# bronemos/view-fusion

Hardware: AMD Instinct MI355X
Metric: denoise_steps_per_sec (higher is better)
Workload: dtype f32; 1 GPU; small UNet 64x64 (33.9M params), B=16/GPU N=6 (S=96 views/GPU), training iteration fwd+bwd+Adam, linear T=2000 schedule; global_batch=16, views=6, parallelism=dp1, launch=HIP-graph replay of the whole iteration

## Files before the change

### include/vf_hip.h

```cpp
#ifndef VF_HIP_H
#define VF_HIP_H
#ifdef __cplusplus
extern "C" {
#endif

int vf_gn_fwd(const float* x, const float* gamma, const float* beta, float* y, float* mean ,
              float* rstd , int S, int C, int HW, int groups, float eps, int silu, void* stream);
int vf_gn_bwd_emits_rowsum(int C, int HW, int groups);
int vf_gn_bwd(const float* x, const float* gamma, const float* beta, const float* mean, const float* rstd,
              const float* dy, const float* addend, float* dx, float* dgamma_part, float* dbeta_part,
              float* dx_rowsum, int S, int C, int HW, int groups, int silu, void* stream);
int vf_gn_cat_fwd(const float* x, const float* x2, int C1, const float* gamma, const float* beta, float* y, float* mean,
                  float* rstd, int S, int C, int HW, int groups, float eps, int silu, void* stream);
int vf_gn_cat_bwd(const float* x, const float* x2, int C1, const float* gamma, const float* beta, const float* mean,
                  const float* rstd, const float* dy, const float* addend, const float* addend2, float* dx, float* dx2,
                  float* dgamma_part, float* dbeta_part, float* dx_rowsum, int S, int C, int HW, int groups, int silu,
                  void* stream);
int vf_rowsum(const float* x, float* out , int rows, int len, void* stream);
int vf_bias_grad(const float* dy, float* db, float* dvb, int S, int C, int HW, void* stream);
int vf_colsum(const float* part , float* out , int batch, int S, int C,
              void* stream);
int vf_colsum_multi(const void* desc, int n, long total_blocks, void* stream);

int vf_conv_pack_sizes(int Cout, int Cin, int KS, long* fwd_floats, long* bwd_floats);
int vf_conv_pack_weights(const float* w_oihw, float* w_fwd, float* w_bwd , int Cout, int Cin, int KS,
                         void* stream);
int vf_conv_pack_weights_multi(const void* desc, int nlayers, long total_blocks, void* stream);
int vf_conv_fwd(const float* x, const float* w_packed, const float* bias ,
                const float* view_bias , const float* residual , float* y,
                float* ws , long ws_floats, int S, int Cin, int Cout, int H, int W, int KS, int mode,
                void* stream);
int vf_conv_fwd_gn(const float* x, const float* w_packed, const float* bias, const float* view_bias, const float* residual,
                   float* y, int store_y, const float* gn_gamma, const float* gn_beta, float* a_out, float* gn_stats,
                   int groups, float eps, int silu, float* ws, long ws_floats, int S, int Cin, int Cout, int H, int W,
                   int KS, int mode, void* stream);
int vf_conv_small_supported(int Cin, int Cout, int H, int W, int KS, int mode);
int vf_conv_small(const float* x, const float* x2 , int C1, const float* w_oihw, const float* bias ,
                  const float* view_bias , const float* residual , float* y, int S, int Cin, int Cout,
                  int H, int W, int KS, int mode, void* stream);
int vf_conv_small_res(const float* x, const float* w_oihw, const float* bias , const float* view_bias ,
                      float* y, int S, int Cin, int Cout, int H, int W, const float* rx, const float* rx2 ,
                      int rC1, int rC, const float* rw_oihw, const float* rbias , void* stream);
int vf_conv_small_gn(const float* x, const float* x2 , int C1, const float* w_oihw, const float* bias ,
                     const float* view_bias , const float* residual , float* y, int S, int Cin,
                     int Cout, int H, int W, int KS, const unsigned long long* in_stats ,
                     const float* in_gamma, const float* in_beta, int in_groups, float eps, int silu,
                     unsigned long long* out_stats , const float* rx , const float* rx2 ,
                     int rC1, int rC, const float* rw_oihw, const float* rbias , const float* w_packed ,
                     int mode, void* stream);
long vf_conv_small_pack_floats(int Cout, int Cin);
int vf_conv_small_pack(const float* w_oihw, float* w_packed, int Cout, int Cin, void* stream);
long vf_conv_fwd_ws_floats(int S, int Cin, int Cout, int H, int W, int KS);
int vf_conv1x1_cat_fwd(const float* x1, const float* x2, int C1, const float* w_packed, const float* bias, float* y,
                       float* ws, long ws_floats, int S, int Cin, int Cout, int H, int W, void* stream);
int vf_conv1x1_cat_dgrad(const float* dy, const float* w_packed_bwd, float* dx1, float* dx2, int C1, int S, int Cin,
                         int Cout, int H, int W, void* stream);
int vf_conv1x1_cat_wgrad(const float* x1, const float* x2, int C1, const float* dy, float* dw_oihw, float* ws,
                         long ws_floats, int S, int Cin, int Cout, int H, int W, void* stream);
long vf_conv1x1_bf16x3_pack_dwords(int M, int K);
int vf_conv1x1_bf16x3_pack(const float* w_oihw, void* w3_fwd, void* w3_bwd, int Cout, int Cin, void* stream);
int vf_conv1x1_bf16x3(const float* x, const float* x2, int C1in, const void* w3, const float* bias,
                      const float* view_bias, const float* residual, float* y, float* y2, int C1out, int S, int Cin,
                      int Cout, int HW, void* stream);
long vf_conv_wgrad_ws_floats(int S, int Cin, int Cout, int H, int W, int KS);
int vf_conv_wgrad(const float* x, const float* dy, float* dw_oihw, float* ws, long ws_floats, int S, int Cin,
                  int Cout, int H, int W, int KS, int mode, void* stream);
int vf_conv_wgrad_main(const float* x, const float* dy, float* dw_oihw, float* ws, long ws_floats, int S, int Cin,
                       int Cout, int H, int W, int KS, int mode, long long* desc9, int* nblocks, void* stream);
int vf_conv1x1_cat_wgrad_main(const float* x1, const float* x2, int C1, const float* dy, float* dw_oihw, float* ws,
                              long ws_floats, int S, int Cin, int Cout, int H, int W, long long* desc9, int* nblocks,
                              void* stream);
int vf_sumpool2(const float* x, float* y, long n_out, int Wo, void* stream);

int vf_wino_supported(int H, int W, int mode);
int vf_wino_pack_sizes(int Cout, int Cin, long* fwd_floats, long* bwd_floats);
int vf_wino_pack_weights(const float* w_oihw, float* u_fwd, float* u_bwd , int Cout, int Cin,
                         void* stream);
int vf_wino_pack_weights_multi(const void* desc, int nlayers, long total_blocks, void* stream);
long vf_wino_conv_ws_floats(int S, int Cin, int Cout, int H, int W);
int vf_wino_conv_fill_pct(int S, int Cin, int Cout, int H, int W, int* tiles_out);
int vf_wino_conv_fwd(const float* x, const float* u_packed, const float* bias, const float* view_bias,
                     const float* residual, float* y, float* ws, long ws_floats, int S, int Cin, int Cout, int H,
                     int W, int mode, void* stream);
int vf_wino_conv_gn_fusable(int S, int Cin, int Cout, int H, int W, int mode, int groups);
int vf_wino_conv_fwd_gn(const float* x, const float* u_packed, const float* bias , const float* view_bias ,
                        const float* residual , float* y, int store_y, const float* gn_gamma, const float* gn_beta,
                        float* a_out, int groups, float eps, int silu, float* ws, long ws_floats, int S, int Cin, int Cout,
                        int H, int W, int mode, void* stream);
int vf_wino44_supported(int H, int W, int mode);
int vf_wino44_pack_sizes(int Cout, int Cin, long* fwd_floats, long* bwd_floats);
int vf_wino44_pack_weights(const float* w_oihw, float* u_fwd, float* u_bwd , int Cout, int Cin,
                           void* stream);
int vf_wino44_pack_weights_multi(const void* desc, int nlayers, long total_blocks, void* stream);
long vf_wino44_conv_ws_floats(int S, int Cin, int Cout, int H, int W);
int vf_wino44_conv_fill_pct(int S, int Cin, int Cout, int H, int W, int* tiles_out);
int vf_wino44_conv_fwd(const float* x, const float* u_packed, const float* bias, const float* view_bias,
                       const float* residual, float* y, float* ws, long ws_floats, int S, int Cin, int Cout, int H,
                       int W, int mode, void* stream);
int vf_wino_wgrad_supported(int H, int W, int mode);
long vf_wino_wgrad_ws_floats(int S, int Cin, int Cout, int H, int W);
int vf_wino_wgrad(const float* x, const float* dy, float* dw_oihw, float* db, float* db2, float* ws, long ws_floats,
                  int S, int Cin, int Cout, int H, int W, int mode, void* stream);
int vf_wino_wgrad_main(const float* x, const float* dy, float* dw_oihw, float* db, float* db2, float* ws, long ws_floats,
                       int S, int Cin, int Cout, int H, int W, int mode, long long* desc9, int* nblocks, void* stream);
int vf_wino44_reduce_multi(const void* table, int nrows, int nblocks, void* stream);

int vf_time_affine_fwd(const void* desc, int ngroups, const float* emb, float* out, int S, int K, int CT,
                       void* stream);
long vf_time_affine_ws_floats(int S, int K);
int vf_time_affine_bwd(const void* desc, int ngroups, const float* emb, const float* de, float* dw ,
                       float* db , const void* gdst, float* demb , float* ws, int S, int K,
                       int CT, void* stream);

int vf_bgemm(const float* A, const float* B, float* C, const float* bias , int batch, int M, int N,
             int K, long sAb, long sAm, long sAk, long sBb, long sBk, long sBn, long sCb, long sCm, long sCn,
             float alpha, float beta, void* stream);
int vf_attention_fwd(const float* qkv, float* out, float* P , int S, int C, int L, void* stream);
int vf_attention_dscore(const float* qkv, const float* dO, const float* P, float* dS, float* dqkv, int S, int C, int L,
                        void* stream);
int vf_attention_dvdk(const float* qkv, const float* dO, const float* P, const float* dS, float* dqkv, int S, int C, int L,
                      void* stream);
int vf_attn_stream_fwd(const float* qkv, float* out, float* lse , int S, int C, int L, void* stream);
int vf_attn_stream_bwd(const float* qkv, const float* out, const float* dO, const float* lse, float* delta,
                       float* dqkv, int S, int C, int L, void* stream);
int vf_softmax_fwd(const float* x, float* y, int rows, int cols, void* stream);
int vf_softmax_bwd(const float* y, const float* dy, float* dx, int rows, int cols, void* stream);

int vf_sincos_embed(const float* level , const float* angle , float* out , int S, int dim,
                    void* stream);
int vf_swish_fwd(const float* x, float* y, long n, void* stream);
int vf_swish_bwd(const float* x, const float* dy, float* dx, long n, void* stream);
int vf_concat_channels(float* a, float* b, float* out, int S, long na, long nb, int split, void* stream);
int vf_dropout(const float* x, const float* u, float* y, long n, float p, void* stream);

int vf_gather_level(const float* gammas, const long long* t, const float* u , float* level, int B,
                    void* stream);
int vf_stack_views(const float* y_cond , const float* y_t ,
                   const float* noise , const float* level, const float* angle, const int* off ,
                   float* x , float* level_s, float* angle_s, int B, int Nmax,
                   int Cc , int HW, int S,
                   int copy_cond, void* stream);
int vf_compose_fwd(const float* unet_out, const int* off, const float* target , float* noise_hat,
                   float* weights , float* loss_part , float* loss, int B,
                   int Cout, int HW, int maxV, int weighting, void* stream);
int vf_compose_mse_bwd(const float* unet_out, const int* off, const float* target, const float* noise_hat,
                       const float* gloss, float* dout, int B, int Cout, int HW, int weighting, void* stream);
int vf_p_sample_tail(const float* unet_out, const int* off, const float* y_t, const float* z ,
                     const long long* t, const float* sqrt_recip_gammas, const float* sqrt_recipm1_gammas,
                     const float* posterior_log_variance, const float* posterior_mean_coef1,
                     const float* posterior_mean_coef2, float* y_next , float* mean_out ,
                     float* weights , int B, int Cout, int HW, int maxV, int weighting, int clip,
                     void* stream);

int vf_psnr(const float* generated, const float* target, float* out , int B, int n, void* stream);

int vf_adam_multi(const void* desc, int ntensors, long total_blocks, float lr, float beta1, float beta2, float eps,
                  float bias_correction1, float bias_correction2, void* stream);
int vf_adam_multi_dev(const void* desc, int ntensors, long total_blocks, const float* scalars, float beta1, float beta2,
                      float eps, void* stream);
int vf_adam_set_scalars(float* scalars, float lr, float bc1, float bc2, void* stream);

int vf_xgmi_alloc(void** ptr, long bytes);
int vf_xgmi_free(void* ptr);
int vf_xgmi_export(void* ptr, void* handle64 );
int vf_xgmi_open(const void* handle64, void** ptr);
int vf_xgmi_close(void* ptr);
int vf_xgmi_signal(const void* const* peer_flags, int world, int rank, int slot, unsigned epoch, void* stream);
int vf_xgmi_wait(const void* my_flags, int world, int slot_lo, int slot_hi, unsigned epoch, void* status,
                 long timeout_us, void* stream);
int vf_xgmi_reduce_adam(const void* desc, int ntensors, long total_blocks, const void* const* peer_bases,
                        const float* my_base, float* gavg_base, int world, const float* scalars, float beta1,
                        float beta2, float eps, void* stream);

#ifdef __cplusplus
}
#endif
#endif
```

### view_fusion_amd/_lib.py

```python
import ctypes
import os

import torch

_HERE = os.path.dirname(os.path.abspath(__file__))
LIB_PATH = os.path.join(_HERE, "lib", "libvf_hip.so")
_OVERRIDE = os.environ.get("VF_HIP_LIB") if os.environ.get("VF_DEBUG_AB") == "1" else None
if _OVERRIDE:
    LIB_PATH = _OVERRIDE
elif os.environ.get("VF_HIP_LIB"):
    import warnings
    warnings.warn("VF_HIP_LIB is ignored unless VF_DEBUG_AB=1 (kernel-tuning aid)", stacklevel=2)

_P, _I, _L, _F = ctypes.c_void_p, ctypes.c_int, ctypes.c_long, ctypes.c_float

SIGNATURES = {
    "vf_gn_fwd": [_P, _P, _P, _P, _P, _P, _I, _I, _I, _I, _F, _I, _P],
    "vf_gn_bwd_emits_rowsum": [_I, _I, _I],
    "vf_gn_cat_fwd": [_P, _P, _I, _P, _P, _P, _P, _P, _I, _I, _I, _I, _F, _I, _P],
    "vf_gn_cat_bwd": [_P, _P, _I, _P, _P, _P, _P, _P, _P, _P, _P, _P, _P, _P, _P, _I, _I, _I, _I, _I, _P],
    "vf_conv1x1_cat_fwd": [_P, _P, _I, _P, _P, _P, _P, _L, _I, _I, _I, _I, _I, _P],
    "vf_conv1x1_cat_dgrad": [_P, _P, _P, _P, _I, _I, _I, _I, _I, _I, _P],
    "vf_conv1x1_cat_wgrad": [_P, _P, _I, _P, _P, _P, _L, _I, _I, _I, _I, _I, _P],
    "vf_gn_bwd": [_P, _P, _P, _P, _P, _P, _P, _P, _P, _P, _P, _I, _I, _I, _I, _I, _P],
    "vf_rowsum": [_P, _P, _I, _I, _P],
    "vf_bias_grad": [_P, _P, _P, _I, _I, _I, _P],
    "vf_colsum": [_P, _P, _I, _I, _I, _P],
    "vf_colsum_multi": [_P, _I, _L, _P],
    "vf_conv_pack_sizes": [_I, _I, _I, ctypes.POINTER(_L), ctypes.POINTER(_L)],
    "vf_conv_pack_weights": [_P, _P, _P, _I, _I, _I, _P],
    "vf_conv_pack_weights_multi": [_P, _I, _L, _P],
    "vf_conv_fwd": [_P, _P, _P, _P, _P, _P, _P, _L, _I, _I, _I, _I, _I, _I, _I, _P],
    "vf_conv_fwd_ws_floats": [_I, _I, _I, _I, _I, _I],
    "vf_conv_fwd_gn": [_P, _P, _P, _P, _P, _P, _I, _P, _P, _P, _P, _I, _F, _I, _P, _L, _I, _I, _I, _I, _I, _I, _I, _P],
    "vf_conv_wgrad_ws_floats": [_I, _I, _I, _I, _I, _I],
    "vf_conv_wgrad": [_P, _P, _P, _P, _L, _I, _I, _I, _I, _I, _I, _I, _P],
    "vf_conv1x1_bf16x3_pack_dwords": [_I, _I],
    "vf_conv1x1_bf16x3_pack": [_P, _P, _P, _I, _I, _P],
    "vf_conv1x1_bf16x3": [_P, _P, _I, _P, _P, _P, _P, _P, _P, _I, _I, _I, _I, _I, _P],
    "vf_wino_supported": [_I, _I, _I],
    "vf_wino_pack_sizes": [_I, _I, ctypes.POINTER(_L), ctypes.POINTER(_L)],
    "vf_wino_pack_weights": [_P, _P, _P, _I, _I, _P],
    "vf_wino_pack_weights_multi": [_P, _I, _L, _P],
    "vf_wino_conv_ws_floats": [_I, _I, _I, _I, _I],
    "vf_wino_conv_fill_pct": [_I, _I, _I, _I, _I, ctypes.POINTER(_I)],
    "vf_wino_conv_fwd": [_P, _P, _P, _P, _P, _P, _P, _L, _I, _I, _I, _I, _I, _I, _P],
    "vf_wino_conv_gn_fusable": [_I, _I, _I, _I, _I, _I, _I],
    "vf_wino_conv_fwd_gn": [_P, _P, _P, _P, _P, _P, _I, _P, _P, _P, _I, _F, _I, _P, _L, _I, _I, _I, _I, _I, _I, _P],
    "vf_wino44_supported": [_I, _I, _I],
    "vf_wino44_pack_sizes": [_I, _I, ctypes.POINTER(_L), ctypes.POINTER(_L)],
    "vf_wino44_pack_weights": [_P, _P, _P, _I, _I, _P],
    "vf_wino44_pack_weights_multi": [_P, _I, _L, _P],
    "vf_wino44_conv_ws_floats": [_I, _I, _I, _I, _I],
    "vf_wino44_conv_fill_pct": [_I, _I, _I, _I, _I, ctypes.POINTER(_I)],
    "vf_wino44_conv_fwd": [_P, _P, _P, _P, _P, _P, _P, _L, _I, _I, _I, _I, _I, _I, _P],
    "vf_wino_wgrad_ws_floats": [_I, _I, _I, _I, _I],
    "vf_wino_wgrad_supported": [_I, _I, _I],
    "vf_wino_wgrad": [_P, _P, _P, _P, _P, _P, _L, _I, _I, _I, _I, _I, _I, _P],
    "vf_wino_wgrad_main": [_P, _P, _P, _P, _P, _P, _L, _I, _I, _I, _I, _I, _I, _P, _P, _P],
    "vf_wino44_reduce_multi": [_P, _I, _I, _P],
    "vf_conv_wgrad_main": [_P, _P, _P, _P, _L, _I, _I, _I, _I, _I, _I, _I, _P, _P, _P],
    "vf_conv1x1_cat_wgrad_main": [_P, _P, _I, _P, _P, _P, _L, _I, _I, _I, _I, _I, _P, _P, _P],
    "vf_sumpool2": [_P, _P, _L, _I, _P],
    "vf_time_affine_fwd": [_P, _I, _P, _P, _I, _I, _I, _P],
    "vf_time_affine_ws_floats": [_I, _I],
    "vf_time_affine_bwd": [_P, _I, _P, _P, _P, _P, _P, _P, _P, _I, _I, _I, _P],
    "vf_bgemm": [_P, _P, _P, _P, _I, _I, _I, _I, _L, _L, _L, _L, _L, _L, _L, _L, _L, _F, _F, _P],
    "vf_attention_fwd": [_P, _P, _P, _I, _I, _I, _P],
    "vf_attention_dscore": [_P, _P, _P, _P, _P, _I, _I, _I, _P],
    "vf_attention_dvdk": [_P, _P, _P, _P, _P, _I, _I, _I, _P],
    "vf_attn_stream_fwd": [_P, _P, _P, _I, _I, _I, _P],
    "vf_attn_stream_bwd": [_P, _P, _P, _P, _P, _P, _I, _I, _I, _P],
    "vf_softmax_fwd": [_P, _P, _I, _I, _P],
    "vf_softmax_bwd": [_P, _P, _P, _I, _I, _P],
    "vf_sincos_embed": [_P, _P, _P, _I, _I, _P],
    "vf_swish_fwd": [_P, _P, _L, _P],
    "vf_swish_bwd": [_P, _P, _P, _L, _P],
    "vf_concat_channels": [_P, _P, _P, _I, _L, _L, _I, _P],
    "vf_dropout": [_P, _P, _P, _L, _F, _P],
    "vf_adam_multi": [_P, _I, _L, _F, _F, _F, _F, _F, _F, _P],
    "vf_conv_small_supported": [_I, _I, _I, _I, _I, _I],
    "vf_conv_small": [_P, _P, _I, _P, _P, _P, _P, _P, _I, _I, _I, _I, _I, _I, _I, _P],
    "vf_conv_small_res": [_P, _P, _P, _P, _P, _I, _I, _I, _I, _I, _P, _P, _I, _I, _P, _P, _P],
    "vf_conv_small_gn": [_P, _P, _I, _P, _P, _P, _P, _P, _I, _I, _I, _I, _I, _I, _P, _P, _P, _I, _F, _I, _P, _P, _P, _I, _I,
                         _P, _P, _P, _I, _P],
    "vf_conv_small_pack_floats": [_I, _I],
    "vf_conv_small_pack": [_P, _P, _I, _I, _P],
    "vf_adam_multi_dev": [_P, _I, _L, _P, _F, _F, _F, _P],
    "vf_adam_set_scalars": [_P, _F, _F, _F, _P],
    "vf_xgmi_alloc": [ctypes.POINTER(_P), _L],
    "vf_xgmi_free": [_P],
    "vf_xgmi_export": [_P, _P],
    "vf_xgmi_open": [_P, ctypes.POINTER(_P)],
    "vf_xgmi_close": [_P],
    "vf_xgmi_signal": [ctypes.POINTER(_P), _I, _I, _I, ctypes.c_uint, _P],
    "vf_xgmi_wait": [_P, _I, _I, _I, ctypes.c_uint, _P, _L, _P],
    "vf_xgmi_reduce_adam": [_P, _I, _L, ctypes.POINTER(_P), _P, _P, _I, _P, _F, _F, _F, _P],
    "vf_psnr": [_P, _P, _P, _I, _I, _P],
    "vf_gather_level": [_P, _P, _P, _P, _I, _P],
    "vf_stack_views": [_P, _P, _P, _P, _P, _P, _P, _P, _P, _I, _I, _I, _I, _I, _I, _P],
    "vf_compose_fwd": [_P, _P, _P, _P, _P, _P, _P, _I, _I, _I, _I, _I, _P],
    "vf_compose_mse_bwd": [_P, _P, _P, _P, _P, _P, _I, _I, _I, _I, _P],
    "vf_p_sample_tail": [_P, _P, _P, _P, _P, _P, _P, _P, _P, _P, _P, _P, _P, _I, _I, _I, _I, _I, _I, _P],
}
_RESTYPE = {"vf_conv1x1_bf16x3_pack_dwords": _L, "vf_conv_wgrad_ws_floats": _L, "vf_time_affine_ws_floats": _L, "vf_wino_conv_ws_floats": _L, "vf_wino44_conv_ws_floats": _L, "vf_wino_wgrad_ws_floats": _L, "vf_conv_fwd_ws_floats": _L,
            "vf_conv_small_pack_floats": _L}

_lib = None
N_CALLS = 0


class VFHipError(RuntimeError):
    pass


def load():
    global _lib
    if _lib is None:
        if not os.path.exists(LIB_PATH):
            raise VFHipError(
                f"{LIB_PATH} not found: build it with `python -m view_fusion_amd.build` "
                "(there is no CPU / eager fallback for the ViewFusion hot path)")
        lib = ctypes.CDLL(LIB_PATH)
        if _OVERRIDE:
            import sys
            print(f"[view_fusion_amd] VF_DEBUG_AB: loading {LIB_PATH} instead of lib/libvf_hip.so", file=sys.stderr)
        missing = [name for name in SIGNATURES if not hasattr(lib, name)]
        if missing:
            raise VFHipError(f"{LIB_PATH} does not export {missing}: stale build? run `python -m view_fusion_amd.build`")
        for name, args in SIGNATURES.items():
            fn = getattr(lib, name)
            fn.argtypes = args
            fn.restype = _RESTYPE.get(name, _I)
        _lib = lib
    return _lib


def call(name, *args):
    global N_CALLS
    N_CALLS += 1
    rc = getattr(load(), name)(*args)
    if rc != 0:
        raise VFHipError(f"{name} failed with hipError_t {rc}")
```

### view_fusion_amd/csrc/common.h

```cpp
#pragma once
#include <hip/hip_runtime.h>
#include <stdint.h>

typedef float f32x2 __attribute__((ext_vector_type(2)));
typedef float f32x4 __attribute__((ext_vector_type(4)));
typedef float f32x16 __attribute__((ext_vector_type(16)));

#define VF_WAVE 64

#define VF_RETURN_LAST_ERROR() return (int)hipGetLastError()

__device__ __forceinline__ float wave_sum(float v) {
#pragma unroll
    for (int o = 32; o > 0; o >>= 1) v += __shfl_xor(v, o, VF_WAVE);
    return v;
}

template <int SEG>
__device__ __forceinline__ float seg_sum(float v) {
#pragma unroll
    for (int o = SEG / 2; o > 0; o >>= 1) v += __shfl_xor(v, o, VF_WAVE);
    return v;
}

__device__ __forceinline__ float wave_max(float v) {
#pragma unroll
    for (int o = 32; o > 0; o >>= 1) v = fmaxf(v, __shfl_xor(v, o, VF_WAVE));
    return v;
}

template <int NT>
__device__ __forceinline__ float block_sum(float v, float* red) {
    v = wave_sum(v);
    const int lane = threadIdx.x & 63, wid = threadIdx.x >> 6;
    __syncthreads();
    if (lane == 0) red[wid] = v;
    __syncthreads();
    float t = 0.f;
#pragma unroll
    for (int i = 0; i < NT / 64; ++i) t += red[i];
    return t;
}

__device__ __forceinline__ float sigmoid_f(float z) {
#ifdef VF_EXACT_SILU
    return 1.0f / (1.0f + expf(-z));
#else
    return __builtin_amdgcn_rcpf(1.0f + __builtin_amdgcn_exp2f(z * -1.44269504088896341f));
#endif
}
__device__ __forceinline__ float silu_f(float z) { return z * sigmoid_f(z); }

__device__ __forceinline__ unsigned xcd_remap(unsigned bid, unsigned nblk) {
    const unsigned q = nblk >> 3, r = nblk & 7u;
    const unsigned xcd = bid & 7u, slot = bid >> 3;
    const unsigned start = xcd < r ? xcd * (q + 1) : r * (q + 1) + (xcd - r) * q;
    return start + slot;
}

__device__ __forceinline__ f32x2 pk_sub(f32x2 a, f32x2 b) {
    f32x2 d;
    asm("v_pk_add_f32 %0, %1, %2 neg_lo:[0,1] neg_hi:[0,1]" : "=v"(d) : "v"(a), "v"(b));
    return d;
}
__device__ __forceinline__ f32x2 pk_add(f32x2 a, f32x2 b) {
    f32x2 d;
    asm("v_pk_add_f32 %0, %1, %2" : "=v"(d) : "v"(a), "v"(b));
    return d;
}
template <int K>
__device__ __forceinline__ f32x2 pk_fmak(f32x2 a, f32x2 c) {
    f32x2 d;
    if (K == 2) asm("v_pk_fma_f32 %0, %1, 2.0, %2 op_sel_hi:[1,0,1]" : "=v"(d) : "v"(a), "v"(c));
    else if (K == 4) asm("v_pk_fma_f32 %0, %1, 4.0, %2 op_sel_hi:[1,0,1]" : "=v"(d) : "v"(a), "v"(c));
    else {
        const f32x2 a2 = pk_add(a, a);
        asm("v_pk_fma_f32 %0, %1, 4.0, %2 op_sel_hi:[1,0,1]" : "=v"(d) : "v"(a2), "v"(c));
    }
    return d;
}
__device__ __forceinline__ f32x2 pk_fma(f32x2 a, f32x2 b, f32x2 c) {
    f32x2 d;
    asm("v_pk_fma_f32 %0, %1, %2, %3" : "=v"(d) : "v"(a), "v"(b), "v"(c));
    return d;
}
__device__ __forceinline__ f32x2 pk_nmul4_add(f32x2 a, f32x2 c) {
    f32x2 d;
    asm("v_pk_fma_f32 %0, %1, 4.0, %2 op_sel_hi:[1,0,1] neg_lo:[1,0,0] neg_hi:[1,0,0]" : "=v"(d) : "v"(a), "v"(c));
    return d;
}
__device__ __forceinline__ f32x2 pk_hi_pm_lo(f32x2 p) {
    f32x2 d;
    asm("v_pk_add_f32 %0, %1, %1 op_sel:[1,0] op_sel_hi:[1,0] neg_hi:[0,1]" : "=v"(d) : "v"(p));
    return d;
}
__device__ __forceinline__ f32x2 pk_hi_pm_2lo(f32x2 q) {
    f32x2 d;
    asm("v_pk_fma_f32 %0, %1, 2.0, %1 op_sel:[0,0,1] op_sel_hi:[0,0,1] neg_hi:[1,0,0]" : "=v"(d) : "v"(q));
    return d;
}
__device__ __forceinline__ f32x2 pk_lo_pm_hi(f32x2 a, f32x2 b) {
    f32x2 d;
    asm("v_pk_add_f32 %0, %1, %2 op_sel:[0,1] op_sel_hi:[0,1] neg_hi:[0,1]" : "=v"(d) : "v"(a), "v"(b));
    return d;
}

__device__ __forceinline__ float dpp_row_shr1(float v) {
    return __int_as_float(__builtin_amdgcn_update_dpp(0, __float_as_int(v), 0x111, 0xf, 0xf, true));
}

#define VF_LDS_BARRIER() asm volatile("s_waitcnt lgkmcnt(0)\n\ts_barrier" ::: "memory")

__device__ __forceinline__ const char* uniform_ptr(const void* p) {
    const unsigned long long v = (unsigned long long)p;
    const unsigned lo = __builtin_amdgcn_readfirstlane((unsigned)v), hi = __builtin_amdgcn_readfirstlane((unsigned)(v >> 32));
    return (const char*)(((unsigned long long)hi << 32) | lo);
}
```

### view_fusion_amd/csrc/norm.hip

```cpp
#include "common.h"
#include "any_geom.h"

namespace {

__device__ __forceinline__ float4 ld_nt(const float4* p) {
    const f32x4 t = __builtin_nontemporal_load(reinterpret_cast<const f32x4*>(p));
    return make_float4(t.x, t.y, t.z, t.w);
}

__device__ __forceinline__ const float4* cat_ptr(const float* x1, const float* x2, int C1, int C, int s, int c,
                                                 int HW) {
    return reinterpret_cast<const float4*>(c < C1 ? x1 + ((size_t)s * C1 + c) * HW
                                                  : x2 + ((size_t)s * (C - C1) + (c - C1)) * HW);
}

template <int NV, int NT>
__global__ __launch_bounds__(NT) void gn_fwd_kernel(const float* __restrict__ x, const float* __restrict__ x2, int C1,
                                                    const float* __restrict__ gamma,
                                                    const float* __restrict__ beta,
                                                    float* __restrict__ y, float* __restrict__ mean_out,
                                                    float* __restrict__ rstd_out, int C, int HW, int cpg,
                                                    float eps, int silu) {
    __shared__ float red[NT / 64];
    const int G = C / cpg;
    const int sg = blockIdx.x;
    const int s = sg / G, g = sg - s * G;
    const size_t base = ((size_t)s * C + (size_t)g * cpg) * HW;
    const int n = cpg * HW, n4 = n >> 2;
    const int hwsh = 31 - __clz(HW >> 2), hwmask = (HW >> 2) - 1;
    const float4* x4 = reinterpret_cast<const float4*>(x + base);
    float4* y4 = reinterpret_cast<float4*>(y + base);

    float4 v[NV];
    float gam[NV], bet[NV];
    if (x2) {
#pragma unroll
        for (int i = 0; i < NV; ++i) {
            const int idc = min((int)threadIdx.x + i * NT, n4 - 1);
            v[i] = cat_ptr(x, x2, C1, C, s, g * cpg + (idc >> hwsh), HW)[idc & hwmask];
        }
    } else {
#pragma unroll
        for (int i = 0; i < NV; ++i) v[i] = x4[min((int)threadIdx.x + i * NT, n4 - 1)];
    }
#pragma unroll
    for (int i = 0; i < NV; ++i) {
        const int c = g * cpg + (min((int)threadIdx.x + i * NT, n4 - 1) >> hwsh);
        gam[i] = gamma[c];
        bet[i] = beta[c];
    }
#ifdef VF_GN_PRESTATS
    const float mean = mean_out[sg], rstd = rstd_out[sg];
    (void)red; (void)n; (void)eps;
#else
    float sum = 0.f;
#pragma unroll
    for (int i = 0; i < NV; ++i) {
        if ((int)threadIdx.x + i * NT >= n4) v[i] = make_float4(0.f, 0.f, 0.f, 0.f);
        sum += (v[i].x + v[i].y) + (v[i].z + v[i].w);
    }
    const float mean = block_sum<NT>(sum, red) / (float)n;
    float sq = 0.f;
#pragma unroll
    for (int i = 0; i < NV; ++i) {
        const float a = v[i].x - mean, b = v[i].y - mean, c = v[i].z - mean, d = v[i].w - mean;
        const float q = (a * a + b * b) + (c * c + d * d);
        sq += (int)threadIdx.x + i * NT < n4 ? q : 0.f;
    }
    const float var = block_sum<NT>(sq, red) / (float)n;
    const float rstd = 1.0f / sqrtf(var + eps);
    if (threadIdx.x == 0) {
        mean_out[sg] = mean;
        rstd_out[sg] = rstd;
    }
#endif
#pragma unroll
    for (int i = 0; i < NV; ++i) {
        const int idx = threadIdx.x + i * NT;
        if (idx < n4) {
            const float ga = gam[i] * rstd;
            const float be = bet[i] - mean * ga;
            float4 o;
            o.x = v[i].x * ga + be;
            o.y = v[i].y * ga + be;
            o.z = v[i].z * ga + be;
            o.w = v[i].w * ga + be;
            if (silu) {
                o.x = silu_f(o.x);
                o.y = silu_f(o.y);
                o.z = silu_f(o.z);
                o.w = silu_f(o.w);
            }
            y4[idx] = o;
        }
    }
}

__device__ __forceinline__ float dsilu_mul(float z, float dy) {
    const float sg = sigmoid_f(z);
    return dy * (sg * (1.0f + z * (1.0f - sg)));
}

__global__ __launch_bounds__(256) void gn_bwd_rows_kernel(const float* __restrict__ x,
                                                          const float* __restrict__ dy,
                                                          const float* __restrict__ gamma,
                                                          const float* __restrict__ beta,
                                                          const float* __restrict__ mean,
                                                          const float* __restrict__ rstd,
                                                          float* __restrict__ dbeta_part,
                                                          float* __restrict__ dgamma_part, int rows, int C,
                                                          int HW, int cpg, int silu) {
    const int row = blockIdx.x * 4 + (threadIdx.x >> 6);
    if (row >= rows) return;
    const int lane = threadIdx.x & 63;
    const int s = row / C, c = row - s * C;
    const int sg = s * (C / cpg) + c / cpg;
    const float mu = mean[sg], r = rstd[sg], ga = gamma[c], be = beta[c];
    const float4* x4 = reinterpret_cast<const float4*>(x + (size_t)row * HW);
    const float4* d4 = reinterpret_cast<const float4*>(dy + (size_t)row * HW);
    float a = 0.f, b = 0.f;
    for (int i = lane; i < (HW >> 2); i += 64) {
        const float4 xv = x4[i], dv = d4[i];
        const float xs[4] = {xv.x, xv.y, xv.z, xv.w};
        const float ds[4] = {dv.x, dv.y, dv.z, dv.w};
#pragma unroll
        for (int j = 0; j < 4; ++j) {
            const float xh = (xs[j] - mu) * r;
            const float dz = silu ? dsilu_mul(xh * ga + be, ds[j]) : ds[j];
            a += dz;
            b += dz * xh;
        }
    }
    a = wave_sum(a);
    b = wave_sum(b);
    if (lane == 0) {
        dbeta_part[row] = a;
        dgamma_part[row] = b;
    }
}

__global__ __launch_bounds__(256) void gn_bwd_dx_kernel(const float* __restrict__ x,
                                                        const float* __restrict__ dy,
                                                        const float* __restrict__ gamma,
                                                        const float* __restrict__ beta,
                                                        const float* __restrict__ mean,
                                                        const float* __restrict__ rstd,
                                                        const float* __restrict__ dbeta_part,
                                                        const float* __restrict__ dgamma_part,
                                                        float* __restrict__ dx, int C, int HW, int cpg,
                                                        int silu) {
    const int G = C / cpg;
    const int sg = blockIdx.x;
    const int s = sg / G, g = sg - s * G;
    float s1 = 0.f, s2 = 0.f;
    for (int j = 0; j < cpg; ++j) {
        const int c = g * cpg + j;
        const float ga = gamma[c];
        s1 += ga * dbeta_part[s * C + c];
        s2 += ga * dgamma_part[s * C + c];
    }
    const int n = cpg * HW, n4 = n >> 2;
    const int hwsh = 31 - __clz(HW >> 2);
    const float inv_n = 1.0f / (float)n;
    s1 *= inv_n;
    s2 *= inv_n;
    const float mu = mean[sg], r = rstd[sg];
    const size_t base = ((size_t)s * C + (size_t)g * cpg) * HW;
    const float4* x4 = reinterpret_cast<const float4*>(x + base);
    const float4* d4 = reinterpret_cast<const float4*>(dy + base);
    float4* o4 = reinterpret_cast<float4*>(dx + base);
    for (int i = blockIdx.y * 256 + threadIdx.x; i < n4; i += gridDim.y * 256) {
        const int c = g * cpg + (i >> hwsh);
        const float ga = gamma[c], be = beta[c];
        const float4 xv = x4[i], dv = d4[i];
        const float xs[4] = {xv.x, xv.y, xv.z, xv.w};
        const float ds[4] = {dv.x, dv.y, dv.z, dv.w};
        float o[4];
#pragma unroll
        for (int j = 0; j < 4; ++j) {
            const float xh = (xs[j] - mu) * r;
            const float dz = silu ? dsilu_mul(xh * ga + be, ds[j]) : ds[j];
            o[j] = r * (dz * ga - (s1 + xh * s2));
        }
        o4[i] = make_float4(o[0], o[1], o[2], o[3]);
    }
}


template <int NV, int NT, int SEG = 64>
__global__ __launch_bounds__(NT) void gn_bwd_fused_kernel(const float* __restrict__ x, const float* __restrict__ x2,
                                                          int C1, const float* __restrict__ dy,
                                                          const float* __restrict__ gamma,
                                                          const float* __restrict__ beta,
                                                          const float* __restrict__ mean,
                                                          const float* __restrict__ rstd,
                                                          const float* __restrict__ addend,
                                                          const float* __restrict__ addend2, float* __restrict__ dx,
                                                          float* __restrict__ dx2,
                                                          float* __restrict__ dgamma_part,
                                                          float* __restrict__ dbeta_part,
                                                          float* __restrict__ dx_rowsum, int C, int HW, int cpg,
                                                          int silu) {
    constexpr int NWV = NT / 64;
    extern __shared__ float part[];
    const int G = C / cpg;
    const int sg = blockIdx.x;
    const int s = sg / G, g = sg - s * G;
    const size_t base = ((size_t)s * C + (size_t)g * cpg) * HW;
    const int n = cpg * HW, n4 = n >> 2;
    const int hwsh = 31 - __clz(HW >> 2), hwmask = (HW >> 2) - 1;
    const float4* x4 = reinterpret_cast<const float4*>(x + base);
    const float4* d4 = reinterpret_cast<const float4*>(dy + base);
    const int lane = threadIdx.x & 63, wid = threadIdx.x >> 6;
    const float mu = mean[sg], r = rstd[sg];

    for (int i = threadIdx.x; i < NWV * cpg * 3; i += NT) part[i] = 0.f;
    __syncthreads();

    float4 xv[NV], dv[NV];
    float gam[NV], bet[NV];
    if (x2) {
#pragma unroll
        for (int i = 0; i < NV; ++i) {
            const int idc = min((int)threadIdx.x + i * NT, n4 - 1);
            xv[i] = cat_ptr(x, x2, C1, C, s, g * cpg + (idc >> hwsh), HW)[idc & hwmask];
            dv[i] = d4[idc];
        }
    } else {
#pragma unroll
        for (int i = 0; i < NV; ++i) {
            const int idc = min((int)threadIdx.x + i * NT, n4 - 1);
            xv[i] = ld_nt(x4 + idc);
            dv[i] = ld_nt(d4 + idc);
        }
    }
#pragma unroll
    for (int i = 0; i < NV; ++i) {
        if (SEG == 64) {
            const int c = __builtin_amdgcn_readfirstlane(g * cpg + (min(wid * 64 + i * NT, n4 - 1) >> hwsh));
            gam[i] = gamma[c];
            bet[i] = beta[c];
        } else {
            const int c = g * cpg + (min((int)threadIdx.x + i * NT, n4 - 1) >> hwsh);
            gam[i] = gamma[c];
            bet[i] = beta[c];
        }
    }
#pragma unroll
    for (int i = 0; i < NV; ++i) {
        const int idx0 = wid * 64 + i * NT + (SEG == 64 ? 0 : (lane & ~(SEG - 1)));
        float a = 0.f, b = 0.f, xsum = 0.f;
        int cl = 0;
        if (idx0 < n4) {
            cl = idx0 >> hwsh;
            const float ga = gam[i], be = bet[i];
            float xs[4] = {xv[i].x, xv[i].y, xv[i].z, xv[i].w};
            float ds[4] = {dv[i].x, dv[i].y, dv[i].z, dv[i].w};
            const bool ok = threadIdx.x + i * NT < n4;
#pragma unroll
            for (int j = 0; j < 4; ++j) {
                const float xh = (xs[j] - mu) * r;
                float dz = silu ? dsilu_mul(xh * ga + be, ds[j]) : ds[j];
                if (!ok) dz = 0.f;
                xs[j] = xh; ds[j] = dz;
                a += dz; b += dz * xh;
                xsum += ok ? xh : 0.f;
            }
            xv[i] = make_float4(xs[0], xs[1], xs[2], xs[3]);
            dv[i] = make_float4(ds[0], ds[1], ds[2], ds[3]);
        }
        a = seg_sum<SEG>(a);
        b = seg_sum<SEG>(b);
        if (dx_rowsum) xsum = seg_sum<SEG>(xsum);
        if ((lane & (SEG - 1)) == 0 && idx0 < n4) {
            part[(wid * cpg + cl) * 3 + 0] += a;
            part[(wid * cpg + cl) * 3 + 1] += b;
            part[(wid * cpg + cl) * 3 + 2] += xsum;
        }
    }
    __syncthreads();
    float s1 = 0.f, s2 = 0.f, myA = 0.f, myX = 0.f;
    for (int c = 0; c < cpg; ++c) {
        float A = 0.f, B = 0.f, X = 0.f;
#pragma unroll
        for (int w = 0; w < NWV; ++w) {
            A += part[(w * cpg + c) * 3]; B += part[(w * cpg + c) * 3 + 1]; X += part[(w * cpg + c) * 3 + 2];
        }
        const float ga = gamma[g * cpg + c];
        s1 += ga * A; s2 += ga * B;
        if (threadIdx.x == c) {
            dbeta_part[(size_t)s * C + g * cpg + c] = A;
            dgamma_part[(size_t)s * C + g * cpg + c] = B;
            myA = ga * A; myX = X;
        }
    }
    const float inv_n = 1.0f / (float)n;
    s1 *= inv_n; s2 *= inv_n;
    if (dx_rowsum && threadIdx.x < cpg)
        dx_rowsum[(size_t)s * C + g * cpg + threadIdx.x] = r * (myA - (float)HW * s1 - s2 * myX);
    float4* o4 = reinterpret_cast<float4*>(dx + base);
    const float4* a4 = addend ? reinterpret_cast<const float4*>(addend + base) : nullptr;
#pragma unroll
    for (int i = 0; i < NV; ++i) {
        const float ga = gam[i];
        dv[i].x = r * (dv[i].x * ga - (s1 + xv[i].x * s2));
        dv[i].y = r * (dv[i].y * ga - (s1 + xv[i].y * s2));
        dv[i].z = r * (dv[i].z * ga - (s1 + xv[i].z * s2));
        dv[i].w = r * (dv[i].w * ga - (s1 + xv[i].w * s2));
    }
    if (x2) {
        if (addend) {
#pragma unroll
            for (int i = 0; i < NV; ++i) {
                const int idc = min((int)threadIdx.x + i * NT, n4 - 1);
                xv[i] = cat_ptr(addend, addend2, C1, C, s, g * cpg + (idc >> hwsh), HW)[idc & hwmask];
            }
#pragma unroll
            for (int i = 0; i < NV; ++i) { dv[i].x += xv[i].x; dv[i].y += xv[i].y; dv[i].z += xv[i].z; dv[i].w += xv[i].w; }
        }
#pragma unroll
        for (int i = 0; i < NV; ++i) {
            const int idx = threadIdx.x + i * NT;
            if (idx < n4)
                const_cast<float4*>(cat_ptr(dx, dx2, C1, C, s, g * cpg + (idx >> hwsh), HW))[idx & hwmask] = dv[i];
        }
        return;
    }
    if (a4) {
#pragma unroll
        for (int i = 0; i < NV; ++i) xv[i] = a4[min((int)threadIdx.x + i * NT, n4 - 1)];
#pragma unroll
        for (int i = 0; i < NV; ++i) { dv[i].x += xv[i].x; dv[i].y += xv[i].y; dv[i].z += xv[i].z; dv[i].w += xv[i].w; }
    }
    if (addend2) {
        const float4* b4 = reinterpret_cast<const float4*>(addend2 + base);
#pragma unroll
        for (int i = 0; i < NV; ++i) xv[i] = b4[min((int)threadIdx.x + i * NT, n4 - 1)];
#pragma unroll
        for (int i = 0; i < NV; ++i) { dv[i].x += xv[i].x; dv[i].y += xv[i].y; dv[i].z += xv[i].z; dv[i].w += xv[i].w; }
    }
#pragma unroll
    for (int i = 0; i < NV; ++i) {
        const int idx = threadIdx.x + i * NT;
        if (idx < n4) o4[idx] = dv[i];
    }
}

__global__ void add_inplace_kernel(float4* __restrict__ y, const float4* __restrict__ a, size_t n4) {
    const size_t i = (size_t)blockIdx.x * blockDim.x + threadIdx.x;
    if (i < n4) { float4 v = y[i]; const float4 t = a[i]; v.x += t.x; v.y += t.y; v.z += t.z; v.w += t.w; y[i] = v; }
}

__device__ __forceinline__ float lane_sum_f4(const float4* __restrict__ p, int n4, int lane) {
    float acc[8] = {0.f, 0.f, 0.f, 0.f, 0.f, 0.f, 0.f, 0.f};
    int i = lane;
    for (; i + 7 * 64 < n4; i += 8 * 64) {
        float4 v[8];
#pragma unroll
        for (int j = 0; j < 8; ++j) v[j] = p[i + 64 * j];
#pragma unroll
        for (int j = 0; j < 8; ++j) acc[j] += (v[j].x + v[j].y) + (v[j].z + v[j].w);
    }
    if (i < n4) {
        float4 v[8];
#pragma unroll
        for (int j = 0; j < 8; ++j) v[j] = p[min(i + 64 * j, n4 - 1)];
#pragma unroll
        for (int j = 0; j < 8; ++j) acc[j] += i + 64 * j < n4 ? (v[j].x + v[j].y) + (v[j].z + v[j].w) : 0.f;
    }
    return ((acc[0] + acc[1]) + (acc[2] + acc[3])) + ((acc[4] + acc[5]) + (acc[6] + acc[7]));
}

__global__ __launch_bounds__(256) void rowsum_kernel(const float* __restrict__ x, float* __restrict__ out,
                                                     int rows, int len) {
    const int row = blockIdx.x * 4 + (threadIdx.x >> 6);
    if (row >= rows) return;
    const int lane = threadIdx.x & 63;
    const float4* x4 = reinterpret_cast<const float4*>(x + (size_t)row * len);
    const float a = wave_sum(lane_sum_f4(x4, len >> 2, lane));
    if (lane == 0) out[row] = a;
}

__global__ __launch_bounds__(256) void bias_grad_kernel(const float* __restrict__ dy, float* __restrict__ db,
                                                        float* __restrict__ dvb, int S, int C, int HW) {
    __shared__ float red[4];
    const int c = blockIdx.x, lane = threadIdx.x & 63, wid = threadIdx.x >> 6;
    float tot = 0.f;
    const int n4 = HW >> 2;
    if (n4 <= 64) {
        for (int s = wid; s < S; s += 32) {
            float4 v[8];
#pragma unroll
            for (int j = 0; j < 8; ++j)
                v[j] = reinterpret_cast<const float4*>(dy + ((size_t)min(s + 4 * j, S - 1) * C + c) * HW)[min(lane, n4 - 1)];
#pragma unroll
            for (int j = 0; j < 8; ++j) {
                const float a = wave_sum(lane < n4 ? (v[j].x + v[j].y) + (v[j].z + v[j].w) : 0.f);
                if (s + 4 * j < S) {
                    if (lane == 0 && dvb) dvb[(size_t)(s + 4 * j) * C + c] = a;
                    tot += a;
                }
            }
        }
    } else {
        for (int s = wid; s < S; s += 4) {
            const float4* p = reinterpret_cast<const float4*>(dy + ((size_t)s * C + c) * HW);
            const float a = wave_sum(lane_sum_f4(p, n4, lane));
            if (lane == 0 && dvb) dvb[(size_t)s * C + c] = a;
            tot += a;
        }
    }
    if (lane == 0) red[wid] = tot;
    __syncthreads();
    if (threadIdx.x == 0 && db) db[c] = (red[0] + red[1]) + (red[2] + red[3]);
}

__global__ __launch_bounds__(256) void colsum_kernel(const float* __restrict__ part, float* __restrict__ out,
                                                     int S, int C) {
    __shared__ float red[4][64];
    const int cx = threadIdx.x & 63, ry = threadIdx.x >> 6;
    const int c = blockIdx.x * 64 + cx;
    const float* p = part + (size_t)blockIdx.y * S * C;
    float a = 0.f;
    if (c < C) {
        float acc[8] = {0.f, 0.f, 0.f, 0.f, 0.f, 0.f, 0.f, 0.f};
        for (int s = ry; s < S; s += 32) {
            float t[8];
#pragma unroll
            for (int j = 0; j < 8; ++j) t[j] = p[(size_t)min(s + 4 * j, S - 1) * C + c];
#pragma unroll
            for (int j = 0; j < 8; ++j) acc[j] += s + 4 * j < S ? t[j] : 0.f;
        }
        a = ((acc[0] + acc[1]) + (acc[2] + acc[3])) + ((acc[4] + acc[5]) + (acc[6] + acc[7]));
    }
    red[ry][cx] = a;
    __syncthreads();
    if (ry == 0 && c < C) out[(size_t)blockIdx.y * C + c] = (red[0][cx] + red[1][cx]) + (red[2][cx] + red[3][cx]);
}

struct ColsumDesc {
    const float* part;
    float* out;
    long long S, C, batch, first_block;
};
__global__ __launch_bounds__(256) void colsum_multi_kernel(const ColsumDesc* __restrict__ desc, int n) {
    __shared__ float red[4][64];
    const long long vb = blockIdx.x;
    int lo = 0, hi = n;
    while (hi - lo > 1) {
        const int mid = (lo + hi) >> 1;
        if (desc[mid].first_block <= vb) lo = mid; else hi = mid;
    }
    const ColsumDesc d = desc[lo];
    const int S = (int)d.S, C = (int)d.C;
    const int nbx = (C + 63) / 64;
    const int rel = (int)(vb - d.first_block);
    const int bx = rel % nbx, by = rel / nbx;
    const int cx = threadIdx.x & 63, ry = threadIdx.x >> 6;
    const int c = bx * 64 + cx;
    const float* p = d.part + (size_t)by * S * C;
    float a = 0.f;
    if (c < C) {
        float acc[8] = {0.f, 0.f, 0.f, 0.f, 0.f, 0.f, 0.f, 0.f};
        for (int s = ry; s < S; s += 32) {
            float t[8];
#pragma unroll
            for (int j = 0; j < 8; ++j) t[j] = p[(size_t)min(s + 4 * j, S - 1) * C + c];
#pragma unroll
            for (int j = 0; j < 8; ++j) acc[j] += s + 4 * j < S ? t[j] : 0.f;
        }
        a = ((acc[0] + acc[1]) + (acc[2] + acc[3])) + ((acc[4] + acc[5]) + (acc[6] + acc[7]));
    }
    red[ry][cx] = a;
    __syncthreads();
    if (ry == 0 && c < C) d.out[(size_t)by * C + c] = (red[0][cx] + red[1][cx]) + (red[2][cx] + red[3][cx]);
}

template <int NV, int NT>
int launch_gn_fwd(const float* x, const float* x2, int C1, const float* gamma, const float* beta, float* y, float* mean,
                  float* rstd, int S, int C, int HW, int cpg, float eps, int silu, hipStream_t st) {
    hipLaunchKernelGGL((gn_fwd_kernel<NV, NT>), dim3(S * (C / cpg)), dim3(NT), 0, st, x, x2, C1, gamma, beta, y, mean,
                       rstd, C, HW, cpg, eps, silu);
    VF_RETURN_LAST_ERROR();
}

}

extern "C" {

int vf_gn_cat_fwd(const float* x, const float* x2, int C1, const float* gamma, const float* beta, float* y, float* mean,
                  float* rstd, int S, int C, int HW, int groups, float eps, int silu, void* stream) {
    hipStream_t st = (hipStream_t)stream;
    if (S <= 0) return 0;
    if (groups <= 0 || C % groups != 0 || (x2 && (C1 <= 0 || C1 >= C))) return (int)hipErrorInvalidValue;
    const int cpg = C / groups;
    const long n4 = (long)cpg * HW / 4;
    if (HW < 4 || (HW & (HW - 1)) || n4 > 32768) {
        if (x2) return (int)hipErrorInvalidValue;
        return vfi_gn_any_fwd(x, gamma, beta, y, mean, rstd, S, C, HW, groups, eps, silu, st);
    }
#define VF_GN(NV, NT) return launch_gn_fwd<NV, NT>(x, x2, C1, gamma, beta, y, mean, rstd, S, C, HW, cpg, eps, silu, st)
    if (n4 <= 64) VF_GN(1, 64);
    if (n4 <= 256) VF_GN(1, 256);
    if (n4 <= 512) VF_GN(2, 256);
    if (n4 <= 1024) VF_GN(4, 256);
    if (n4 <= 2048) VF_GN(8, 256);
    if (n4 <= 3072) VF_GN(12, 256);
    if (n4 <= 4096) VF_GN(16, 256);
    if (n4 <= 6144) VF_GN(12, 512);
    if (n4 <= 8192) VF_GN(16, 512);
    if (n4 <= 16384) VF_GN(16, 1024);
    if (n4 <= 32768) VF_GN(32, 1024);
#undef VF_GN
    return (int)hipErrorInvalidValue;
}

int vf_gn_fwd(const float* x, const float* gamma, const float* beta, float* y, float* mean, float* rstd, int S,
              int C, int HW, int groups, float eps, int silu, void* stream) {
    return vf_gn_cat_fwd(x, nullptr, C, gamma, beta, y, mean, rstd, S, C, HW, groups, eps, silu, stream);
}

int vf_gn_bwd_emits_rowsum(int C, int HW, int groups) {
    if (groups <= 0 || C % groups != 0 || HW < 4 || (HW & (HW - 1))) return 0;
    const long n4g = (long)(C / groups) * HW / 4;
    return ((HW >= 256 && n4g <= 8192) || (HW == 64 && n4g <= 1024)) ? 1 : 0;
}

int vf_gn_cat_bwd(const float* x, const float* x2, int C1, const float* gamma, const float* beta, const float* mean,
                  const float* rstd, const float* dy, const float* addend, const float* addend2, float* dx, float* dx2,
                  float* dgamma_part, float* dbeta_part, float* dx_rowsum, int S, int C, int HW, int groups, int silu,
                  void* stream) {
    hipStream_t st = (hipStream_t)stream;
    if (S <= 0) return 0;
    if (groups <= 0 || C % groups != 0) return (int)hipErrorInvalidValue;
    if (HW < 4 || (HW & (HW - 1))) {
        if (x2) return (int)hipErrorInvalidValue;
        return vfi_gn_any_bwd(x, gamma, beta, mean, rstd, dy, addend, addend2, dx, dgamma_part, dbeta_part, S, C, HW, groups,
                              silu, st);
    }
    if (x2 && (C1 <= 0 || C1 >= C || !dx2 || (addend && !addend2) || !vf_gn_bwd_emits_rowsum(C, HW, groups)))
        return (int)hipErrorInvalidValue;
    const int cpg = C / groups;
    const int rows = S * C;
    const long n4g = (long)cpg * HW / 4;
    if (HW == 64 && n4g <= 1024) {
#define VF_GNB16(NV)                                                                                       \
    {                                                                                                      \
        hipLaunchKernelGGL((gn_bwd_fused_kernel<NV, 256, 16>), dim3(S * groups), dim3(256), 4 * cpg * 3 * 4, st, x, x2, C1, dy, \
                           gamma, beta, mean, rstd, addend, addend2, dx, dx2, dgamma_part, dbeta_part, dx_rowsum, C, HW, cpg, silu); \
        VF_RETURN_LAST_ERROR();                                                                            \
    }
        if (n4g <= 256) VF_GNB16(1)
        if (n4g <= 512) VF_GNB16(2)
        VF_GNB16(4)
#undef VF_GNB16
    }
    if (HW >= 256 && n4g <= 8192) {
#define VF_GNB(NV, NT)                                                                                     \
    {                                                                                                      \
        hipLaunchKernelGGL((gn_bwd_fused_kernel<NV, NT>), dim3(S * groups), dim3(NT), (NT / 64) * cpg * 3 * 4, st, \
                           x, x2, C1, dy, gamma, beta, mean, rstd, addend, addend2, dx, dx2, dgamma_part, dbeta_part, \
                           dx_rowsum, C, HW, cpg, silu);                                                   \
        VF_RETURN_LAST_ERROR();                                                                            \
    }
        if (n4g <= 256) VF_GNB(1, 256)
        if (n4g <= 512) VF_GNB(2, 256)
        if (n4g <= 1024) VF_GNB(4, 256)
        if (n4g <= 2048) VF_GNB(8, 256)
        if (n4g <= 4096) VF_GNB(8, 512)
        if (n4g <= 6144) VF_GNB(12, 512)
        VF_GNB(8, 1024)
#undef VF_GNB
    }
    hipLaunchKernelGGL(gn_bwd_rows_kernel, dim3((rows + 3) / 4), dim3(256), 0, st, x, dy, gamma, beta, mean, rstd,
                       dbeta_part, dgamma_part, rows, C, HW, cpg, silu);
    const int n4 = cpg * HW / 4;
    int chunks = (n4 + 1023) / 1024;
    if (chunks < 1) chunks = 1;
    hipLaunchKernelGGL(gn_bwd_dx_kernel, dim3(S * groups, chunks), dim3(256), 0, st, x, dy, gamma, beta, mean,
                       rstd, dbeta_part, dgamma_part, dx, C, HW, cpg, silu);
    const size_t t4 = (size_t)S * C * HW / 4;
    if (addend)
        hipLaunchKernelGGL(add_inplace_kernel, dim3((unsigned)((t4 + 255) / 256)), dim3(256), 0, st, (float4*)dx,
                           (const float4*)addend, t4);
    if (addend2)
        hipLaunchKernelGGL(add_inplace_kernel, dim3((unsigned)((t4 + 255) / 256)), dim3(256), 0, st, (float4*)dx,
                           (const float4*)addend2, t4);
    VF_RETURN_LAST_ERROR();
}

int vf_gn_bwd(const float* x, const float* gamma, const float* beta, const float* mean, const float* rstd,
              const float* dy, const float* addend, float* dx, float* dgamma_part, float* dbeta_part,
              float* dx_rowsum, int S, int C, int HW, int groups, int silu, void* stream) {
    return vf_gn_cat_bwd(x, nullptr, C, gamma, beta, mean, rstd, dy, addend, nullptr, dx, nullptr, dgamma_part,
                         dbeta_part, dx_rowsum, S, C, HW, groups, silu, stream);
}

int vf_rowsum(const float* x, float* out, int rows, int len, void* stream) {
    if (rows <= 0) return 0;
    if (len & 3) return vfi_rowsum_any(x, out, rows, len, (hipStream_t)stream);
    hipLaunchKernelGGL(rowsum_kernel, dim3((rows + 3) / 4), dim3(256), 0, (hipStream_t)stream, x, out, rows, len);
    VF_RETURN_LAST_ERROR();
}

int vf_bias_grad(const float* dy, float* db, float* dvb, int S, int C, int HW, void* stream) {
    if (S <= 0 || C <= 0) return 0;
    if (HW & 3) return vfi_bias_grad_any(dy, db, dvb, S, C, HW, (hipStream_t)stream);
    hipLaunchKernelGGL(bias_grad_kernel, dim3(C), dim3(256), 0, (hipStream_t)stream, dy, db, dvb, S, C, HW);
    VF_RETURN_LAST_ERROR();
}

int vf_colsum_multi(const void* desc, int n, long total_blocks, void* stream) {
    if (n <= 0 || total_blocks <= 0) return 0;
    hipLaunchKernelGGL(colsum_multi_kernel, dim3((unsigned)total_blocks), dim3(256), 0, (hipStream_t)stream,
                       (const ColsumDesc*)desc, n);
    VF_RETURN_LAST_ERROR();
}

int vf_colsum(const float* part, float* out, int batch, int S, int C, void* stream) {
    if (C <= 0 || batch <= 0) return 0;
    hipLaunchKernelGGL(colsum_kernel, dim3((C + 63) / 64, batch), dim3(256), 0, (hipStream_t)stream, part, out, S,
                       C);
    VF_RETURN_LAST_ERROR();
}

}
```

### view_fusion_amd/csrc/winograd24.hip

```cpp
#include "common.h"
#include "wino_plan.h"

namespace {

constexpr int WTCO = 64;
constexpr int WTT = 32;
constexpr int WCK = 8;
constexpr int NSL = 24;
constexpr int WINO_PERSIST = 256;

struct WinoArgs {
    const float* x;
    const float* u;
    const float* bias;
    const float* vbias;
    const float* res;
    float* y;
    int S, Cin, Cout, CinP, CoutP;
    int nfull, tail_split;
    float* ws;
    int npers;
};

template <int LOGW, int MODE>
// ... 381 lines not shown
                    make_float4(o1[rr][0] + bb + er[rr][1].x, o1[rr][1] + bb + er[rr][1].y,
                                o1[rr][2] + bb + er[rr][1].z, o1[rr][3] + bb + er[rr][1].w);
            }
        }
#ifdef VF_STAMPS
        {
            const unsigned long long t_3 = __builtin_amdgcn_s_memtime();
            st_pro += t_1 - t_0; st_loop += t_2 - t_1; st_epi += t_3 - t_2; st_tiles += 1; st_ea += t_a - t_2; st_eb += t_b - t_a; st_ec += t_c - t_b;
        }
#endif
        if (!has_next) break;
        VF_STAMP(t_g);
        VF_STAGE_V0();
        VF_STAMP(t_h);
        VF_LDS_BARRIER();
#ifdef VF_STAMPS
        {
            const unsigned long long t_i = __builtin_amdgcn_s_memtime();
            st_x[0] += t_d - t_c; st_x[1] += t_e - t_d; st_x[2] += t_f - t_e; st_x[3] += t_g - t_f; st_x[4] += t_h - t_g; st_x[5] += t_i - t_h; st_x[6] += 1;
        }
#endif
        cur = nx;
        lin = lin_next;
    }
#ifdef VF_STAMPS
    if (tid == 0 && !partial) {
        atomicAdd(&g_stamps[0], st_pro); atomicAdd(&g_stamps[1], st_loop); atomicAdd(&g_stamps[2], st_epi);
        atomicAdd(&g_stamps[3], st_tiles); atomicAdd(&g_stamps[4], st_ea); atomicAdd(&g_stamps[5], st_eb); atomicAdd(&g_stamps[6], st_ec);
        for (int i = 0; i < 8; ++i) atomicAdd(&g_stamps[8 + i], st_x[i]);
    }
#endif
#undef VF_STAMP
#undef VF_ULOAD
#undef VF_ULOAD_ALL
#undef VF_XLOAD
#undef VF_XSTORE
#undef VF_XZERO
#undef VF_STAGE_ROWS
#undef VF_STAGE_V0
#undef VF_SLICE
#undef VF_BFRAG
#undef VF_CHUNK
#undef VF_WREAD
}

__device__ __forceinline__ void wino_pack_group(const float* __restrict__ w, float* __restrict__ uf,
                                                float* __restrict__ ub, int Cout, int Cin, size_t nf, size_t nb,
                                                size_t group) {
    constexpr int GSZ = NSL * WTCO * WCK;
    const size_t ngf = nf / GSZ;
    const bool bwd = group >= ngf;
    if (bwd) {
        group -= ngf;
        if (group >= nb / GSZ || !ub) return;
    }
    const int M = bwd ? Cin : Cout, K = bwd ? Cout : Cin;
    const int nchunk = (K + WCK - 1) / WCK;
    const int chunk = group % nchunk, mt = group / nchunk;
    const int t = threadIdx.x;
    const int m = t >> 3, k8 = t & 7;
    const int mm = mt * 64 + m, kk = chunk * WCK + k8;
    double g[9];
#pragma unroll
    for (int i = 0; i < 9; ++i) g[i] = 0.0;
    if (mm < M && kk < K) {
        const int co = bwd ? kk : mm, ci = bwd ? mm : kk;
        const float* p = w + ((size_t)co * Cin + ci) * 9;
#pragma unroll
        for (int i = 0; i < 9; ++i) g[i] = (double)(bwd ? p[8 - i] : p[i]);
    }
    double tq[4][3];
#pragma unroll
    for (int q = 0; q < 3; ++q) {
        const double h = 0.5 * (g[q] + g[6 + q]), e = 0.5 * g[3 + q];
        tq[0][q] = g[q];
        tq[1][q] = h + e;
        tq[2][q] = h - e;
        tq[3][q] = g[6 + q];
    }
    float* out = (bwd ? ub : uf) + group * (size_t)GSZ + t;
#pragma unroll
    for (int i = 0; i < 4; ++i) {
        const double x0 = i == 3 ? -tq[i][0] : tq[i][0], x1 = i == 3 ? -tq[i][1] : tq[i][1], x2 = i == 3 ? -tq[i][2] : tq[i][2];
        const double a6 = -(x0 + x2) / 6.0, b6 = x1 / 6.0;
        const double a24 = x0 / 24.0 + x2 / 6.0, b12 = x1 / 12.0;
        out[(6 * i + 0) * (WTCO * WCK)] = (float)(x0 / 4.0);
        out[(6 * i + 1) * (WTCO * WCK)] = (float)(a6 - b6);
        out[(6 * i + 2) * (WTCO * WCK)] = (float)(a6 + b6);
        out[(6 * i + 3) * (WTCO * WCK)] = (float)(a24 + b12);
        out[(6 * i + 4) * (WTCO * WCK)] = (float)(a24 - b12);
        out[(6 * i + 5) * (WTCO * WCK)] = (float)x2;
    }
}

__global__ __launch_bounds__(512) void wino_pack_kernel(const float* __restrict__ w, float* __restrict__ uf,
                                                        float* __restrict__ ub, int Cout, int Cin, size_t nf,
                                                        size_t nb) {
    wino_pack_group(w, uf, ub, Cout, Cin, nf, nb, blockIdx.x);
}

constexpr int PACK_BLOCKS = NSL * WTCO * WCK / 256;

struct WPackDesc {
    const float* w;
    float* uf;
    float* ub;
    long long Cout, Cin, nf, nb, first_block;
};
__global__ __launch_bounds__(512) void wino_pack_multi_kernel(const WPackDesc* __restrict__ desc, int nlayers) {
    const long long vb = (long long)blockIdx.x * PACK_BLOCKS;
    int lo = 0, hi = nlayers;
    while (hi - lo > 1) {
        const int mid = (lo + hi) >> 1;
        if (desc[mid].first_block <= vb) lo = mid; else hi = mid;
    }
    const WPackDesc d = desc[lo];
    wino_pack_group(d.w, d.uf, d.ub, (int)d.Cout, (int)d.Cin, (size_t)d.nf, (size_t)d.nb,
                    (size_t)((vb - d.first_block) / PACK_BLOCKS));
}

inline int rup(int v, int m) { return (v + m - 1) / m * m; }

template <int LOGW>
__global__ __launch_bounds__(256) void wino_fixup_kernel(WinoArgs a, int ntail) {
    using G = WGeo<LOGW, 0>;
    const size_t idx = (size_t)blockIdx.x * 256 + threadIdx.x;
    const int tl = idx % WTT;
    const int col = (idx / WTT) % WTCO;
    const int j = idx / (WTT * WTCO);
    if (j >= ntail) return;
    const int ncot = a.CoutP / WTCO;
    const int logical = a.nfull + j;
    const int cot = logical % ncot, wg = logical / ncot;
    const int s = G::g_view(wg) + G::t_img(tl), r0 = G::g_row(wg);
    const int co = cot * WTCO + col;
    if (s >= a.S || co >= a.Cout) return;
    const int orow = r0 + 2 * G::t_row(tl), ocol = 4 * G::t_col(tl);
    const size_t o = ((size_t)s * a.Cout + co) * G::HW + (size_t)orow * G::W + ocol;
    float4 t0[8], t1[8];
#pragma unroll
    for (int p = 0; p < 8; ++p) {
        const float* w8 = a.ws + ((((size_t)j * a.tail_split + min(p, a.tail_split - 1)) * WTCO + col) * WTT + tl) * 8;
        t0[p] = *reinterpret_cast<const float4*>(w8);
        t1[p] = *reinterpret_cast<const float4*>(w8 + 4);
    }
    float b = 0.f;
    if (a.bias) b += a.bias[co];
    if (a.vbias) b += a.vbias[(size_t)s * a.Cout + co];
    float4 q0 = make_float4(0.f, 0.f, 0.f, 0.f), q1 = q0;
    if (a.res) {
        q0 = *reinterpret_cast<const float4*>(a.res + o);
        q1 = *reinterpret_cast<const float4*>(a.res + o + G::W);
    }
    float4 v0 = make_float4(0.f, 0.f, 0.f, 0.f), v1 = v0;
#pragma unroll
    for (int p = 0; p < 8; ++p) {
        if (p < a.tail_split) {
            v0.x += t0[p].x; v0.y += t0[p].y; v0.z += t0[p].z; v0.w += t0[p].w;
            v1.x += t1[p].x; v1.y += t1[p].y; v1.z += t1[p].z; v1.w += t1[p].w;
        }
    }
    v0.x += b; v0.y += b; v0.z += b; v0.w += b;
    v1.x += b; v1.y += b; v1.z += b; v1.w += b;
    v0.x += q0.x; v0.y += q0.y; v0.z += q0.z; v0.w += q0.w;
    v1.x += q1.x; v1.y += q1.y; v1.z += q1.z; v1.w += q1.w;
    *reinterpret_cast<float4*>(a.y + o) = v0;
    *reinterpret_cast<float4*>(a.y + o + G::W) = v1;
}

template <int LOGW, int NV>
__global__ __launch_bounds__(512) void wino_fixup_gn_kernel(WinoArgs a, const float* __restrict__ gamma,
                                                            const float* __restrict__ beta, float* __restrict__ a_out,
                                                            int store_y, int cpg, float eps, int silu) {
    using G = WGeo<LOGW, 0>;
    static_assert(G::IPG == 1, "maps of at least 16x16");
    constexpr int NT = 512, TPV = G::HW / 8;
    __shared__ float red[NT / 64];
    const int ngroups = a.Cout / cpg;
    const int s = blockIdx.x / ngroups, g = blockIdx.x - s * ngroups;
    const int nel = cpg * TPV, ncot = a.CoutP / WTCO;
    float4 v0[NV], v1[NV];
    size_t oo[NV];
    float gam[NV], bet[NV], badd[NV];
    float4 t0[NV][4], t1[NV][4];
    const float* wsb[NV];
#pragma unroll
    for (int i = 0; i < NV; ++i) {
        const int e = min((int)threadIdx.x + i * NT, nel - 1);
        const int c = g * cpg + e / TPV, tv = e % TPV;
        const int wg = s * G::WPI + tv / WTT, tl = tv % WTT;
        const int j = wg * ncot + c / WTCO;
        wsb[i] = a.ws + (((size_t)j * a.tail_split * WTCO + c % WTCO) * WTT + tl) * 8;
#pragma unroll
        for (int p = 0; p < 4; ++p) {
            const float* w8 = wsb[i] + (size_t)min(p, a.tail_split - 1) * (WTCO * WTT * 8);
            t0[i][p] = *reinterpret_cast<const float4*>(w8);
            t1[i][p] = *reinterpret_cast<const float4*>(w8 + 4);
        }
        const int orow = G::g_row(wg) + 2 * G::t_row(tl), ocol = 4 * G::t_col(tl);
        oo[i] = ((size_t)s * a.Cout + c) * G::HW + (size_t)orow * G::W + ocol;
        float b = 0.f;
        if (a.bias) b += a.bias[c];
        if (a.vbias) b += a.vbias[(size_t)s * a.Cout + c];
        badd[i] = b;
        gam[i] = gamma[c];
        bet[i] = beta[c];
        v0[i] = make_float4(0.f, 0.f, 0.f, 0.f);
        v1[i] = v0[i];
        if (a.res) {
            v0[i] = *reinterpret_cast<const float4*>(a.res + oo[i]);
            v1[i] = *reinterpret_cast<const float4*>(a.res + oo[i] + G::W);
        }
    }
    float sum = 0.f;
#pragma unroll
    for (int i = 0; i < NV; ++i) {
        float4 q0 = make_float4(0.f, 0.f, 0.f, 0.f), q1 = q0;
#pragma unroll
        for (int p = 0; p < 4; ++p) {
            if (p < a.tail_split) {
                q0.x += t0[i][p].x; q0.y += t0[i][p].y; q0.z += t0[i][p].z; q0.w += t0[i][p].w;
                q1.x += t1[i][p].x; q1.y += t1[i][p].y; q1.z += t1[i][p].z; q1.w += t1[i][p].w;
            }
        }
        if (a.tail_split > 4) {
            float4 u0[4], u1[4];
#pragma unroll
            for (int p = 0; p < 4; ++p) {
                const float* w8 = wsb[i] + (size_t)min(4 + p, a.tail_split - 1) * (WTCO * WTT * 8);
                u0[p] = *reinterpret_cast<const float4*>(w8);
                u1[p] = *reinterpret_cast<const float4*>(w8 + 4);
            }
#pragma unroll
            for (int p = 0; p < 4; ++p) {
                if (4 + p < a.tail_split) {
                    q0.x += u0[p].x; q0.y += u0[p].y; q0.z += u0[p].z; q0.w += u0[p].w;
                    q1.x += u1[p].x; q1.y += u1[p].y; q1.z += u1[p].z; q1.w += u1[p].w;
                }
            }
        }
        const float b = badd[i];
        q0.x += b; q0.y += b; q0.z += b; q0.w += b;
        q1.x += b; q1.y += b; q1.z += b; q1.w += b;
        v0[i] = make_float4(q0.x + v0[i].x, q0.y + v0[i].y, q0.z + v0[i].z, q0.w + v0[i].w);
        v1[i] = make_float4(q1.x + v1[i].x, q1.y + v1[i].y, q1.z + v1[i].z, q1.w + v1[i].w);
        const bool ok = (int)threadIdx.x + i * NT < nel;
        if (store_y && ok) {
            *reinterpret_cast<float4*>(a.y + oo[i]) = v0[i];
            *reinterpret_cast<float4*>(a.y + oo[i] + G::W) = v1[i];
        }
        if (!ok) { v0[i] = make_float4(0.f, 0.f, 0.f, 0.f); v1[i] = v0[i]; }
        sum += ((v0[i].x + v0[i].y) + (v0[i].z + v0[i].w)) + ((v1[i].x + v1[i].y) + (v1[i].z + v1[i].w));
    }
    const float inv_n = 1.0f / (float)(nel * 8);
    const float mean = block_sum<NT>(sum, red) * inv_n;
    float sq = 0.f;
#pragma unroll
    for (int i = 0; i < NV; ++i) {
        const float d0 = v0[i].x - mean, d1 = v0[i].y - mean, d2 = v0[i].z - mean, d3 = v0[i].w - mean;
        const float d4 = v1[i].x - mean, d5 = v1[i].y - mean, d6 = v1[i].z - mean, d7 = v1[i].w - mean;
        const float q = ((d0 * d0 + d1 * d1) + (d2 * d2 + d3 * d3)) + ((d4 * d4 + d5 * d5) + (d6 * d6 + d7 * d7));
        sq += (int)threadIdx.x + i * NT < nel ? q : 0.f;
    }
    const float var = block_sum<NT>(sq, red) * inv_n;
    const float rstd = 1.0f / sqrtf(var + eps);
#pragma unroll
    for (int i = 0; i < NV; ++i) {
        if ((int)threadIdx.x + i * NT < nel) {
            const float ga = gam[i] * rstd, be = bet[i] - mean * ga;
            float4 o0 = make_float4(v0[i].x * ga + be, v0[i].y * ga + be, v0[i].z * ga + be, v0[i].w * ga + be);
            float4 o1 = make_float4(v1[i].x * ga + be, v1[i].y * ga + be, v1[i].z * ga + be, v1[i].w * ga + be);
            if (silu) {
                o0.x = silu_f(o0.x); o0.y = silu_f(o0.y); o0.z = silu_f(o0.z); o0.w = silu_f(o0.w);
                o1.x = silu_f(o1.x); o1.y = silu_f(o1.y); o1.z = silu_f(o1.z); o1.w = silu_f(o1.w);
            }
            *reinterpret_cast<float4*>(a_out + oo[i]) = o0;
            *reinterpret_cast<float4*>(a_out + oo[i] + G::W) = o1;
        }
    }
}

inline int wino_groups(int S, int H, int W) {
    const int tiles = (H / 2) * (W / 4);
    return tiles >= WTT ? S * (tiles / WTT) : (S + WTT / tiles - 1) / (WTT / tiles);
}

struct WinoGn {
    const float* gamma = nullptr;
    const float* beta = nullptr;
    float* a_out = nullptr;
    int groups = 0, silu = 0, store_y = 1;
    float eps = 0.f;
};

inline bool wino_gn_fusable(int S, int Cin, int Cout, int H, int W, int groups) {
    if (W < 16 || groups <= 0 || Cout % groups != 0) return false;
    const int T = wino_groups(S, H, W) * (rup(Cout, WTCO) / WTCO);
    int nfull, split;
    wino_tail_plan(T, rup(Cin, WCK) / WCK, &nfull, &split);
    return nfull == 0 && split >= 2 && split <= 8 && (long)(Cout / groups) * (H * W / 8) <= 2048;
}

template <int LOGW, int MODE>
int launch_wino(WinoArgs a, size_t ws_floats, hipStream_t st, const WinoGn& gn = WinoGn()) {
    using G = WGeo<LOGW, MODE>;
    const int T = G::groups(a.S) * (a.CoutP / WTCO);
    wino_tail_plan(T, a.CinP / WCK, &a.nfull, &a.tail_split);
    const int ntail = T - a.nfull;
    if ((size_t)ntail * a.tail_split * WTCO * WTT * 8 > ws_floats || !a.ws) {
        a.nfull = T;
        a.tail_split = 1;
    }
    const int nt = T - a.nfull;
    if (gn.gamma && !(a.nfull == 0 && a.tail_split >= 2)) return (int)hipErrorInvalidValue;
    a.npers = a.nfull < WINO_PERSIST ? a.nfull : WINO_PERSIST;
    hipLaunchKernelGGL((wino_conv_kernel<LOGW, MODE>), dim3(a.npers + nt * a.tail_split), dim3(512), 0, st, a);
    if constexpr (LOGW >= 4) {
        if (gn.gamma) {
            const int cpg = a.Cout / gn.groups;
            const long nel = (long)cpg * ((1 << (2 * LOGW)) / 8);
            const dim3 grid(a.S * gn.groups);
#define VF_FGN(NV) hipLaunchKernelGGL((wino_fixup_gn_kernel<LOGW, NV>), grid, dim3(512), 0, st, a, gn.gamma, gn.beta, gn.a_out, \
                                      gn.store_y, cpg, gn.eps, gn.silu)
            if (nel <= 512) VF_FGN(1);
            else if (nel <= 1024) VF_FGN(2);
            else VF_FGN(4);
#undef VF_FGN
            VF_RETURN_LAST_ERROR();
        }
    }
    if (nt > 0)
        hipLaunchKernelGGL((wino_fixup_kernel<LOGW>), dim3((nt * WTCO * WTT + 255) / 256), dim3(256), 0, st, a, nt);
    VF_RETURN_LAST_ERROR();
}

}

extern "C" {

int vf_wino_pack_sizes(int Cout, int Cin, long* fwd_floats, long* bwd_floats) {
    *fwd_floats = (long)NSL * rup(Cin, WCK) * rup(Cout, WTCO);
    *bwd_floats = (long)NSL * rup(Cout, WCK) * rup(Cin, WTCO);
    return 0;
}

int vf_wino_pack_weights(const float* w_oihw, float* u_fwd, float* u_bwd, int Cout, int Cin, void* stream) {
    const size_t nf = (size_t)NSL * rup(Cin, WCK) * rup(Cout, WTCO);
    const size_t nb = u_bwd ? (size_t)NSL * rup(Cout, WCK) * rup(Cin, WTCO) : 0;
    hipLaunchKernelGGL(wino_pack_kernel, dim3((unsigned)((nf + nb) / (NSL * WTCO * WCK))), dim3(512), 0,
                       (hipStream_t)stream, w_oihw, u_fwd, u_bwd, Cout, Cin, nf, nb);
    VF_RETURN_LAST_ERROR();
}

int vf_wino_pack_weights_multi(const void* desc, int nlayers, long total_blocks, void* stream) {
    if (nlayers <= 0 || total_blocks <= 0) return 0;
    hipLaunchKernelGGL(wino_pack_multi_kernel, dim3((unsigned)(total_blocks / PACK_BLOCKS)), dim3(512), 0,
                       (hipStream_t)stream, (const WPackDesc*)desc, nlayers);
    VF_RETURN_LAST_ERROR();
}

int vf_wino_supported(int H, int W, int mode) {
    return (H == W && (W == 8 || W == 16 || W == 32 || W == 64) && (mode == 0 || mode == 2)) ? 1 : 0;
}

long vf_wino_conv_ws_floats(int S, int Cin, int Cout, int H, int W) {
    const int T = wino_groups(S, H, W) * (rup(Cout, WTCO) / WTCO);
    int nfull, split;
    wino_tail_plan(T, rup(Cin, WCK) / WCK, &nfull, &split);
    return (long)(T - nfull) * split * WTCO * WTT * 8;
}

int vf_wino_conv_fill_pct(int S, int Cin, int Cout, int H, int W, int* tiles_out) {
    const int T = wino_groups(S, H, W) * (rup(Cout, WTCO) / WTCO);
    const int nch = rup(Cin, WCK) / WCK;
    int nfull, split;
    wino_tail_plan(T, nch, &nfull, &split, 0.0);
    if (tiles_out) *tiles_out = T;
    if (T <= 0) return 0;
    const double time = (nfull + WINO_SLOTS - 1) / WINO_SLOTS + (T > nfull ? wino_tail_time(T - nfull, split, nch, 0.0) : 0.0);
    return (int)(100.0 * T / WINO_SLOTS / time);
}

int vf_wino_conv_fwd(const float* x, const float* u_packed, const float* bias, const float* view_bias,
                     const float* residual, float* y, float* ws, long ws_floats, int S, int Cin, int Cout, int H,
                     int W, int mode, void* stream) {
    if (S <= 0) return 0;
    if (!vf_wino_supported(H, W, mode)) return (int)hipErrorInvalidValue;
    WinoArgs a;
    a.x = x; a.u = u_packed; a.bias = bias; a.vbias = view_bias; a.res = residual; a.y = y;
    a.S = S; a.Cin = Cin; a.Cout = Cout; a.CinP = rup(Cin, WCK); a.CoutP = rup(Cout, WTCO);
    a.ws = ws;
    hipStream_t st = (hipStream_t)stream;
    const size_t nws = ws ? (size_t)ws_floats : 0;
    if (W == 8) return mode == 0 ? launch_wino<3, 0>(a, nws, st) : launch_wino<3, 2>(a, nws, st);
    if (W == 16) return mode == 0 ? launch_wino<4, 0>(a, nws, st) : launch_wino<4, 2>(a, nws, st);
    if (W == 32) return mode == 0 ? launch_wino<5, 0>(a, nws, st) : launch_wino<5, 2>(a, nws, st);
    return mode == 0 ? launch_wino<6, 0>(a, nws, st) : launch_wino<6, 2>(a, nws, st);
}

int vf_wino_conv_gn_fusable(int S, int Cin, int Cout, int H, int W, int mode, int groups) {
    return (vf_wino_supported(H, W, mode) && wino_gn_fusable(S, Cin, Cout, H, W, groups)) ? 1 : 0;
}

int vf_wino_conv_fwd_gn(const float* x, const float* u_packed, const float* bias, const float* view_bias,
                        const float* residual, float* y, int store_y, const float* gn_gamma, const float* gn_beta,
                        float* a_out, int groups, float eps, int silu, float* ws, long ws_floats, int S, int Cin, int Cout,
                        int H, int W, int mode, void* stream) {
    if (S <= 0) return 0;
    if (!vf_wino_conv_gn_fusable(S, Cin, Cout, H, W, mode, groups) || !ws || !gn_gamma || !gn_beta || !a_out)
        return (int)hipErrorInvalidValue;
    WinoArgs a;
    a.x = x; a.u = u_packed; a.bias = bias; a.vbias = view_bias; a.res = residual; a.y = y;
    a.S = S; a.Cin = Cin; a.Cout = Cout; a.CinP = rup(Cin, WCK); a.CoutP = rup(Cout, WTCO);
    a.ws = ws;
    WinoGn gn;
    gn.gamma = gn_gamma; gn.beta = gn_beta; gn.a_out = a_out; gn.groups = groups; gn.silu = silu; gn.store_y = store_y; gn.eps = eps;
    hipStream_t st = (hipStream_t)stream;
    const size_t nws = (size_t)ws_floats;
    if (W == 16) return mode == 0 ? launch_wino<4, 0>(a, nws, st, gn) : launch_wino<4, 2>(a, nws, st, gn);
    if (W == 32) return mode == 0 ? launch_wino<5, 0>(a, nws, st, gn) : launch_wino<5, 2>(a, nws, st, gn);
    return mode == 0 ? launch_wino<6, 0>(a, nws, st, gn) : launch_wino<6, 2>(a, nws, st, gn);
}

}

#ifdef VF_STAMPS
extern "C" void vf_debug_stamps(unsigned long long* out8, int reset) {
    if (out8) (void)hipMemcpyFromSymbol(out8, HIP_SYMBOL(g_stamps), 128);
    if (reset) { unsigned long long z[16] = {0}; (void)hipMemcpyToSymbol(HIP_SYMBOL(g_stamps), z, 128); }
}
#endif
```

### view_fusion_amd/csrc/winograd44f.hip

```cpp
#include "common.h"
#include "wino_plan.h"

namespace {

constexpr int FCO = 64;
constexpr int FTT = 32;
constexpr int FCK = 8;
constexpr int FNS = 36;
constexpr int F44_PERSIST = 256;

__host__ __device__ constexpr int f44_p(int a, int b) {
    return a == 0 ? b : a == 1 ? (b < 3 ? 6 + b : 12 + b) : a == 2 ? 9 + b : a == 3 ? 18 + b
         : a == 4 ? (b < 3 ? 24 + b : 30 + b) : 27 + b;
}

struct F44Args {
    const float* x;
    const float* u;
    const float* bias;
    const float* vbias;
    const float* res;
    float* y;
    int S, Cin, Cout, CinP, CoutP;
    int nfull, tail_split;
// ... 295 lines not shown
            int c = 1;                                                                                   \
            for (; c + 1 < nch; c += 2) {                                                                \
                VF_CHUNK(c, 1, 0, bfB, bfA, TH);                                                         \
                VF_CHUNK(c + 1, 0, 0, bfA, bfB, TH);                                                     \
            }                                                                                            \
            if (c < nch) VF_CHUNK(c, 1, 0, bfB, bfA, TH);                                                \
        }
        if (nch <= 0) {
#pragma unroll
            for (int b = 0; b < 9; ++b) acc[b] = (f32x16){0};
        } else if (th == 0) {
            VF_LOOP(0);
        } else {
            VF_LOOP(1);
        }
#undef VF_LOOP

        VF_STAMP(t_2);
        const unsigned lin_next = lin + F44_PERSIST;
        const bool has_next = !partial && lin_next < (unsigned)a.nfull;
        const unsigned logical_cur = logical_of(lin);
        int s, r0, cot_;
        tile_pos(logical_cur, s, r0, cot_);
        const int co0 = cot_ * FCO;

        int lane_e = lane;
        asm volatile("" : "+v"(lane_e));
        const int li_e = lane_e & 31, lh_e = lane_e >> 5;
        const int orow = r0 + 4 * G::t_row(li_e), ocol = 4 * G::t_col(li_e);
        float* const xch = Vl;
        const Tile nx = make_tile(has_next ? logical_of(lin_next) : logical_cur);
        VF_ULOAD_ALL(nx, 0);
        VF_XLOAD(nx, 0, xr0, xr1, xr2);
        VF_XLOAD(nx, min(1, clast), yr0, yr1, yr2);

        const bool jh = wg_ & 1;
        constexpr int XB = 8 * 7 * 4 * 64;
        static_assert(2 * XB <= XCH && VSZ <= XB, "exchange buffers");
        const int cob = co0 + cw * 32 + 4 * lh_e + wg_;
        float ebias[4];
#pragma unroll
        for (int k = 0; k < 4; ++k) ebias[k] = 0.f;
        if (!partial) {
            if (a.bias) {
#pragma unroll
                for (int k = 0; k < 4; ++k) ebias[k] = a.bias[min(cob + 8 * k, a.Cout - 1)];
            }
            if (a.vbias) {
#pragma unroll
                for (int k = 0; k < 4; ++k) ebias[k] += a.vbias[(size_t)s * a.Cout + min(cob + 8 * k, a.Cout - 1)];
            }
        }
        float4 er[4];
#pragma unroll
        for (int y = 0; y < 4; ++y) er[y] = make_float4(0.f, 0.f, 0.f, 0.f);
#pragma unroll
        for (int ph = 0; ph < 5; ++ph) {
            if (ph < 4) {
                float* xo = xch + (ph & 1) * XB + (size_t)(wid * 7) * (4 * 64) + lane_e;
#pragma unroll
                for (int k = 0; k < 2; ++k) {
                    const int r = 4 * ph + 2 * k;
                    const f32x2 m0 = (f32x2){acc[0][r], acc[0][r + 1]}, m1 = (f32x2){acc[1][r], acc[1][r + 1]};
                    const f32x2 m2 = (f32x2){acc[2][r], acc[2][r + 1]}, m3 = (f32x2){acc[3][r], acc[3][r + 1]};
                    const f32x2 m4 = (f32x2){acc[4][r], acc[4][r + 1]}, m5 = (f32x2){acc[5][r], acc[5][r + 1]};
                    const f32x2 s12 = pk_add(m1, m2), d12 = pk_sub(m1, m2), s34 = pk_add(m3, m4), d34 = pk_sub(m3, m4);
                    const f32x2 T0 = pk_add(pk_add(m0, s12), s34);
                    const f32x2 T1 = pk_fmak<2>(d34, d12);
                    const f32x2 T2 = pk_fmak<4>(s34, s12);
                    const f32x2 T3 = pk_add(pk_fmak<8>(d34, d12), m5);
                    const f32x2 h0 = (f32x2){acc[6][r], acc[6][r + 1]}, h1 = (f32x2){acc[7][r], acc[7][r + 1]};
                    const f32x2 h2 = (f32x2){acc[8][r], acc[8][r + 1]};
                    f32x2 H0, H1, H2;
                    if (jh) {
                        H0 = pk_add(h0, h1); H1 = pk_sub(h0, h1); H2 = h2;
                    } else {
                        H2 = pk_add(h1, h2); H1 = pk_sub(h1, h2); H0 = pk_add(h0, H2);
                    }
                    xo[(0 * 4 + 2 * k) * 64] = T0.x; xo[(0 * 4 + 2 * k + 1) * 64] = T0.y;
                    xo[(1 * 4 + 2 * k) * 64] = T1.x; xo[(1 * 4 + 2 * k + 1) * 64] = T1.y;
                    xo[(2 * 4 + 2 * k) * 64] = T2.x; xo[(2 * 4 + 2 * k + 1) * 64] = T2.y;
                    xo[(3 * 4 + 2 * k) * 64] = T3.x; xo[(3 * 4 + 2 * k + 1) * 64] = T3.y;
                    xo[(4 * 4 + 2 * k) * 64] = H0.x; xo[(4 * 4 + 2 * k + 1) * 64] = H0.y;
                    xo[(5 * 4 + 2 * k) * 64] = H1.x; xo[(5 * 4 + 2 * k + 1) * 64] = H1.y;
                    xo[(6 * 4 + 2 * k) * 64] = H2.x; xo[(6 * 4 + 2 * k + 1) * 64] = H2.y;
                }
            }
            if (ph > 0) {
                constexpr int GS = 2 * 7 * 4 * 64, VS = 4 * 64;
                const int co = cob + 8 * (ph - 1);
                const float* xi = xch + ((ph - 1) & 1) * XB + (size_t)(cw * 7) * (4 * 64) + wg_ * 64 + lane_e;
                float T[6][4];
#pragma unroll
                for (int c = 0; c < 4; ++c) {
                    T[0][c] = xi[0 * GS + c * VS];
                    T[2][c] = xi[1 * GS + c * VS];
                    T[3][c] = xi[2 * GS + c * VS];
                    T[5][c] = xi[3 * GS + c * VS];
                }
                {
                    const float A_ = xi[0 * GS + 4 * VS], B_ = xi[0 * GS + 5 * VS], C_ = xi[0 * GS + 6 * VS];
                    const float D_ = xi[1 * GS + 4 * VS], E_ = xi[1 * GS + 5 * VS], F_ = xi[1 * GS + 6 * VS];
                    T[1][0] = A_ + D_; T[1][1] = __builtin_fmaf(2.f, E_, B_); T[1][2] = __builtin_fmaf(4.f, D_, C_);
                    T[1][3] = __builtin_fmaf(8.f, E_, B_) + F_;
                }
                {
                    const float A_ = xi[2 * GS + 4 * VS], B_ = xi[2 * GS + 5 * VS], C_ = xi[2 * GS + 6 * VS];
                    const float D_ = xi[3 * GS + 4 * VS], E_ = xi[3 * GS + 5 * VS], F_ = xi[3 * GS + 6 * VS];
                    T[4][0] = A_ + D_; T[4][1] = __builtin_fmaf(2.f, E_, B_); T[4][2] = __builtin_fmaf(4.f, D_, C_);
                    T[4][3] = __builtin_fmaf(8.f, E_, B_) + F_;
                }
                float Y[4][4];
#pragma unroll
                for (int c = 0; c < 4; ++c) {
                    const float S12 = T[1][c] + T[2][c], D12 = T[1][c] - T[2][c];
                    const float S34 = T[3][c] + T[4][c], D34 = T[3][c] - T[4][c];
                    Y[0][c] = (T[0][c] + S12) + S34;
                    Y[1][c] = __builtin_fmaf(2.f, D34, D12);
                    Y[2][c] = __builtin_fmaf(4.f, S34, S12);
                    Y[3][c] = __builtin_fmaf(8.f, D34, D12) + T[5][c];
                }
                if (partial) {
                    float* w16 = a.ws + (((size_t)tail_id * FCO + (co - co0)) * FTT + li_e) * 16;
#pragma unroll
                    for (int y = 0; y < 4; ++y)
                        *reinterpret_cast<float4*>(w16 + 4 * y) = make_float4(Y[y][0], Y[y][1], Y[y][2], Y[y][3]);
                } else if (co < a.Cout) {
                    const float bb = ebias[ph - 1];
                    const size_t o = ((size_t)s * a.Cout + co) * G::HW + (size_t)orow * G::W + ocol;
#pragma unroll
                    for (int y = 0; y < 4; ++y)
                        *reinterpret_cast<float4*>(a.y + o + y * G::W) =
                            make_float4(Y[y][0] + bb + er[y].x, Y[y][1] + bb + er[y].y, Y[y][2] + bb + er[y].z,
                                        Y[y][3] + bb + er[y].w);
                }
            }
            if (ph < 4 && !partial && a.res) {
                const int co = min(cob + 8 * ph, a.Cout - 1);
                const size_t o = ((size_t)s * a.Cout + co) * G::HW + (size_t)orow * G::W + ocol;
#pragma unroll
                for (int y = 0; y < 4; ++y) er[y] = *reinterpret_cast<const float4*>(a.res + o + y * G::W);
            }
            if (ph == 3 && has_next) VF_STAGE_ROWS(nx);
            if (ph == 4 && has_next) VF_STAGE_V0();
#ifdef VF_STAMPS44F
            t_p[ph] = __builtin_amdgcn_s_memtime();
#endif
            if (ph < 4 || has_next) VF_LDS_BARRIER();
        }
        VF_STAMP(t_3);
#ifdef VF_STAMPS44F
        st_e[2] += t_p[0] - t_2; st_e[3] += t_p[1] - t_p[0]; st_e[4] += t_p[2] - t_p[1];
        st_e[5] += t_p[3] - t_p[2]; st_e[6] += t_p[4] - t_p[3];
        st_loop += t_2 - t_1; st_epi += t_3 - t_2; st_tiles += 1; st_e[0] += t_3 - t_2;
#endif
        if (!has_next) break;
        cur = nx;
        lin = lin_next;
    }
#ifdef VF_STAMPS44F
    if (tid == 0 && !partial) {
        atomicAdd(&g_stamps44f[0], st_loop); atomicAdd(&g_stamps44f[1], st_epi); atomicAdd(&g_stamps44f[2], st_tiles);
        for (int i = 0; i < 7; ++i) atomicAdd(&g_stamps44f[3 + i], st_e[i]);
        atomicAdd(&g_stamps44f[10], __builtin_amdgcn_s_memtime() - ct_0);
        atomicAdd(&g_stamps44f[11], __builtin_amdgcn_s_memrealtime() - rt_0);
    }
#endif
#undef VF_STAMP
#undef VF_ULOAD
#undef VF_ULOAD_ALL
#undef VF_XLOAD
#undef VF_XST1
#undef VF_XSTORE
#undef VF_SID
#undef VF_SROW
#undef VF_SCG
#undef VF_SUY
#undef VF_STAGE_ROWS
#undef VF_STAGE_V0
#undef VF_SLICE
#undef VF_BFRAG
#undef VF_CHUNK
#undef VF_WIN_READ4
#undef VF_WIN_READ2
#undef VF_WIN_WRITE
}

__device__ __forceinline__ void f44_pack_group(const float* __restrict__ w, float* __restrict__ uf,
                                               float* __restrict__ ub, int Cout, int Cin, size_t nf, size_t nb,
                                               size_t group) {
    constexpr int GSZ = FNS * FCO * FCK;
    const size_t ngf = nf / GSZ;
    const bool bwd = group >= ngf;
    if (bwd) {
        group -= ngf;
        if (group >= nb / GSZ || !ub) return;
    }
    const int M = bwd ? Cin : Cout, K = bwd ? Cout : Cin;
    const int nchunk = (K + FCK - 1) / FCK;
    const int chunk = group % nchunk, mt = group / nchunk;
    const int t = threadIdx.x;
    const int m = t >> 3, k8 = t & 7;
    const int mm = mt * 64 + m, kk = chunk * FCK + k8;
    double g[9];
#pragma unroll
    for (int i = 0; i < 9; ++i) g[i] = 0.0;
    if (mm < M && kk < K) {
        const int co = bwd ? kk : mm, ci = bwd ? mm : kk;
        const float* p = w + ((size_t)co * Cin + ci) * 9;
#pragma unroll
        for (int i = 0; i < 9; ++i) g[i] = (double)(bwd ? p[8 - i] : p[i]);
    }
    auto g4 = [](double x0, double x1, double x2, double* o) {
        const double a6 = -(x0 + x2) / 6.0, b6 = x1 / 6.0;
        const double a24 = x0 / 24.0 + x2 / 6.0, b12 = x1 / 12.0;
        o[0] = x0 / 4.0; o[1] = a6 - b6; o[2] = a6 + b6; o[3] = a24 + b12; o[4] = a24 - b12; o[5] = x2;
    };
    double tq[6][3];
#pragma unroll
    for (int q = 0; q < 3; ++q) {
        double o[6];
        g4(g[q], g[3 + q], g[6 + q], o);
#pragma unroll
        for (int i = 0; i < 6; ++i) tq[i][q] = o[i];
    }
    float* out = (bwd ? ub : uf) + group * (size_t)GSZ + t;
#pragma unroll
    for (int i = 0; i < 6; ++i) {
        double o[6];
        g4(tq[i][0], tq[i][1], tq[i][2], o);
#pragma unroll
        for (int j = 0; j < 6; ++j) out[f44_p(i, j) * (FCO * FCK)] = (float)o[j];
    }
}

__global__ __launch_bounds__(512) void wino44f_pack_kernel(const float* __restrict__ w, float* __restrict__ uf,
                                                           float* __restrict__ ub, int Cout, int Cin, size_t nf,
                                                           size_t nb) {
    f44_pack_group(w, uf, ub, Cout, Cin, nf, nb, blockIdx.x);
}

constexpr int F44_PACK_BLOCKS = FNS * FCO * FCK / 256;

struct F44PackDesc {
    const float* w;
    float* uf;
    float* ub;
    long long Cout, Cin, nf, nb, first_block;
};
__global__ __launch_bounds__(512) void wino44f_pack_multi_kernel(const F44PackDesc* __restrict__ desc, int nlayers) {
    const long long vb = (long long)blockIdx.x * F44_PACK_BLOCKS;
    int lo = 0, hi = nlayers;
    while (hi - lo > 1) {
        const int mid = (lo + hi) >> 1;
        if (desc[mid].first_block <= vb) lo = mid; else hi = mid;
    }
    const F44PackDesc d = desc[lo];
    f44_pack_group(d.w, d.uf, d.ub, (int)d.Cout, (int)d.Cin, (size_t)d.nf, (size_t)d.nb,
                   (size_t)((vb - d.first_block) / F44_PACK_BLOCKS));
}

inline int rupf(int v, int m) { return (v + m - 1) / m * m; }

template <int LOGW>
__global__ __launch_bounds__(256) void wino44_fixup_kernel(F44Args a, int ntail) {
    using G = FGeo<LOGW, 0>;
    const size_t idx = (size_t)blockIdx.x * 256 + threadIdx.x;
    const int yy = idx & 3;
    const int tl = (idx >> 2) % FTT;
    const int col = (idx / (4 * FTT)) % FCO;
    const int j = idx / (4 * FTT * FCO);
    if (j >= ntail) return;
    const int ncot = a.CoutP / FCO;
    const int logical = a.nfull + j;
    const int cot = logical % ncot, wg = logical / ncot;
    const int s = wg / G::WPI, r0 = (wg % G::WPI) * 4 * G::TR;
    const int co = cot * FCO + col;
    if (co >= a.Cout) return;
    const int orow = r0 + 4 * G::t_row(tl) + yy, ocol = 4 * G::t_col(tl);
    const size_t o = ((size_t)s * a.Cout + co) * G::HW + (size_t)orow * G::W + ocol;
    float4 t[8];
#pragma unroll
    for (int p = 0; p < 8; ++p)
        t[p] = *reinterpret_cast<const float4*>(
            a.ws + ((((size_t)j * a.tail_split + min(p, a.tail_split - 1)) * FCO + col) * FTT + tl) * 16 + 4 * yy);
    float b = 0.f;
    if (a.bias) b += a.bias[co];
    if (a.vbias) b += a.vbias[(size_t)s * a.Cout + co];
    float4 q = make_float4(0.f, 0.f, 0.f, 0.f);
    if (a.res) q = *reinterpret_cast<const float4*>(a.res + o);
    float4 v = make_float4(0.f, 0.f, 0.f, 0.f);
#pragma unroll
    for (int p = 0; p < 8; ++p) {
        if (p < a.tail_split) { v.x += t[p].x; v.y += t[p].y; v.z += t[p].z; v.w += t[p].w; }
    }
    v.x += b; v.y += b; v.z += b; v.w += b;
    v.x += q.x; v.y += q.y; v.z += q.z; v.w += q.w;
    *reinterpret_cast<float4*>(a.y + o) = v;
}

inline int f44_groups(int S, int H, int W) { return S * ((H / 4) * (W / 4) / FTT); }

template <int LOGW, int MODE, bool RAGGED>
int launch_f44r(F44Args a, size_t ws_floats, hipStream_t st) {
    using G = FGeo<LOGW, MODE>;
    const int T = G::groups(a.S) * (a.CoutP / FCO);
    wino_tail_plan(T, a.CinP / FCK, &a.nfull, &a.tail_split);
    const int ntail = T - a.nfull;
    if ((size_t)ntail * a.tail_split * FCO * FTT * 16 > ws_floats || !a.ws) {
        a.nfull = T;
        a.tail_split = 1;
    }
    const int nt = T - a.nfull;
    a.npers = a.nfull < F44_PERSIST ? a.nfull : F44_PERSIST;
    hipLaunchKernelGGL((wino44_conv_kernel<LOGW, MODE, RAGGED>), dim3(a.npers + nt * a.tail_split), dim3(512), 0, st, a);
    if (nt > 0)
        hipLaunchKernelGGL((wino44_fixup_kernel<LOGW>), dim3((nt * FCO * FTT * 4 + 255) / 256), dim3(256), 0, st, a, nt);
    VF_RETURN_LAST_ERROR();
}

template <int LOGW, int MODE>
int launch_f44(F44Args a, size_t ws_floats, hipStream_t st) {
    return (a.Cin & (FCK - 1)) ? launch_f44r<LOGW, MODE, true>(a, ws_floats, st) : launch_f44r<LOGW, MODE, false>(a, ws_floats, st);
}

}

extern "C" {

int vf_wino44_pack_sizes(int Cout, int Cin, long* fwd_floats, long* bwd_floats) {
    *fwd_floats = (long)FNS * rupf(Cin, FCK) * rupf(Cout, FCO);
    *bwd_floats = (long)FNS * rupf(Cout, FCK) * rupf(Cin, FCO);
    return 0;
}

int vf_wino44_pack_weights(const float* w_oihw, float* u_fwd, float* u_bwd, int Cout, int Cin, void* stream) {
    const size_t nf = (size_t)FNS * rupf(Cin, FCK) * rupf(Cout, FCO);
    const size_t nb = u_bwd ? (size_t)FNS * rupf(Cout, FCK) * rupf(Cin, FCO) : 0;
    hipLaunchKernelGGL(wino44f_pack_kernel, dim3((unsigned)((nf + nb) / (FNS * FCO * FCK))), dim3(512), 0,
                       (hipStream_t)stream, w_oihw, u_fwd, u_bwd, Cout, Cin, nf, nb);
    VF_RETURN_LAST_ERROR();
}

int vf_wino44_pack_weights_multi(const void* desc, int nlayers, long total_blocks, void* stream) {
    if (nlayers <= 0 || total_blocks <= 0) return 0;
    hipLaunchKernelGGL(wino44f_pack_multi_kernel, dim3((unsigned)(total_blocks / F44_PACK_BLOCKS)), dim3(512), 0,
                       (hipStream_t)stream, (const F44PackDesc*)desc, nlayers);
    VF_RETURN_LAST_ERROR();
}

int vf_wino44_supported(int H, int W, int mode) {
    return (H == W && (W == 32 || W == 64) && (mode == 0 || mode == 2)) ? 1 : 0;
}

long vf_wino44_conv_ws_floats(int S, int Cin, int Cout, int H, int W) {
    const int T = f44_groups(S, H, W) * (rupf(Cout, FCO) / FCO);
    int nfull, split;
    wino_tail_plan(T, rupf(Cin, FCK) / FCK, &nfull, &split);
    return (long)(T - nfull) * split * FCO * FTT * 16;
}

int vf_wino44_conv_fill_pct(int S, int Cin, int Cout, int H, int W, int* tiles_out) {
    const int T = f44_groups(S, H, W) * (rupf(Cout, FCO) / FCO);
    const int nch = rupf(Cin, FCK) / FCK;
    int nfull, split;
    wino_tail_plan(T, nch, &nfull, &split, 0.0);
    if (tiles_out) *tiles_out = T;
    if (T <= 0) return 0;
    const double time = (nfull + WINO_SLOTS - 1) / WINO_SLOTS + (T > nfull ? wino_tail_time(T - nfull, split, nch, 0.0) : 0.0);
    return (int)(100.0 * T / WINO_SLOTS / time);
}

int vf_wino44_conv_fwd(const float* x, const float* u_packed, const float* bias, const float* view_bias,
                       const float* residual, float* y, float* ws, long ws_floats, int S, int Cin, int Cout, int H,
                       int W, int mode, void* stream) {
    if (S <= 0) return 0;
    if (!vf_wino44_supported(H, W, mode)) return (int)hipErrorInvalidValue;
    F44Args a;
    a.x = x; a.u = u_packed; a.bias = bias; a.vbias = view_bias; a.res = residual; a.y = y;
    a.S = S; a.Cin = Cin; a.Cout = Cout; a.CinP = rupf(Cin, FCK); a.CoutP = rupf(Cout, FCO);
    a.ws = ws;
    hipStream_t st = (hipStream_t)stream;
    const size_t nws = ws ? (size_t)ws_floats : 0;
    if (W == 32) return mode == 0 ? launch_f44<5, 0>(a, nws, st) : launch_f44<5, 2>(a, nws, st);
    return mode == 0 ? launch_f44<6, 0>(a, nws, st) : launch_f44<6, 2>(a, nws, st);
}

}

#ifdef VF_STAMPS44F
extern "C" void vf_debug_stamps44f(unsigned long long* out16, int reset) {
    if (out16) (void)hipMemcpyFromSymbol(out16, HIP_SYMBOL(g_stamps44f), 128);
    if (reset) { unsigned long long z[16] = {0}; (void)hipMemcpyToSymbol(HIP_SYMBOL(g_stamps44f), z, 128); }
}
#endif
```

### view_fusion_amd/ops/conv.py

```python
import ctypes

import torch

from .. import _lib, reducer
from .state import st
from .bf16x3 import _packed_b3, _use_b3
from .core import _MODES, _c, _call, _check, _launch, _ptr, _stream, _workspace
from .deferred import _defer_begin, _gout, _rowsum_get, _rowsum_put, _wred_ws
from .norm import group_norm
from .packing import _WINO_ABI, _conv_ws, _packed, _packed_small, _packed_wino, _wino_ws
from .policy import use_small_conv, use_winograd, use_winograd_wgrad, wino_kind


def _wgrad(entry, front, back, need, owners, keep, generic, flops, tag, strm):
    dev = keep[0].device
    ws = _wred_ws(dev, need) if (st.WRED_DEFER and (st.WRED_DEFER_GENERIC or not generic)
                                 and _defer_begin(owners, st.slab_sums)) else None
    if ws is None:
        ws = _workspace(dev, need)
        _launch("conv_wgrad", flops, entry, *front, _ptr(ws), ws.numel(), *back, strm, tag=tag)
        return False
    row, nblk = (ctypes.c_longlong * 9)(), ctypes.c_int(0)
    _launch("conv_wgrad", flops, entry + "_main", *front, _ptr(ws), ws.numel(), *back, ctypes.cast(row, ctypes.c_void_p),
            ctypes.cast(ctypes.pointer(nblk), ctypes.c_void_p), strm, tag=tag)
    st.slab_sums.add(dev, (list(row), nblk.value, (ws, *keep)))
    return True


def _conv_small(x, x2, weight, bias, view_bias, residual, S, Cin, Cout, H, W, KS, m):
    wd = weight.detach()
    _check(wd)
    y = torch.empty(S, Cout, H, W, device=x.device, dtype=torch.float32)
    wp = _packed_small(weight) if KS == 3 else None
    if wp is not None:
        _launch("conv_fwd", 2.0 * S * Cout * Cin * 9 * H * W, "vf_conv_small_gn", _ptr(x), None, 0, _ptr(wd), _ptr(bias),
                _ptr(view_bias), _ptr(residual), _ptr(y), S, Cin, Cout, H, W, 3, None, None, None, 0, 1e-5, 0, None, None,
                None, 0, 0, None, None, _ptr(wp), m, _stream(), tag=(Cin, Cout, H, KS, m))
        return y
    _launch("conv_fwd", 2.0 * S * Cout * Cin * KS * KS * H * W, "vf_conv_small", _ptr(x), _ptr(x2),
            x.shape[1] if x2 is not None else 0, _ptr(wd), _ptr(bias), _ptr(view_bias), _ptr(residual), _ptr(y), S, Cin,
            Cout, H, W, KS, m, _stream(), tag=(Cin, Cout, H, KS, m))
    return y


def _conv_small_res(x, layer, view_bias, res_layer, rx, rx2):
    S, Cin, H, W = x.shape
    Cout = layer.weight.shape[0]
    rC = res_layer.weight.shape[1]
    rC1 = rx.shape[1]
    assert rC1 + (rx2.shape[1] if rx2 is not None else 0) == rC and res_layer.weight.shape[0] == Cout
    wd, rwd = layer.weight.detach(), res_layer.weight.detach()
    _check(x, wd, rwd, layer.bias, view_bias, rx, rx2, res_layer.bias)
    y = torch.empty(S, Cout, H, W, device=x.device, dtype=torch.float32)
    wp = _packed_small(layer)
    if wp is not None:
        _launch("conv_fwd", 2.0 * S * Cout * (Cin * 9 + rC) * H * W, "vf_conv_small_gn", _ptr(x), None, 0, _ptr(wd),
                _ptr(layer.bias), _ptr(view_bias), None, _ptr(y), S, Cin, Cout, H, W, 3, None, None, None, 0, 1e-5, 0, None,
                _ptr(rx), _ptr(rx2), rC1, rC, _ptr(rwd), _ptr(res_layer.bias), _ptr(wp), 0, _stream(), tag=(Cin, Cout, H, 3, 0))
        return y
    _launch("conv_fwd", 2.0 * S * Cout * (Cin * 9 + rC) * H * W, "vf_conv_small_res", _ptr(x), _ptr(wd), _ptr(layer.bias),
            _ptr(view_bias), _ptr(y), S, Cin, Cout, H, W, _ptr(rx), _ptr(rx2), rC1, rC, _ptr(rwd), _ptr(res_layer.bias),
            _stream(), tag=(Cin, Cout, H, 3, 0))
    return y


class _Conv2dFn(torch.autograd.Function):

    @staticmethod
    def forward(ctx, x, weight, bias, view_bias, residual, layer, mode, training, twin, tap=False):
        _check(x, bias, view_bias, residual)
        ctx.tap = tap
        if tap:
            ctx.set_materialize_grads(False)
        S, Cin, Hi, Wi = x.shape
        Cout, _, KS, _ = weight.shape
        m = _MODES[mode]
        if m == 1 and (Hi % 2 or Wi % 2):
            raise ValueError(f"stride-2 conv on a {Hi}x{Wi} map: both sides must be even")
        H, W = (Hi // 2, Wi // 2) if m == 1 else ((Hi * 2, Wi * 2) if m == 2 else (Hi, Wi))
        y = torch.empty(S, Cout, H, W, device=x.device, dtype=torch.float32)
        flops = 2.0 * S * Cout * Cin * KS * KS * H * W
        nb = 4.0 * (x.numel() + y.numel() + weight.numel() + (residual.numel() if residual is not None else 0))
        wino = wino_kind(S, Cin, Cout, H, W, KS, m, train=bool(training))
        ctx.b3 = _use_b3(KS, m, H * W)
        if ctx.b3:
            wf, wb = _packed_b3(layer, force=training)
            _launch("conv_fwd", flops, "vf_conv1x1_bf16x3", _ptr(x), None, 0, ctypes.c_void_p(wf.data_ptr()), _ptr(bias),
                    _ptr(view_bias), _ptr(residual), _ptr(y), None, 0, S, Cin, Cout, H * W, _stream(),
                    tag=(Cin, Cout, H, KS, m))
        elif wino:
            wf, wb = _packed_wino(layer, training, wino)
            ws, nws = _wino_ws(x.device, S, Cin, Cout, H, W, wino)
            _launch("conv_fwd", flops, _WINO_ABI[wino][3], _ptr(x), _ptr(wf), _ptr(bias), _ptr(view_bias),
                    _ptr(residual), _ptr(y), _ptr(ws), nws, S, Cin, Cout, H, W, m, _stream(),
                    tag=(Cin, Cout, H, KS, m), nbytes=nb)
        else:
            wf, wb = _packed(layer, force=training)
            ws, nws = _conv_ws(x.device, S, Cin, Cout, H, W, KS)
            _launch("conv_fwd", flops, "vf_conv_fwd", _ptr(x), _ptr(wf), _ptr(bias), _ptr(view_bias),
                    _ptr(residual), _ptr(y), _ptr(ws), nws, S, Cin, Cout, H, W, KS, m, _stream(),
                    tag=(Cin, Cout, H, KS, m))
        ctx.flops, ctx.tag = flops, (Cin, Cout, H, KS, m)
        ctx.save_for_backward(x)
        ctx.wino = wino
        ctx.wb, ctx.m, ctx.KS, ctx.Cout = wb, m, KS, Cout
        ctx.has = (bias is not None, view_bias is not None, residual is not None)
        ctx.pw, ctx.pb, ctx.twin = weight, bias, (twin.bias if twin is not None else None)
        return (y, x.view_as(x)) if tap else y

    @staticmethod
    def backward(ctx, dy, dtap=None):
        (x,) = ctx.saved_tensors
        dy = _c(dy)
        dtap = _c(dtap) if dtap is not None else None
        S, Cin, Hi, Wi = x.shape
        _, Cout, H, W = dy.shape
        KS, m = ctx.KS, ctx.m
        strm = _stream()
        dx = dw = db = dvb = dres = None
        if ctx.needs_input_grad[0] and ctx.wino:
            dfull = torch.empty(S, Cin, H, W, device=x.device, dtype=torch.float32)
            ws, nws = _wino_ws(x.device, S, Cout, Cin, H, W, ctx.wino)
            _launch("conv_dgrad", ctx.flops, _WINO_ABI[ctx.wino][3], _ptr(dy), _ptr(ctx.wb), None, None, None,
                    _ptr(dfull), _ptr(ws), nws, S, Cout, Cin, H, W, 0, strm, tag=ctx.tag,
                    nbytes=4.0 * (dy.numel() + dfull.numel() + ctx.pw.numel()))
            if m == 2:
                dx = torch.empty_like(x)
                _call("vf_sumpool2", _ptr(dfull), _ptr(dx), dx.numel(), Wi, strm)
            else:
                dx = dfull
        elif ctx.needs_input_grad[0] and ctx.b3:
            dx = torch.empty_like(x)
            _launch("conv_dgrad", ctx.flops, "vf_conv1x1_bf16x3", _ptr(dy), None, 0, ctypes.c_void_p(ctx.wb.data_ptr()), None,
                    None, None, _ptr(dx), None, 0, S, Cout, Cin, H * W, strm, tag=ctx.tag)
        elif ctx.needs_input_grad[0]:
            if m == 0:
                dx = torch.empty_like(x)
                ws, nws = _conv_ws(x.device, S, Cout, Cin, H, W, KS)
                _launch("conv_dgrad", ctx.flops, "vf_conv_fwd", _ptr(dy), _ptr(ctx.wb), None, None, None, _ptr(dx),
                        _ptr(ws), nws, S, Cout, Cin, H, W, KS, 0, strm, tag=ctx.tag)
            elif m == 1:
                dx = torch.empty_like(x)
                _launch("conv_dgrad", ctx.flops, "vf_conv_fwd", _ptr(dy), _ptr(ctx.wb), None, None, _ptr(dtap), _ptr(dx),
                        None, 0, S, Cout, Cin, H, W, KS, 4, strm, tag=ctx.tag)
                dtap = None
            else:
                dup = torch.empty(S, Cin, H, W, device=x.device, dtype=torch.float32)
                _launch("conv_dgrad", ctx.flops, "vf_conv_fwd", _ptr(dy), _ptr(ctx.wb), None, None, None, _ptr(dup),
                        None, 0, S, Cout, Cin, H, W, KS, 0, strm, tag=ctx.tag)
                dx = torch.empty_like(x)
                _call("vf_sumpool2", _ptr(dup), _ptr(dx), dx.numel(), Wi, strm)
        hb, hv, hr = ctx.has
        want_b, want_v = hb and ctx.needs_input_grad[2], hv and ctx.needs_input_grad[3]
        arena = reducer.ACTIVE is not None
        hit = _rowsum_get(dy) if (want_b or want_v) else None
        if hit is not None:
            dvb, db = hit[1], (hit[2].view_as(hit[2]) if hit[2] is not None else None)
        db2 = None
        if ctx.needs_input_grad[1] and use_winograd_wgrad(S, Cin, Cout, H, W, KS, m):
            need = _lib.load().vf_wino_wgrad_ws_floats(S, Cin, Cout, H, W)
            dw = _gout(ctx.pw, Cout, Cin, 3, 3, like=x)
            db_here = None
            if want_b and db is None:
                db = db_here = _gout(ctx.pb, Cout, like=x)
                if hr:
                    db2 = _gout(ctx.twin, Cout, like=x)
            owners = [ctx.pw] + ([ctx.pb] if db_here is not None else []) + \
                     ([ctx.twin] if (db2 is not None and ctx.twin is not None) else [])
            if _wgrad("vf_wino_wgrad", (_ptr(x), _ptr(dy), _ptr(dw), _ptr(db_here), _ptr(db2)), (S, Cin, Cout, H, W, m),
                      need, owners, (dw, db_here, db2), False, ctx.flops, ctx.tag, strm):
                dw = dw.view_as(dw)
                if db_here is not None:
                    db = db_here.view_as(db_here)
        elif ctx.needs_input_grad[1]:
            need = _lib.load().vf_conv_wgrad_ws_floats(S, Cin, Cout, H, W, KS)
            dw = _gout(ctx.pw, Cout, Cin, KS, KS, like=x)
            if _wgrad("vf_conv_wgrad", (_ptr(x), _ptr(dy), _ptr(dw)), (S, Cin, Cout, H, W, KS, m), need, [ctx.pw],
                      (dw, None, None), True, ctx.flops, ctx.tag, strm):
                dw = dw.view_as(dw)
        if want_b or want_v:
            if (want_v and dvb is None) or (want_b and db is None and dvb is None):
                if Cout >= 192:
                    db_new = _gout(ctx.pb, Cout, like=x) if (want_b and db is None) else None
                    dvb = torch.empty(S, Cout, device=x.device, dtype=torch.float32) if want_v else None
                    _call("vf_bias_grad", _ptr(dy), _ptr(db_new), _ptr(dvb), S, Cout, H * W, strm)
                    db = db_new if db_new is not None else db
                else:
                    dvb = torch.empty(S, Cout, device=x.device, dtype=torch.float32)
                    _call("vf_rowsum", _ptr(dy), _ptr(dvb), S * Cout, H * W, strm)
            if want_b and db is None:
                db = _gout(ctx.pb, Cout, like=x)
                _call("vf_colsum", _ptr(dvb), _ptr(db), 1, S, Cout, strm)
            if hr and want_b:
                _rowsum_put(dy, dvb, db2 if (db2 is not None or arena) else db)
            if not want_b:
                db = None
            if not want_v:
                dvb = None
        if hr and ctx.needs_input_grad[4]:
            dres = dy
        if dtap is not None:
            dx = dtap if dx is None else dx + dtap
        return dx, dw, db, dvb, dres, None, None, None, None, None


class _Conv1x1CatFn(torch.autograd.Function):

    @staticmethod
    def forward(ctx, x1, x2, weight, bias, layer, training):
        _check(x1, x2, bias)
        S, C1, H, W = x1.shape
        Cout, Cin = weight.shape[0], weight.shape[1]
        y = torch.empty(S, Cout, H, W, device=x1.device, dtype=torch.float32)
        ctx.b3 = _use_b3(1, 0, H * W)
        if ctx.b3:
            wf, wb = _packed_b3(layer, force=training)
            _launch("conv_fwd", 2.0 * S * Cout * Cin * H * W, "vf_conv1x1_bf16x3", _ptr(x1), _ptr(x2), C1,
                    ctypes.c_void_p(wf.data_ptr()), _ptr(bias), None, None, _ptr(y), None, 0, S, Cin, Cout, H * W, _stream(),
                    tag=(Cin, Cout, H, 1, 0))
        else:
            wf, wb = _packed(layer, force=training)
            ws, nws = _conv_ws(x1.device, S, Cin, Cout, H, W, 1)
            _launch("conv_fwd", 2.0 * S * Cout * Cin * H * W, "vf_conv1x1_cat_fwd", _ptr(x1), _ptr(x2), C1, _ptr(wf),
                    _ptr(bias), _ptr(y), _ptr(ws), nws, S, Cin, Cout, H, W, _stream(), tag=(Cin, Cout, H, 1, 0))
        ctx.save_for_backward(x1, x2)
        ctx.wb, ctx.dims, ctx.has_bias = wb, (Cin, Cout), bias is not None
        ctx.pw, ctx.pb = weight, bias
        return y

    @staticmethod
    def backward(ctx, dy):
        x1, x2 = ctx.saved_tensors
        dy = _c(dy)
        S, C1, H, W = x1.shape
        Cin, Cout = ctx.dims
        strm = _stream()
        flops, tag = 2.0 * S * Cout * Cin * H * W, (Cin, Cout, H, 1, 0)
        dx1 = dx2 = dw = db = None
        if ctx.needs_input_grad[0] or ctx.needs_input_grad[1]:
            dx1, dx2 = torch.empty_like(x1), torch.empty_like(x2)
            if ctx.b3:
                _launch("conv_dgrad", flops, "vf_conv1x1_bf16x3", _ptr(dy), None, 0, ctypes.c_void_p(ctx.wb.data_ptr()), None,
                        None, None, _ptr(dx1), _ptr(dx2), C1, S, Cout, Cin, H * W, strm, tag=tag)
            else:
                _launch("conv_dgrad", flops, "vf_conv1x1_cat_dgrad", _ptr(dy), _ptr(ctx.wb), _ptr(dx1), _ptr(dx2), C1, S,
                        Cin, Cout, H, W, strm, tag=tag)
        if ctx.needs_input_grad[2]:
            need = _lib.load().vf_conv_wgrad_ws_floats(S, Cin, Cout, H, W, 1)
            dw = _gout(ctx.pw, Cout, Cin, 1, 1, like=x1)
            if _wgrad("vf_conv1x1_cat_wgrad", (_ptr(x1), _ptr(x2), C1, _ptr(dy), _ptr(dw)), (S, Cin, Cout, H, W), need,
                      [ctx.pw], (dw, None, None), True, flops, tag, strm):
                dw = dw.view_as(dw)
        if ctx.has_bias and ctx.needs_input_grad[3]:
            hit = _rowsum_get(dy)
            db = hit[2].view_as(hit[2]) if (hit is not None and hit[2] is not None) else None
            if db is None:
                dvb = hit[1] if hit is not None else None
                if dvb is None:
                    dvb = torch.empty(S, Cout, device=x1.device, dtype=torch.float32)
                    _call("vf_rowsum", _ptr(dy), _ptr(dvb), S * Cout, H * W, strm)
                db = _gout(ctx.pb, Cout, like=x1)
                _call("vf_colsum", _ptr(dvb), _ptr(db), 1, S, Cout, strm)
        return dx1, dx2, dw, db, None, None


def conv1x1_cat(x1, x2, layer):
    if not torch.is_grad_enabled():
        S, C1, H, W = x1.shape
        Cout, Cin = layer.weight.shape[0], layer.weight.shape[1]
        if use_small_conv(S, Cin, Cout, H, W, 1, 0):
            _check(x1, x2, layer.bias)
            return _conv_small(x1, x2, layer.weight, layer.bias, None, None, S, Cin, Cout, H, W, 1, 0)
    training = torch.is_grad_enabled() and layer.weight.requires_grad
    return _Conv1x1CatFn.apply(x1, x2, layer.weight, layer.bias, layer, training)


def conv2d(x, layer, view_bias=None, residual=None, mode="same", twin=None, tap=False, res_fold=None):
    if not torch.is_grad_enabled():
        S, Cin, Hi, Wi = x.shape
        Cout, _, KS, _ = layer.weight.shape
        m = _MODES[mode]
        H, W = (Hi // 2, Wi // 2) if m == 1 else ((Hi * 2, Wi * 2) if m == 2 else (Hi, Wi))
        if res_fold is not None:
            assert residual is None and not tap
            return _conv_small_res(x, layer, view_bias, *res_fold)
        if use_small_conv(S, Cin, Cout, H, W, KS, m):
            _check(x, layer.bias, view_bias, residual)
            y = _conv_small(x, None, layer.weight, layer.bias, view_bias, residual, S, Cin, Cout, H, W, KS, m)
            return (y, x) if tap else y
    assert res_fold is None
    training = torch.is_grad_enabled() and layer.weight.requires_grad
    if tap and torch.is_grad_enabled():
        return _Conv2dFn.apply(x, layer.weight, layer.bias, view_bias, residual, layer, mode, training, twin, True)
    y = _Conv2dFn.apply(x, layer.weight, layer.bias, view_bias, residual, layer, mode, training, twin)
    return (y, x) if tap else y


def conv2d_gn(x, layer, gn, groups, silu, view_bias=None, residual=None, mode="same", want_y=False, res_fold=None):
    S, Cin, Hi, Wi = x.shape
    Cout, _, KS, _ = layer.weight.shape
    m = _MODES[mode]
    H, W = (Hi // 2, Wi // 2) if m == 1 else ((Hi * 2, Wi * 2) if m == 2 else (Hi, Wi))
    lib = _lib.load()
    fused = (not torch.is_grad_enabled() and not use_winograd(S, Cin, Cout, H, W, KS, m, False) and not _use_b3(KS, m, H * W)
             and not use_small_conv(S, Cin, Cout, H, W, KS, m)
             and lib.vf_conv_fwd_ws_floats(S, Cin, Cout, H, W, KS) > 0)
    if (st.WINO_GN_FUSION and not fused and not torch.is_grad_enabled() and res_fold is None
            and m in (0, 2) and KS == 3 and wino_kind(S, Cin, Cout, H, W, KS, m, False) == 1
            and lib.vf_wino_conv_gn_fusable(S, Cin, Cout, H, W, m, groups)):
        _check(x, layer.bias, view_bias, residual, gn.weight, gn.bias)
        y = torch.empty(S, Cout, H, W, device=x.device, dtype=torch.float32) if want_y else None
        a = torch.empty(S, Cout, H, W, device=x.device, dtype=torch.float32)
        wf, _ = _packed_wino(layer, False, 1)
        ws, nws = _wino_ws(x.device, S, Cin, Cout, H, W, 1)
        _launch("conv_fwd", 2.0 * S * Cout * Cin * 9 * H * W, "vf_wino_conv_fwd_gn", _ptr(x), _ptr(wf), _ptr(layer.bias),
                _ptr(view_bias), _ptr(residual), _ptr(y), int(want_y), _ptr(gn.weight), _ptr(gn.bias), _ptr(a), groups, 1e-5,
                int(silu), _ptr(ws), nws, S, Cin, Cout, H, W, m, _stream(), tag=(Cin, Cout, H, KS, m))
        return y, a
    if not fused:
        y = conv2d(x, layer, view_bias=view_bias, residual=residual, mode=mode, res_fold=res_fold)
        return y, group_norm(y, gn.weight, gn.bias, groups, silu)
    assert res_fold is None
    _check(x, layer.bias, view_bias, residual, gn.weight, gn.bias)
    y = torch.empty(S, Cout, H, W, device=x.device, dtype=torch.float32)
    a = torch.empty_like(y)
    stats = torch.empty(2 * S * groups, device=x.device, dtype=torch.float32)
    wf, _ = _packed(layer, force=False)
    ws, nws = _conv_ws(x.device, S, Cin, Cout, H, W, KS)
    _call("vf_conv_fwd_gn", _ptr(x), _ptr(wf), _ptr(layer.bias), _ptr(view_bias), _ptr(residual), _ptr(y), int(want_y),
              _ptr(gn.weight), _ptr(gn.bias), _ptr(a), _ptr(stats), groups, 1e-5, int(silu), _ptr(ws), nws, S, Cin, Cout,
              H, W, KS, m, _stream())
    return (y if want_y else None), a
```

### view_fusion_amd/ops/norm.py

```python
import torch

from .. import _lib, reducer
from .state import st
from .core import _c, _check, _launch, _ptr, _stream
from .deferred import _colsum, _rowsum_put


def _gn_forward(x, gamma, beta, groups, silu):
    _check(x, gamma, beta)
    S, C, H, W = x.shape
    y = torch.empty_like(x)
    mean = torch.empty(S * groups, device=x.device, dtype=torch.float32)
    rstd = torch.empty_like(mean)
    _launch("gn_fwd", 0.0, "vf_gn_fwd", _ptr(x), _ptr(gamma), _ptr(beta), _ptr(y), _ptr(mean), _ptr(rstd), S, C, H * W,
            groups, 1e-5, int(silu), _stream(), nbytes=8.0 * x.numel())
    return y, mean, rstd


def _gb_grads(parts, gb):
    _, S, C = parts.shape
    dgb = reducer.ACTIVE.slot_pair(*gb) if reducer.ACTIVE is not None else None
    if dgb is None:
        dgb = torch.empty(2, C, device=parts.device, dtype=torch.float32)
    _colsum(parts, dgb, 2, S, C, gb)
    return dgb[0], dgb[1]


def _gn_backward(ctx, dy, addend, addend2=None):
    x, gamma, beta, mean, rstd = ctx.saved_tensors
    dy = _c(dy)
    S, C, H, W = x.shape
    dx = torch.empty_like(x)
    parts = torch.empty(2, S, C, device=x.device, dtype=torch.float32)
    rowsum = None
    if addend is None and st.ROWSUM_FUSION and _lib.load().vf_gn_bwd_emits_rowsum(C, H * W, ctx.groups):
        rowsum = torch.empty(S, C, device=x.device, dtype=torch.float32)
    if addend is None and addend2 is not None:
        addend, addend2 = addend2, None
    _launch("gn_bwd", 0.0, "vf_gn_cat_bwd", _ptr(x), None, C, _ptr(gamma), _ptr(beta), _ptr(mean), _ptr(rstd), _ptr(dy),
            _ptr(addend), _ptr(addend2), _ptr(dx), None, _ptr(parts[0]), _ptr(parts[1]), _ptr(rowsum), S, C, H * W,
            ctx.groups, ctx.silu, _stream(),
            nbytes=4.0 * x.numel() * (3 + (addend is not None) + (addend2 is not None)))
    if rowsum is not None:
        _rowsum_put(dx, rowsum, None)
    return (dx, *_gb_grads(parts, ctx.gb))


class _GroupNormFn(torch.autograd.Function):
    @staticmethod
    def forward(ctx, x, gamma, beta, groups, silu):
        y, mean, rstd = _gn_forward(x, gamma, beta, groups, silu)
        ctx.save_for_backward(x, gamma, beta, mean, rstd)
        ctx.groups, ctx.silu, ctx.gb = groups, int(silu), (gamma, beta)
        return y

    @staticmethod
    def backward(ctx, dy):
        return (*_gn_backward(ctx, dy, None), None, None)


class _GroupNormSkipFn(torch.autograd.Function):

    @staticmethod
    def forward(ctx, x, gamma, beta, groups, silu):
        y, mean, rstd = _gn_forward(x, gamma, beta, groups, silu)
        ctx.save_for_backward(x, gamma, beta, mean, rstd)
        ctx.groups, ctx.silu, ctx.gb = groups, int(silu), (gamma, beta)
        ctx.set_materialize_grads(False)
        return y, x.view_as(x), x.view_as(x)

    @staticmethod
    def backward(ctx, dy, dskip, dtap):
        return (*_gn_backward(ctx, dy, None if dskip is None else _c(dskip), None if dtap is None else _c(dtap)),
                None, None)


class _GroupNormCatSkipFn(torch.autograd.Function):

    @staticmethod
    def forward(ctx, x1, x2, gamma, beta, groups, silu):
        _check(x1, x2, gamma, beta)
        S, C1, H, W = x1.shape
        C = C1 + x2.shape[1]
        y = torch.empty(S, C, H, W, device=x1.device, dtype=torch.float32)
        mean = torch.empty(S * groups, device=x1.device, dtype=torch.float32)
        rstd = torch.empty_like(mean)
        _launch("gn_fwd", 0.0, "vf_gn_cat_fwd", _ptr(x1), _ptr(x2), C1, _ptr(gamma), _ptr(beta), _ptr(y), _ptr(mean),
                _ptr(rstd), S, C, H * W, groups, 1e-5, int(silu), _stream(), nbytes=8.0 * y.numel())
        ctx.save_for_backward(x1, x2, gamma, beta, mean, rstd)
        ctx.groups, ctx.silu, ctx.gb = groups, int(silu), (gamma, beta)
        return y, x1.view_as(x1), x2.view_as(x2)

    @staticmethod
    def backward(ctx, dy, d1, d2):
        x1, x2, gamma, beta, mean, rstd = ctx.saved_tensors
        dy = _c(dy)
        S, C1, H, W = x1.shape
        C = C1 + x2.shape[1]
        if (d1 is None) != (d2 is None):
            d1 = torch.zeros_like(x1) if d1 is None else d1
            d2 = torch.zeros_like(x2) if d2 is None else d2
        d1 = None if d1 is None else _c(d1)
        d2 = None if d2 is None else _c(d2)
        dx1, dx2 = torch.empty_like(x1), torch.empty_like(x2)
        parts = torch.empty(2, S, C, device=x1.device, dtype=torch.float32)
        _launch("gn_bwd", 0.0, "vf_gn_cat_bwd", _ptr(x1), _ptr(x2), C1, _ptr(gamma), _ptr(beta), _ptr(mean), _ptr(rstd),
                _ptr(dy), _ptr(d1), _ptr(d2), _ptr(dx1), _ptr(dx2), _ptr(parts[0]), _ptr(parts[1]), None, S, C, H * W,
                ctx.groups, ctx.silu, _stream(), nbytes=4.0 * dy.numel() * (3 + (d1 is not None)))
        return (dx1, dx2, *_gb_grads(parts, ctx.gb), None, None)


def cat_fusable(C1, C, HW, groups):
    return C1 % 64 == 0 and bool(_lib.load().vf_gn_bwd_emits_rowsum(C, HW, groups))


def group_norm_cat_skip(x1, x2, weight, bias, groups, silu):
    return _GroupNormCatSkipFn.apply(x1, x2, weight, bias, groups, silu)


def group_norm(x, weight, bias, groups, silu):
    return _GroupNormFn.apply(x, weight, bias, groups, silu)


def group_norm_skip(x, weight, bias, groups, silu, tap=False):
    if not (torch.is_grad_enabled() and x.requires_grad):
        y = _GroupNormFn.apply(x, weight, bias, groups, silu)
        return (y, x, x) if tap else (y, x)
    out = _GroupNormSkipFn.apply(x, weight, bias, groups, silu)
    return out if tap else out[:2]
```

### view_fusion_amd/ops/state.py

```python
import os


class State:
    def __init__(self):
        self.KERNEL_LOG = None
        self._KIND_OVERRIDE = None
        self.WINOGRAD = True
        self.FORCE_WINOGRAD = False
        self.WINO_MIN_TILES = int(os.environ.get("VF_WINO_MIN_TILES", 30))
        self.WINO_MIN_FILL = int(os.environ.get("VF_WINO_MIN_FILL", 65))
        self.WINO_WGRAD_MIN_TILES = int(os.environ.get("VF_WINO_WGRAD_MIN_TILES", 256))
        self.WINOGRAD_WGRAD = True
        self.WINOGRAD44 = os.environ.get("VF_WINO44", "1") == "1"
        self.FORCE_WINOGRAD44 = False
        self.SMALL_CONV = os.environ.get("VF_SMALL_CONV", "1") == "1"
        self.SMALL_CONV_MAX_WGS = (int(os.environ.get("VF_SMALL_CONV_MAX_WGS1", 1024)),
                          int(os.environ.get("VF_SMALL_CONV_MAX_WGS3", 512)))
        self.SMALL_CONV_MAX_CIN3 = int(os.environ.get("VF_SMALL_CONV_MAX_CIN3", 256))
        self.SMALL_CONV_MAX_S3 = int(os.environ.get("VF_SMALL_CONV_MAX_S3", 1))
        self.SMALL_PACK = os.environ.get("VF_SMALL_PACK", "1") == "1"
        self.RES_FOLD = os.environ.get("VF_RES_FOLD", "1") == "1"
        self.WINO_GN_FUSION = os.environ.get("VF_WINO_GN", "1") == "1"
        self.ATTN_DSCORE = os.environ.get("VF_ATTN_DSCORE", "1") != "0"
        self.ATTN_DVDK = os.environ.get("VF_ATTN_DVDK", "1") != "0"
        self.BF16X3 = os.environ.get("VF_BF16X3") == "1"
        self.ROWSUM_FUSION = True
        self.COLSUM_DEFER = True
        self.WRED_DEFER = os.environ.get("VF_WRED_DEFER", "1") != "0"
        self.WRED_DEFER_GENERIC = os.environ.get("VF_WRED_DEFER_GENERIC", "1") != "0"
        self.col_sums = None
        self.slab_sums = None
        self._PENDING_TASK = None
        self._WRED_ARENA = {}
        self._ws = {}
        self._WINO_KIND_CACHE = {}
        self._TA_DESC = {}
        self._TA_GDST = {}
        self._VC_CACHE = []


st = State()
```

### view_fusion_amd/unet.py

```python
import torch
from torch import nn


class _Named(nn.Module):

    def __init__(self, **children):
        super().__init__()
        for name, mod in children.items():
            self.add_module(name, mod)

    def __getitem__(self, name):
        return self._modules[name]


def _norm_act_conv(cin, cout, groups):
    return _Named(block=_Named(**{"0": nn.GroupNorm(groups, cin), "3": nn.Conv2d(cin, cout, 3, padding=1)}))


class _ResBlock(nn.Module):
    def __init__(self, cin, cout, emb_dim, groups, dropout=0):
        super().__init__()
        self.noise_func = _Named(noise_func=_Named(**{"0": nn.Linear(emb_dim, cout)}))
        self.block1 = _norm_act_conv(cin, cout, groups)
        self.block2 = _norm_act_conv(cout, cout, groups)
        self.res_conv = nn.Conv2d(cin, cout, 1) if cin != cout else nn.Identity()
        self.groups = groups
        self.dropout = float(dropout)

    def _drop(self, a, draws):
        if self.dropout == 0 or not self.training:
            return a
        from . import ops
        return ops.dropout(a, self.dropout, next(draws) if draws is not None else None)

    def _forward_inference(self, x, e, skip, a_in, next_gn):
        from . import ops
        b1, b2 = self.block1["block"], self.block2["block"]
        conv1, conv2 = b1["3"], b2["3"]
        S, _, H, W = x.shape
        Cout = conv2.weight.shape[0]
        if skip is not None:
            C1, C = x.shape[1], x.shape[1] + skip.shape[1]
            if not (isinstance(self.res_conv, nn.Conv2d) and ops.cat_fusable(C1, C, x.shape[2] * x.shape[3], self.groups)):
                x, skip = ops.concat_channels(x, skip), None
        fold = (self.res_conv, x, skip) if ops.can_fold_residual(S, Cout, H, W, self.res_conv) else None
        res = None
        if skip is not None:
            if fold is None:
                res = ops.conv1x1_cat(x, skip, self.res_conv)
            a, _, _ = ops.group_norm_cat_skip(x, skip, b1["0"].weight, b1["0"].bias, self.groups, silu=True)
        else:
            if isinstance(self.res_conv, nn.Identity):
                res = x
            elif fold is None:
                res = ops.conv2d(x, self.res_conv)
            a = a_in if a_in is not None else ops.group_norm(x, b1["0"].weight, b1["0"].bias, self.groups, silu=True)
        _, a2 = ops.conv2d_gn(a, conv1, b2["0"], self.groups, True, view_bias=e)
        if next_gn is None:
            return ops.conv2d(a2, conv2, residual=res, res_fold=fold), None
        return ops.conv2d_gn(a2, conv2, next_gn[0], self.groups, next_gn[1], residual=res, want_y=True, res_fold=fold)

    def forward(self, x, e, skip=None, tap=False, draws=None):
        from . import ops
        b1, b2 = self.block1["block"], self.block2["block"]
        if skip is not None:
            C1, C = x.shape[1], x.shape[1] + skip.shape[1]
            if not (isinstance(self.res_conv, nn.Conv2d) and ops.cat_fusable(C1, C, x.shape[2] * x.shape[3], self.groups)):
                x, skip = ops.concat_channels(x, skip), None
        if skip is not None:
            a, x1, x2 = ops.group_norm_cat_skip(x, skip, b1["0"].weight, b1["0"].bias, self.groups, silu=True)
            h = ops.conv2d(a, b1["3"], view_bias=e)
            a = self._drop(ops.group_norm(h, b2["0"].weight, b2["0"].bias, self.groups, silu=True), draws)
            return ops.conv2d(a, b2["3"], residual=ops.conv1x1_cat(x1, x2, self.res_conv), twin=self.res_conv)
        a, xs, xt = ops.group_norm_skip(x, b1["0"].weight, b1["0"].bias, self.groups, silu=True, tap=True)
        h = ops.conv2d(a, b1["3"], view_bias=e)
        a = self._drop(ops.group_norm(h, b2["0"].weight, b2["0"].bias, self.groups, silu=True), draws)
        twin = None if isinstance(self.res_conv, nn.Identity) else self.res_conv
        skip = xs if twin is None else ops.conv2d(xs, twin)
        y = ops.conv2d(a, b2["3"], residual=skip, twin=twin)
        return (y, xt) if tap else y


class _SelfAttention(nn.Module):
    def __init__(self, ch, groups):
        super().__init__()
        self.norm = nn.GroupNorm(groups, ch)
        self.qkv = nn.Conv2d(ch, ch * 3, 1, bias=False)
        self.out = nn.Conv2d(ch, ch, 1)
        self.groups = groups

    def forward(self, x, n=None):
        from . import ops
        if n is None:
            n, xs = ops.group_norm_skip(x, self.norm.weight, self.norm.bias, self.groups, silu=False)
        else:
            xs = x
        qkv = ops.conv2d(n, self.qkv)
        o = ops.attention(qkv)
        return ops.conv2d(o, self.out, residual=xs)


class _ResAttnBlock(nn.Module):
    def __init__(self, cin, cout, emb_dim, groups, with_attn, dropout=0):
        super().__init__()
        self.with_attn = with_attn
        self.res_block = _ResBlock(cin, cout, emb_dim, groups, dropout)
        if with_attn:
            self.attn = _SelfAttention(cout, groups)

    def forward_inference(self, x, e, skip=None, a_in=None, next_gn=None):
        if self.with_attn:
            y, n = self.res_block._forward_inference(x, e, skip, a_in, (self.attn.norm, False))
            return self.attn(y, n), None
        return self.res_block._forward_inference(x, e, skip, a_in, next_gn)

    def forward(self, x, e, skip=None, tap=False, draws=None):
        xt = None
        if tap:
            x, xt = self.res_block(x, e, skip, tap=True, draws=draws)
        else:
            x = self.res_block(x, e, skip, draws=draws)
        x = self.attn(x) if self.with_attn else x
        return (x, xt) if tap else x


class _Resample(nn.Module):
    def __init__(self, ch, up):
        super().__init__()
        self.up = up
        self.conv = nn.Conv2d(ch, ch, 3, padding=1) if up else nn.Conv2d(ch, ch, 3, 2, 1)

    def forward(self, x, tap=False):
        from . import ops
        return ops.conv2d(x, self.conv, mode="up2" if self.up else "down2", tap=tap)


class UNet(nn.Module):
    def __init__(self, in_channel=6, out_channel=3, inner_channel=32, norm_groups=32,
                 channel_mults=(1, 2, 4, 8, 8), attn_res=(8,), res_blocks=3, dropout=0,
                 with_noise_level_emb=True, image_size=128):
        super().__init__()
        if not with_noise_level_emb:
            raise TypeError("with_noise_level_emb=False: the reference UNet cannot be constructed without the "
                            "noise-level embedding (nn.Linear(None, C) in FeatureWiseAffine, model/unet.py:165)")
        if not 0 <= dropout < 1:
            raise ValueError(f"dropout probability has to be in [0, 1), got {dropout}")
        self.inner_channel = inner_channel
        self.noise_level_mlp = _Named(**{"0": nn.Linear(inner_channel, inner_channel * 4),
                                         "2": nn.Linear(inner_channel * 4, inner_channel)})
        emb = inner_channel
        ch = inner_channel
        skips = [ch]
        res = image_size
        downs = [nn.Conv2d(in_channel, inner_channel, 3, padding=1)]
        last = len(channel_mults) - 1
        for lvl, mult in enumerate(channel_mults):
            width = inner_channel * mult
            for _ in range(res_blocks):
                downs.append(_ResAttnBlock(ch, width, emb, norm_groups, res in attn_res, dropout))
                ch = width
                skips.append(ch)
            if lvl != last:
                downs.append(_Resample(ch, up=False))
                skips.append(ch)
                res //= 2
        self.downs = nn.ModuleList(downs)
        self.mid = nn.ModuleList([_ResAttnBlock(ch, ch, emb, norm_groups, True, dropout),
                                  _ResAttnBlock(ch, ch, emb, norm_groups, False, dropout)])
        ups = []
        for lvl in reversed(range(len(channel_mults))):
            width = inner_channel * channel_mults[lvl]
            for _ in range(res_blocks + 1):
                ups.append(_ResAttnBlock(ch + skips.pop(), width, emb, norm_groups, res in attn_res, dropout))
                ch = width
            if lvl > 0:
                ups.append(_Resample(ch, up=True))
                res *= 2
        self.ups = nn.ModuleList(ups)
        self.final_conv = _norm_act_conv(ch, out_channel if out_channel is not None else in_channel,
                                         norm_groups)
        self.norm_groups = norm_groups
        self._annotate_geometry(image_size)

    def _annotate_geometry(self, image_size):
        attn_levels = set()

        def mark(conv, lvl, mode="same"):
            object.__setattr__(conv, "_vf_geom", (lvl, mode))

        def mark_block(blk, lvl):
            rb = blk.res_block
            mark(rb.block1["block"]["3"], lvl)
            mark(rb.block2["block"]["3"], lvl)
            if isinstance(rb.res_conv, nn.Conv2d):
                mark(rb.res_conv, lvl)
            if blk.with_attn:
                attn_levels.add(lvl)
                mark(blk.attn.qkv, lvl)
                mark(blk.attn.out, lvl)

        lvl = 0
        for layer in self.downs:
            if isinstance(layer, _ResAttnBlock):
                mark_block(layer, lvl)
            elif isinstance(layer, _Resample):
                lvl += 1
                mark(layer.conv, lvl, "down2")
            else:
                mark(layer, lvl)
        for layer in self.mid:
            mark_block(layer, lvl)
        for layer in self.ups:
            if isinstance(layer, _ResAttnBlock):
                mark_block(layer, lvl)
            else:
                lvl -= 1
                mark(layer.conv, lvl, "up2")
        mark(self.final_conv["block"]["3"], lvl)
        object.__setattr__(self, "_vf_image_size", image_size)
        object.__setattr__(self, "_vf_depth", sum(isinstance(m, _Resample) and not m.up for m in self.downs))
        object.__setattr__(self, "_vf_attn_levels", tuple(sorted(attn_levels)))

    def check_input_size(self, H, W):
        f = 1 << self._vf_depth
        if H <= 0 or W <= 0 or H % f or W % f:
            raise ValueError(f"input size {H}x{W}: both sides must be positive multiples of {f} "
                             f"(2**(len(channel_mults) - 1)) for the encoder / decoder maps to match")
        if (H * W) % 4:
            raise ValueError(f"input size {H}x{W}: H*W must be a multiple of 4")

    def _affine_layers(self):
        lst = getattr(self, "_vf_affine", None)
        if lst is None:
            lst = [m.res_block.noise_func["noise_func"]["0"] for m in list(self.downs) + list(self.mid) + list(self.ups)
                   if isinstance(m, _ResAttnBlock)]
            object.__setattr__(self, "_vf_affine", lst)
        return lst

    def _has_dropout(self):
        return any(isinstance(m, _ResBlock) and m.dropout > 0 for m in self.modules())

    def _forward_inference(self, x, es):
        from . import ops

        def gn1_of(layer):
            if not isinstance(layer, _ResAttnBlock):
                return None
            return (layer.res_block.block1["block"]["0"], True)

        feats, a_next = [], None
        downs = list(self.downs)
        for i, layer in enumerate(downs):
            if isinstance(layer, _ResAttnBlock):
                nxt = downs[i + 1] if i + 1 < len(downs) else self.mid[0]
                x, a_next = layer.forward_inference(x, next(es), a_in=a_next, next_gn=gn1_of(nxt))
            elif isinstance(layer, _Resample):
                x, a_next = layer(x), None
            else:
                x, a_next = ops.conv2d(x, layer), None
            feats.append(x)
        x, a_next = self.mid[0].forward_inference(x, next(es), a_in=a_next, next_gn=gn1_of(self.mid[1]))
        x, a_next = self.mid[1].forward_inference(x, next(es), a_in=a_next, next_gn=None)
        ups = list(self.ups)
        fc = self.final_conv["block"]
        for i, layer in enumerate(ups):
            if isinstance(layer, _ResAttnBlock):
                last = i + 1 == len(ups)
                x, a_next = layer.forward_inference(x, next(es), skip=feats.pop(), next_gn=(fc["0"], True) if last else None)
            else:
                x, a_next = layer(x), None
        a = a_next if a_next is not None else ops.group_norm(x, fc["0"].weight, fc["0"].bias, self.norm_groups, silu=True)
        return ops.conv2d(a, fc["3"])

    def forward(self, x, angle, time, dropout_u=None):
        from . import ops
        draws = iter(dropout_u) if dropout_u is not None else None
        ops._check(x)
        self.check_input_size(x.shape[2], x.shape[3])
        if torch.is_grad_enabled() and self.final_conv["block"]["3"].weight.requires_grad:
            ops.pack_all(self, x.shape[0], tuple(x.shape[2:]))
        mlp = self.noise_level_mlp
        inference = not torch.is_grad_enabled() and not (self.training and self._has_dropout())

        def embed():
            pe = ops.sincos_embedding(time, angle, self.inner_channel)
            emb = ops.linear(pe, mlp["0"].weight, mlp["0"].bias)
            emb = ops.linear(ops.swish(emb), mlp["2"].weight, mlp["2"].bias)
            return ops.time_affine_all(emb, self._affine_layers())

        if inference:
            return self._forward_inference(x, iter(embed()))
        es = iter(embed())

        feats = []
        for layer in self.downs:
            if isinstance(layer, _ResAttnBlock):
                x, xin = layer(x, next(es), tap=True, draws=draws)
                if feats:
                    feats[-1] = xin
            elif isinstance(layer, _Resample):
                x, xin = layer(x, tap=True)
                if feats:
                    feats[-1] = xin
            else:
                x = ops.conv2d(x, layer)
            feats.append(x)
        first = True
        for layer in self.mid:
            if first:
                x, feats[-1] = layer(x, next(es), tap=True, draws=draws)
                first = False
            else:
                x = layer(x, next(es), draws=draws)
        for layer in self.ups:
            if isinstance(layer, _ResAttnBlock):
                x = layer(x, next(es), feats.pop(), draws=draws)
            else:
                x = layer(x)
        fc = self.final_conv["block"]
        a = ops.group_norm(x, fc["0"].weight, fc["0"].bias, self.norm_groups, silu=True)
        return ops.conv2d(a, fc["3"])
```

Before: 3264 view denoise-steps/s (UNet fwd+bwd per stacked view, incl. compose/MSE/Adam).

## Fold split-K Winograd conv reduction tail into following GroupNorm kernels

Adds 'tail' variants of the Winograd conv forward that leave split-K partial sums in workspace. The following GroupNorm forward and backward kernels then reduce those partials, add bias, view-bias and residual, and write the finished conv output. This removes a separate reduction or epilogue pass and a round trip of the conv output through memory. In exchange it adds index-mapping complexity, a tail handoff between conv and norm tracked in Python via tensor marks, and extra partial reads inside the GN kernels.

```diff
diff --git a/include/vf_hip.h b/include/vf_hip.h
--- a/include/vf_hip.h
+++ b/include/vf_hip.h
@@ -16,6 +16,14 @@
                   const float* rstd, const float* dy, const float* addend, const float* addend2, float* dx, float* dx2,
                   float* dgamma_part, float* dbeta_part, float* dx_rowsum, int S, int C, int HW, int groups, int silu,
                   void* stream);
+int vf_gn_tail_supported(int C, int HW, int groups, int kind, int bwd);
+int vf_gn_fwd_tail(float* x, const float* gamma, const float* beta, float* y, float* mean, float* rstd, int S, int C,
+                   int HW, int groups, float eps, int silu, const float* ws, int kind, int nfull, int split,
+                   const float* bias, const float* view_bias, const float* residual, void* stream);
+int vf_gn_cat_bwd_tail(const float* x, const float* x2, int C1, const float* gamma, const float* beta, const float* mean,
+                       const float* rstd, const float* dy, const float* addend, const float* addend2, float* dx, float* dx2,
+                       float* dgamma_part, float* dbeta_part, float* dx_rowsum, int S, int C, int HW, int groups, int silu,
+                       const float* ws, int kind, int nfull, int split, void* stream);
 int vf_rowsum(const float* x, float* out , int rows, int len, void* stream);
 int vf_bias_grad(const float* dy, float* db, float* dvb, int S, int C, int HW, void* stream);
 int vf_colsum(const float* part , float* out , int batch, int S, int C,
@@ -82,6 +90,9 @@
 int vf_wino_conv_fwd(const float* x, const float* u_packed, const float* bias, const float* view_bias,
                      const float* residual, float* y, float* ws, long ws_floats, int S, int Cin, int Cout, int H,
                      int W, int mode, void* stream);
+int vf_wino_conv_fwd_tail(const float* x, const float* u_packed, const float* bias, const float* view_bias,
+                          const float* residual, float* y, float* ws, long ws_floats, int S, int Cin, int Cout, int H,
+                          int W, int mode, int* plan_out, void* stream);
 int vf_wino_conv_gn_fusable(int S, int Cin, int Cout, int H, int W, int mode, int groups);
 int vf_wino_conv_fwd_gn(const float* x, const float* u_packed, const float* bias , const float* view_bias ,
                         const float* residual , float* y, int store_y, const float* gn_gamma, const float* gn_beta,
@@ -97,6 +108,9 @@
 int vf_wino44_conv_fwd(const float* x, const float* u_packed, const float* bias, const float* view_bias,
                        const float* residual, float* y, float* ws, long ws_floats, int S, int Cin, int Cout, int H,
                        int W, int mode, void* stream);
+int vf_wino44_conv_fwd_tail(const float* x, const float* u_packed, const float* bias, const float* view_bias,
+                            const float* residual, float* y, float* ws, long ws_floats, int S, int Cin, int Cout, int H,
+                            int W, int mode, int* plan_out, void* stream);
 int vf_wino_wgrad_supported(int H, int W, int mode);
 long vf_wino_wgrad_ws_floats(int S, int Cin, int Cout, int H, int W);
 int vf_wino_wgrad(const float* x, const float* dy, float* dw_oihw, float* db, float* db2, float* ws, long ws_floats,
diff --git a/view_fusion_amd/_lib.py b/view_fusion_amd/_lib.py
--- a/view_fusion_amd/_lib.py
+++ b/view_fusion_amd/_lib.py
@@ -19,6 +19,9 @@
     "vf_gn_bwd_emits_rowsum": [_I, _I, _I],
     "vf_gn_cat_fwd": [_P, _P, _I, _P, _P, _P, _P, _P, _I, _I, _I, _I, _F, _I, _P],
     "vf_gn_cat_bwd": [_P, _P, _I, _P, _P, _P, _P, _P, _P, _P, _P, _P, _P, _P, _P, _I, _I, _I, _I, _I, _P],
+    "vf_gn_tail_supported": [_I, _I, _I, _I, _I],
+    "vf_gn_fwd_tail": [_P, _P, _P, _P, _P, _P, _I, _I, _I, _I, _F, _I, _P, _I, _I, _I, _P, _P, _P, _P],
+    "vf_gn_cat_bwd_tail": [_P, _P, _I, _P, _P, _P, _P, _P, _P, _P, _P, _P, _P, _P, _P, _I, _I, _I, _I, _I, _P, _I, _I, _I, _P],
     "vf_conv1x1_cat_fwd": [_P, _P, _I, _P, _P, _P, _P, _L, _I, _I, _I, _I, _I, _P],
     "vf_conv1x1_cat_dgrad": [_P, _P, _P, _P, _I, _I, _I, _I, _I, _I, _P],
     "vf_conv1x1_cat_wgrad": [_P, _P, _I, _P, _P, _P, _L, _I, _I, _I, _I, _I, _P],
@@ -45,6 +48,7 @@
     "vf_wino_conv_ws_floats": [_I, _I, _I, _I, _I],
     "vf_wino_conv_fill_pct": [_I, _I, _I, _I, _I, ctypes.POINTER(_I)],
     "vf_wino_conv_fwd": [_P, _P, _P, _P, _P, _P, _P, _L, _I, _I, _I, _I, _I, _I, _P],
+    "vf_wino_conv_fwd_tail": [_P, _P, _P, _P, _P, _P, _P, _L, _I, _I, _I, _I, _I, _I, ctypes.POINTER(_I), _P],
     "vf_wino_conv_gn_fusable": [_I, _I, _I, _I, _I, _I, _I],
     "vf_wino_conv_fwd_gn": [_P, _P, _P, _P, _P, _P, _I, _P, _P, _P, _I, _F, _I, _P, _L, _I, _I, _I, _I, _I, _I, _P],
     "vf_wino44_supported": [_I, _I, _I],
@@ -54,6 +58,7 @@
     "vf_wino44_conv_ws_floats": [_I, _I, _I, _I, _I],
     "vf_wino44_conv_fill_pct": [_I, _I, _I, _I, _I, ctypes.POINTER(_I)],
     "vf_wino44_conv_fwd": [_P, _P, _P, _P, _P, _P, _P, _L, _I, _I, _I, _I, _I, _I, _P],
+    "vf_wino44_conv_fwd_tail": [_P, _P, _P, _P, _P, _P, _P, _L, _I, _I, _I, _I, _I, _I, ctypes.POINTER(_I), _P],
     "vf_wino_wgrad_ws_floats": [_I, _I, _I, _I, _I],
     "vf_wino_wgrad_supported": [_I, _I, _I],
     "vf_wino_wgrad": [_P, _P, _P, _P, _P, _P, _L, _I, _I, _I, _I, _I, _I, _P],
diff --git a/view_fusion_amd/csrc/common.h b/view_fusion_amd/csrc/common.h
--- a/view_fusion_amd/csrc/common.h
+++ b/view_fusion_amd/csrc/common.h
@@ -50,6 +50,34 @@
 #endif
 }
 __device__ __forceinline__ float silu_f(float z) { return z * sigmoid_f(z); }
+
+struct VfTail {
+    const float* ws;
+    const float* bias;
+    const float* vbias;
+    const float* res;
+    int kind, nfull, split, ncot;
+};
+
+__device__ __forceinline__ int vf_tail_locate(const VfTail& t, int logw, int s, int c, int i4, int* off) {
+    const int row = i4 >> (logw - 2), col4 = i4 & ((1 << (logw - 2)) - 1);
+    const int lth = t.kind == 2 ? 2 : 1;
+    int wg, tl;
+    if (logw == 3) {
+        wg = s >> 2;
+        tl = ((s & 3) << 3) + ((row >> 1) << 1) + col4;
+    } else {
+        const int ltr = 5 - (logw - 2);
+        const int lwpi = logw - lth - ltr;
+        const int trow = row >> lth;
+        wg = (s << lwpi) + (trow >> ltr);
+        tl = ((trow & ((1 << ltr) - 1)) << (logw - 2)) + col4;
+    }
+    const int yy = row & ((1 << lth) - 1);
+    *off = ((((c & 63) << 5) + tl) << (lth + 2)) + 4 * yy;
+    return wg * t.ncot + (c >> 6) - t.nfull;
+}
+__device__ __forceinline__ size_t vf_tail_part_floats(const VfTail& t) { return (size_t)64 * 32 * (t.kind == 2 ? 16 : 8); }
 
 __device__ __forceinline__ unsigned xcd_remap(unsigned bid, unsigned nblk) {
     const unsigned q = nblk >> 3, r = nblk & 7u;
diff --git a/view_fusion_amd/csrc/norm.hip b/view_fusion_amd/csrc/norm.hip
--- a/view_fusion_amd/csrc/norm.hip
+++ b/view_fusion_amd/csrc/norm.hip
@@ -15,12 +15,46 @@
 }
 
 template <int NV, int NT>
+__device__ __forceinline__ void tail_finish(const VfTail& t, const int (&tj)[NV], const int (&toff)[NV], float4 (&v)[NV],
+                                            const float4* safe, float4* fin4, size_t base4, int n4, int s, int C, int c0,
+                                            int hwsh) {
+    const size_t pf = vf_tail_part_floats(t);
+#pragma unroll
+    for (int i = 0; i < NV; ++i)
+        if (tj[i] >= 0) { v[i].x = 0.f + v[i].x; v[i].y = 0.f + v[i].y; v[i].z = 0.f + v[i].z; v[i].w = 0.f + v[i].w; }
+    for (int p = 1; p < t.split; ++p) {
+        float4 q[NV];
+#pragma unroll
+        for (int i = 0; i < NV; ++i)
+            q[i] = *(tj[i] >= 0 ? reinterpret_cast<const float4*>(t.ws + ((size_t)tj[i] * t.split + p) * pf + toff[i]) : safe);
+#pragma unroll
+        for (int i = 0; i < NV; ++i)
+            if (tj[i] >= 0) { v[i].x += q[i].x; v[i].y += q[i].y; v[i].z += q[i].z; v[i].w += q[i].w; }
+    }
+#pragma unroll
+    for (int i = 0; i < NV; ++i) {
+        if (tj[i] < 0) continue;
+        const int idx = (int)threadIdx.x + i * NT, idc = min(idx, n4 - 1);
+        const int c = c0 + (idc >> hwsh);
+        float b = 0.f;
+        if (t.bias) b += t.bias[c];
+        if (t.vbias) b += t.vbias[(size_t)s * C + c];
+        float4 r = make_float4(0.f, 0.f, 0.f, 0.f);
+        if (t.res) r = reinterpret_cast<const float4*>(t.res)[base4 + idc];
+        v[i].x += b; v[i].y += b; v[i].z += b; v[i].w += b;
+        v[i].x += r.x; v[i].y += r.y; v[i].z += r.z; v[i].w += r.w;
+        if (fin4 && idx < n4) fin4[base4 + idc] = v[i];
+    }
+}
+
+template <int NV, int NT, bool TAIL = false>
 __global__ __launch_bounds__(NT) void gn_fwd_kernel(const float* __restrict__ x, const float* __restrict__ x2, int C1,
                                                     const float* __restrict__ gamma,
                                                     const float* __restrict__ beta,
                                                     float* __restrict__ y, float* __restrict__ mean_out,
                                                     float* __restrict__ rstd_out, int C, int HW, int cpg,
-                                                    float eps, int silu) {
+                                                    float eps, int silu, VfTail tail = VfTail(),
+                                                    float* xfin = nullptr) {
     __shared__ float red[NT / 64];
     const int G = C / cpg;
     const int sg = blockIdx.x;
@@ -33,7 +67,21 @@
 
     float4 v[NV];
     float gam[NV], bet[NV];
-    if (x2) {
+    int tj[TAIL ? NV : 1], toff[TAIL ? NV : 1];
+    if constexpr (TAIL) {
+        const int logw = (hwsh + 2) >> 1;
+        int any = 0;
+#pragma unroll
+        for (int i = 0; i < NV; ++i) {
+            const int idc = min((int)threadIdx.x + i * NT, n4 - 1);
+            tj[i] = vf_tail_locate(tail, logw, s, g * cpg + (idc >> hwsh), idc & hwmask, &toff[i]);
+            any |= tj[i] >= 0;
+            v[i] = *(tj[i] >= 0 ? reinterpret_cast<const float4*>(tail.ws + (size_t)tj[i] * tail.split * vf_tail_part_floats(tail) + toff[i])
+                                : x4 + idc);
+        }
+        if (__syncthreads_or(any))
+            tail_finish<NV, NT>(tail, tj, toff, v, reinterpret_cast<const float4*>(tail.ws), reinterpret_cast<float4*>(xfin), base >> 2, n4, s, C, g * cpg, hwsh);
+    } else if (x2) {
 #pragma unroll
         for (int i = 0; i < NV; ++i) {
             const int idc = min((int)threadIdx.x + i * NT, n4 - 1);
@@ -187,7 +235,7 @@
 }
 
 
-template <int NV, int NT, int SEG = 64>
+template <int NV, int NT, int SEG = 64, bool TAIL = false>
 __global__ __launch_bounds__(NT) void gn_bwd_fused_kernel(const float* __restrict__ x, const float* __restrict__ x2,
                                                           int C1, const float* __restrict__ dy,
                                                           const float* __restrict__ gamma,
@@ -200,7 +248,7 @@
                                                           float* __restrict__ dgamma_part,
                                                           float* __restrict__ dbeta_part,
                                                           float* __restrict__ dx_rowsum, int C, int HW, int cpg,
-                                                          int silu) {
+                                                          int silu, VfTail tail = VfTail()) {
     constexpr int NWV = NT / 64;
     extern __shared__ float part[];
     const int G = C / cpg;
@@ -224,15 +272,29 @@
         for (int i = 0; i < NV; ++i) {
             const int idc = min((int)threadIdx.x + i * NT, n4 - 1);
             xv[i] = cat_ptr(x, x2, C1, C, s, g * cpg + (idc >> hwsh), HW)[idc & hwmask];
-            dv[i] = d4[idc];
+            if constexpr (!TAIL) dv[i] = d4[idc];
         }
     } else {
 #pragma unroll
         for (int i = 0; i < NV; ++i) {
             const int idc = min((int)threadIdx.x + i * NT, n4 - 1);
             xv[i] = ld_nt(x4 + idc);
-            dv[i] = ld_nt(d4 + idc);
-        }
+            if constexpr (!TAIL) dv[i] = ld_nt(d4 + idc);
+        }
+    }
+    if constexpr (TAIL) {
+        const int logw = (hwsh + 2) >> 1;
+        int tj[NV], toff[NV], any = 0;
+#pragma unroll
+        for (int i = 0; i < NV; ++i) {
+            const int idc = min((int)threadIdx.x + i * NT, n4 - 1);
+            tj[i] = vf_tail_locate(tail, logw, s, g * cpg + (idc >> hwsh), idc & hwmask, &toff[i]);
+            any |= tj[i] >= 0;
+            dv[i] = *(tj[i] >= 0 ? reinterpret_cast<const float4*>(tail.ws + (size_t)tj[i] * tail.split * vf_tail_part_floats(tail) + toff[i])
+                                 : d4 + idc);
+        }
+        if (__syncthreads_or(any))
+            tail_finish<NV, NT>(tail, tj, toff, dv, reinterpret_cast<const float4*>(tail.ws), nullptr, base >> 2, n4, s, C, g * cpg, hwsh);
     }
 #pragma unroll
     for (int i = 0; i < NV; ++i) {
@@ -484,9 +546,62 @@
     VF_RETURN_LAST_ERROR();
 }
 
+template <int NV, int NT>
+int launch_gn_fwd_tail(float* x, const float* gamma, const float* beta, float* y, float* mean, float* rstd, int S, int C,
+                       int HW, int cpg, float eps, int silu, const VfTail& tail, hipStream_t st) {
+    hipLaunchKernelGGL((gn_fwd_kernel<NV, NT, true>), dim3(S * (C / cpg)), dim3(NT), 0, st, x, nullptr, C, gamma, beta, y,
+                       mean, rstd, C, HW, cpg, eps, silu, tail, x);
+    VF_RETURN_LAST_ERROR();
+}
+
+inline bool tail_map_ok(int HW, int kind) {
+    if (kind == 1) return HW == 64 || HW == 256 || HW == 1024 || HW == 4096;
+    return kind == 2 && (HW == 1024 || HW == 4096);
+}
+inline VfTail make_tail(const float* ws, int kind, int nfull, int split, const float* bias, const float* vbias,
+                        const float* res, int C) {
+    VfTail t;
+    t.ws = ws; t.bias = bias; t.vbias = vbias; t.res = res;
+    t.kind = kind; t.nfull = nfull; t.split = split; t.ncot = (C + 63) / 64;
+    return t;
+}
+
 }
 
 extern "C" {
+
+int vf_gn_fwd(const float*, const float*, const float*, float*, float*, float*, int, int, int, int, float, int, void*);
+int vf_gn_bwd_emits_rowsum(int C, int HW, int groups);
+int vf_gn_cat_bwd(const float*, const float*, int, const float*, const float*, const float*, const float*, const float*,
+                  const float*, const float*, float*, float*, float*, float*, float*, int, int, int, int, int, void*);
+
+int vf_gn_tail_supported(int C, int HW, int groups, int kind, int bwd) {
+    if (groups <= 0 || C <= 0 || C % groups != 0 || !tail_map_ok(HW, kind)) return 0;
+    const long n4g = (long)(C / groups) * HW / 4;
+    if (n4g > 4096) return 0;
+    return bwd ? vf_gn_bwd_emits_rowsum(C, HW, groups) : 1;
+}
+
+int vf_gn_fwd_tail(float* x, const float* gamma, const float* beta, float* y, float* mean, float* rstd, int S, int C,
+                   int HW, int groups, float eps, int silu, const float* ws, int kind, int nfull, int split,
+                   const float* bias, const float* view_bias, const float* residual, void* stream) {
+    if (S <= 0) return 0;
+    if (split < 2 || !ws) return vf_gn_fwd(x, gamma, beta, y, mean, rstd, S, C, HW, groups, eps, silu, stream);
+    if (!vf_gn_tail_supported(C, HW, groups, kind, 0) || split > 8 || nfull < 0) return (int)hipErrorInvalidValue;
+    hipStream_t st = (hipStream_t)stream;
+    const int cpg = C / groups;
+    const long n4 = (long)cpg * HW / 4;
+    const VfTail tail = make_tail(ws, kind, nfull, split, bias, view_bias, residual, C);
+#define VF_GN(NV, NT) return launch_gn_fwd_tail<NV, NT>(x, gamma, beta, y, mean, rstd, S, C, HW, cpg, eps, silu, tail, st)
+    if (n4 <= 64) VF_GN(1, 64);
+    if (n4 <= 256) VF_GN(1, 256);
+    if (n4 <= 512) VF_GN(2, 256);
+    if (n4 <= 1024) VF_GN(4, 256);
+    if (n4 <= 2048) VF_GN(8, 256);
+    if (n4 <= 3072) VF_GN(12, 256);
+    VF_GN(16, 256);
+#undef VF_GN
+}
 
 int vf_gn_cat_fwd(const float* x, const float* x2, int C1, const float* gamma, const float* beta, float* y, float* mean,
                   float* rstd, int S, int C, int HW, int groups, float eps, int silu, void* stream) {
@@ -524,6 +639,40 @@
     if (groups <= 0 || C % groups != 0 || HW < 4 || (HW & (HW - 1))) return 0;
     const long n4g = (long)(C / groups) * HW / 4;
     return ((HW >= 256 && n4g <= 8192) || (HW == 64 && n4g <= 1024)) ? 1 : 0;
+}
+
+int vf_gn_cat_bwd_tail(const float* x, const float* x2, int C1, const float* gamma, const float* beta, const float* mean,
+                       const float* rstd, const float* dy, const float* addend, const float* addend2, float* dx, float* dx2,
+                       float* dgamma_part, float* dbeta_part, float* dx_rowsum, int S, int C, int HW, int groups, int silu,
+                       const float* ws, int kind, int nfull, int split, void* stream) {
+    hipStream_t st = (hipStream_t)stream;
+    if (S <= 0) return 0;
+    if (split < 2 || !ws)
+        return vf_gn_cat_bwd(x, x2, C1, gamma, beta, mean, rstd, dy, addend, addend2, dx, dx2, dgamma_part, dbeta_part,
+                             dx_rowsum, S, C, HW, groups, silu, stream);
+    if (!vf_gn_tail_supported(C, HW, groups, kind, 1) || split > 8 || nfull < 0) return (int)hipErrorInvalidValue;
+    if (x2 && (C1 <= 0 || C1 >= C || !dx2 || (addend && !addend2))) return (int)hipErrorInvalidValue;
+    const int cpg = C / groups;
+    const long n4g = (long)cpg * HW / 4;
+    const VfTail tail = make_tail(ws, kind, nfull, split, nullptr, nullptr, nullptr, C);
+#define VF_GNBT(NV, NT, SEG)                                                                               \
+    {                                                                                                      \
+        hipLaunchKernelGGL((gn_bwd_fused_kernel<NV, NT, SEG, true>), dim3(S * groups), dim3(NT), (NT / 64) * cpg * 3 * 4, st, \
+                           x, x2, C1, dy, gamma, beta, mean, rstd, addend, addend2, dx, dx2, dgamma_part, dbeta_part, \
+                           dx_rowsum, C, HW, cpg, silu, tail);                                             \
+        VF_RETURN_LAST_ERROR();                                                                            \
+    }
+    if (HW == 64) {
+        if (n4g <= 256) VF_GNBT(1, 256, 16)
+        if (n4g <= 512) VF_GNBT(2, 256, 16)
+        VF_GNBT(4, 256, 16)
+    }
+    if (n4g <= 256) VF_GNBT(1, 256, 64)
+    if (n4g <= 512) VF_GNBT(2, 256, 64)
+    if (n4g <= 1024) VF_GNBT(4, 256, 64)
+    if (n4g <= 2048) VF_GNBT(8, 256, 64)
+    VF_GNBT(8, 512, 64)
+#undef VF_GNBT
 }
 
 int vf_gn_cat_bwd(const float* x, const float* x2, int C1, const float* gamma, const float* beta, const float* mean,
diff --git a/view_fusion_amd/csrc/winograd24.hip b/view_fusion_amd/csrc/winograd24.hip
--- a/view_fusion_amd/csrc/winograd24.hip
+++ b/view_fusion_amd/csrc/winograd24.hip
@@ -707,7 +707,7 @@
 }
 
 template <int LOGW, int MODE>
-int launch_wino(WinoArgs a, size_t ws_floats, hipStream_t st, const WinoGn& gn = WinoGn()) {
+int launch_wino(WinoArgs a, size_t ws_floats, hipStream_t st, const WinoGn& gn = WinoGn(), int* plan_out = nullptr) {
     using G = WGeo<LOGW, MODE>;
     const int T = G::groups(a.S) * (a.CoutP / WTCO);
     wino_tail_plan(T, a.CinP / WCK, &a.nfull, &a.tail_split);
@@ -734,7 +734,10 @@
             VF_RETURN_LAST_ERROR();
         }
     }
-    if (nt > 0)
+    if (plan_out) {
+        plan_out[0] = a.nfull;
+        plan_out[1] = a.tail_split;
+    } else if (nt > 0)
         hipLaunchKernelGGL((wino_fixup_kernel<LOGW>), dim3((nt * WTCO * WTT + 255) / 256), dim3(256), 0, st, a, nt);
     VF_RETURN_LAST_ERROR();
 }
@@ -786,9 +789,10 @@
     return (int)(100.0 * T / WINO_SLOTS / time);
 }
 
-int vf_wino_conv_fwd(const float* x, const float* u_packed, const float* bias, const float* view_bias,
-                     const float* residual, float* y, float* ws, long ws_floats, int S, int Cin, int Cout, int H,
-                     int W, int mode, void* stream) {
+static int wino_conv_fwd(const float* x, const float* u_packed, const float* bias, const float* view_bias,
+                         const float* residual, float* y, float* ws, long ws_floats, int S, int Cin, int Cout, int H,
+                         int W, int mode, int* plan_out, void* stream) {
+    if (plan_out) { plan_out[0] = 0; plan_out[1] = 1; }
     if (S <= 0) return 0;
     if (!vf_wino_supported(H, W, mode)) return (int)hipErrorInvalidValue;
     WinoArgs a;
@@ -797,10 +801,24 @@
     a.ws = ws;
     hipStream_t st = (hipStream_t)stream;
     const size_t nws = ws ? (size_t)ws_floats : 0;
-    if (W == 8) return mode == 0 ? launch_wino<3, 0>(a, nws, st) : launch_wino<3, 2>(a, nws, st);
-    if (W == 16) return mode == 0 ? launch_wino<4, 0>(a, nws, st) : launch_wino<4, 2>(a, nws, st);
-    if (W == 32) return mode == 0 ? launch_wino<5, 0>(a, nws, st) : launch_wino<5, 2>(a, nws, st);
-    return mode == 0 ? launch_wino<6, 0>(a, nws, st) : launch_wino<6, 2>(a, nws, st);
+    const WinoGn no_gn;
+    if (W == 8) return mode == 0 ? launch_wino<3, 0>(a, nws, st, no_gn, plan_out) : launch_wino<3, 2>(a, nws, st, no_gn, plan_out);
+    if (W == 16) return mode == 0 ? launch_wino<4, 0>(a, nws, st, no_gn, plan_out) : launch_wino<4, 2>(a, nws, st, no_gn, plan_out);
+    if (W == 32) return mode == 0 ? launch_wino<5, 0>(a, nws, st, no_gn, plan_out) : launch_wino<5, 2>(a, nws, st, no_gn, plan_out);
+    return mode == 0 ? launch_wino<6, 0>(a, nws, st, no_gn, plan_out) : launch_wino<6, 2>(a, nws, st, no_gn, plan_out);
+}
+
+int vf_wino_conv_fwd(const float* x, const float* u_packed, const float* bias, const float* view_bias,
+                     const float* residual, float* y, float* ws, long ws_floats, int S, int Cin, int Cout, int H,
+                     int W, int mode, void* stream) {
+    return wino_conv_fwd(x, u_packed, bias, view_bias, residual, y, ws, ws_floats, S, Cin, Cout, H, W, mode, nullptr, stream);
+}
+
+int vf_wino_conv_fwd_tail(const float* x, const float* u_packed, const float* bias, const float* view_bias,
+                          const float* residual, float* y, float* ws, long ws_floats, int S, int Cin, int Cout, int H,
+                          int W, int mode, int* plan_out, void* stream) {
+    if (!plan_out) return (int)hipErrorInvalidValue;
+    return wino_conv_fwd(x, u_packed, bias, view_bias, residual, y, ws, ws_floats, S, Cin, Cout, H, W, mode, plan_out, stream);
 }
 
 int vf_wino_conv_gn_fusable(int S, int Cin, int Cout, int H, int W, int mode, int groups) {
diff --git a/view_fusion_amd/csrc/winograd44f.hip b/view_fusion_amd/csrc/winograd44f.hip
--- a/view_fusion_amd/csrc/winograd44f.hip
+++ b/view_fusion_amd/csrc/winograd44f.hip
@@ -621,7 +621,7 @@
 inline int f44_groups(int S, int H, int W) { return S * ((H / 4) * (W / 4) / FTT); }
 
 template <int LOGW, int MODE, bool RAGGED>
-int launch_f44r(F44Args a, size_t ws_floats, hipStream_t st) {
+int launch_f44r(F44Args a, size_t ws_floats, hipStream_t st, int* plan_out) {
     using G = FGeo<LOGW, MODE>;
     const int T = G::groups(a.S) * (a.CoutP / FCO);
     wino_tail_plan(T, a.CinP / FCK, &a.nfull, &a.tail_split);
@@ -633,14 +633,18 @@
     const int nt = T - a.nfull;
     a.npers = a.nfull < F44_PERSIST ? a.nfull : F44_PERSIST;
     hipLaunchKernelGGL((wino44_conv_kernel<LOGW, MODE, RAGGED>), dim3(a.npers + nt * a.tail_split), dim3(512), 0, st, a);
-    if (nt > 0)
+    if (plan_out) {
+        plan_out[0] = a.nfull;
+        plan_out[1] = a.tail_split;
+    } else if (nt > 0)
         hipLaunchKernelGGL((wino44_fixup_kernel<LOGW>), dim3((nt * FCO * FTT * 4 + 255) / 256), dim3(256), 0, st, a, nt);
     VF_RETURN_LAST_ERROR();
 }
 
 template <int LOGW, int MODE>
-int launch_f44(F44Args a, size_t ws_floats, hipStream_t st) {
-    return (a.Cin & (FCK - 1)) ? launch_f44r<LOGW, MODE, true>(a, ws_floats, st) : launch_f44r<LOGW, MODE, false>(a, ws_floats, st);
+int launch_f44(F44Args a, size_t ws_floats, hipStream_t st, int* plan_out) {
+    return (a.Cin & (FCK - 1)) ? launch_f44r<LOGW, MODE, true>(a, ws_floats, st, plan_out)
+                               : launch_f44r<LOGW, MODE, false>(a, ws_floats, st, plan_out);
 }
 
 }
@@ -690,9 +694,10 @@
     return (int)(100.0 * T / WINO_SLOTS / time);
 }
 
-int vf_wino44_conv_fwd(const float* x, const float* u_packed, const float* bias, const float* view_bias,
-                       const float* residual, float* y, float* ws, long ws_floats, int S, int Cin, int Cout, int H,
-                       int W, int mode, void* stream) {
+static int wino44_conv_fwd(const float* x, const float* u_packed, const float* bias, const float* view_bias,
+                           const float* residual, float* y, float* ws, long ws_floats, int S, int Cin, int Cout, int H,
+                           int W, int mode, int* plan_out, void* stream) {
+    if (plan_out) { plan_out[0] = 0; plan_out[1] = 1; }
     if (S <= 0) return 0;
     if (!vf_wino44_supported(H, W, mode)) return (int)hipErrorInvalidValue;
     F44Args a;
@@ -701,8 +706,21 @@
     a.ws = ws;
     hipStream_t st = (hipStream_t)stream;
     const size_t nws = ws ? (size_t)ws_floats : 0;
-    if (W == 32) return mode == 0 ? launch_f44<5, 0>(a, nws, st) : launch_f44<5, 2>(a, nws, st);
-    return mode == 0 ? launch_f44<6, 0>(a, nws, st) : launch_f44<6, 2>(a, nws, st);
+    if (W == 32) return mode == 0 ? launch_f44<5, 0>(a, nws, st, plan_out) : launch_f44<5, 2>(a, nws, st, plan_out);
+    return mode == 0 ? launch_f44<6, 0>(a, nws, st, plan_out) : launch_f44<6, 2>(a, nws, st, plan_out);
+}
+
+int vf_wino44_conv_fwd(const float* x, const float* u_packed, const float* bias, const float* view_bias,
+                       const float* residual, float* y, float* ws, long ws_floats, int S, int Cin, int Cout, int H,
+                       int W, int mode, void* stream) {
+    return wino44_conv_fwd(x, u_packed, bias, view_bias, residual, y, ws, ws_floats, S, Cin, Cout, H, W, mode, nullptr, stream);
+}
+
+int vf_wino44_conv_fwd_tail(const float* x, const float* u_packed, const float* bias, const float* view_bias,
+                            const float* residual, float* y, float* ws, long ws_floats, int S, int Cin, int Cout, int H,
+                            int W, int mode, int* plan_out, void* stream) {
+    if (!plan_out) return (int)hipErrorInvalidValue;
+    return wino44_conv_fwd(x, u_packed, bias, view_bias, residual, y, ws, ws_floats, S, Cin, Cout, H, W, mode, plan_out, stream);
 }
 
 }
diff --git a/view_fusion_amd/ops/conv.py b/view_fusion_amd/ops/conv.py
--- a/view_fusion_amd/ops/conv.py
+++ b/view_fusion_amd/ops/conv.py
@@ -25,6 +25,25 @@
             ctypes.cast(ctypes.pointer(nblk), ctypes.c_void_p), strm, tag=tag)
     st.slab_sums.add(dev, (list(row), nblk.value, (ws, *keep)))
     return True
+
+
+def _wino_launch(kind_name, flops, wino, gn_groups, bwd, x, wpk, bias, view_bias, residual, y, S, Cin, Cout, H, W, m, strm,
+                 tag, nb):
+    lib = _lib.load()
+    entry = _WINO_ABI[wino][3]
+    defer = (st.GN_FIXUP and gn_groups > 0 and lib.vf_gn_tail_supported(Cout, H * W, gn_groups, wino, int(bwd))
+             and getattr(lib, _WINO_ABI[wino][4])(S, Cin, Cout, H, W) > 0)
+    if not defer:
+        ws, nws = _wino_ws(x.device, S, Cin, Cout, H, W, wino)
+        _launch(kind_name, flops, entry, _ptr(x), _ptr(wpk), _ptr(bias), _ptr(view_bias), _ptr(residual), _ptr(y), _ptr(ws),
+                nws, S, Cin, Cout, H, W, m, strm, tag=tag, nbytes=nb)
+        return
+    ws = torch.empty(getattr(lib, _WINO_ABI[wino][4])(S, Cin, Cout, H, W), device=x.device, dtype=torch.float32)
+    plan = (ctypes.c_int * 2)()
+    _launch(kind_name, flops, entry + "_tail", _ptr(x), _ptr(wpk), _ptr(bias), _ptr(view_bias), _ptr(residual), _ptr(y),
+            _ptr(ws), ws.numel(), S, Cin, Cout, H, W, m, plan, strm, tag=tag, nbytes=nb)
+    if plan[1] >= 2:
+        st._TAILS[y.data_ptr()] = (y, ws, wino, plan[0], plan[1], bias, view_bias, residual)
 
 
 def _conv_small(x, x2, weight, bias, view_bias, residual, S, Cin, Cout, H, W, KS, m):
@@ -67,9 +86,10 @@
 class _Conv2dFn(torch.autograd.Function):
 
     @staticmethod
-    def forward(ctx, x, weight, bias, view_bias, residual, layer, mode, training, twin, tap=False):
+    def forward(ctx, x, weight, bias, view_bias, residual, layer, mode, training, twin, tap=False, gn_next=0, from_gn=0):
         _check(x, bias, view_bias, residual)
         ctx.tap = tap
+        ctx.from_gn = from_gn
         if tap:
             ctx.set_materialize_grads(False)
         S, Cin, Hi, Wi = x.shape
@@ -90,10 +110,8 @@
                     tag=(Cin, Cout, H, KS, m))
         elif wino:
             wf, wb = _packed_wino(layer, training, wino)
-            ws, nws = _wino_ws(x.device, S, Cin, Cout, H, W, wino)
-            _launch("conv_fwd", flops, _WINO_ABI[wino][3], _ptr(x), _ptr(wf), _ptr(bias), _ptr(view_bias),
-                    _ptr(residual), _ptr(y), _ptr(ws), nws, S, Cin, Cout, H, W, m, _stream(),
-                    tag=(Cin, Cout, H, KS, m), nbytes=nb)
+            _wino_launch("conv_fwd", flops, wino, gn_next, False, x, wf, bias, view_bias, residual, y, S, Cin, Cout, H, W,
+                         m, _stream(), (Cin, Cout, H, KS, m), nb)
         else:
             wf, wb = _packed(layer, force=training)
             ws, nws = _conv_ws(x.device, S, Cin, Cout, H, W, KS)
@@ -120,10 +138,9 @@
         dx = dw = db = dvb = dres = None
         if ctx.needs_input_grad[0] and ctx.wino:
             dfull = torch.empty(S, Cin, H, W, device=x.device, dtype=torch.float32)
-            ws, nws = _wino_ws(x.device, S, Cout, Cin, H, W, ctx.wino)
-            _launch("conv_dgrad", ctx.flops, _WINO_ABI[ctx.wino][3], _ptr(dy), _ptr(ctx.wb), None, None, None,
-                    _ptr(dfull), _ptr(ws), nws, S, Cout, Cin, H, W, 0, strm, tag=ctx.tag,
-                    nbytes=4.0 * (dy.numel() + dfull.numel() + ctx.pw.numel()))
+            _wino_launch("conv_dgrad", ctx.flops, ctx.wino, ctx.from_gn if (m == 0 and dtap is None) else 0, True, dy, ctx.wb,
+                         None, None, None, dfull, S, Cout, Cin, H, W, 0, strm, ctx.tag,
+                         4.0 * (dy.numel() + dfull.numel() + ctx.pw.numel()))
             if m == 2:
                 dx = torch.empty_like(x)
                 _call("vf_sumpool2", _ptr(dfull), _ptr(dx), dx.numel(), Wi, strm)
@@ -201,7 +218,7 @@
             dres = dy
         if dtap is not None:
             dx = dtap if dx is None else dx + dtap
-        return dx, dw, db, dvb, dres, None, None, None, None, None
+        return dx, dw, db, dvb, dres, None, None, None, None, None, None, None
 
 
 class _Conv1x1CatFn(torch.autograd.Function):
@@ -275,7 +292,7 @@
     return _Conv1x1CatFn.apply(x1, x2, layer.weight, layer.bias, layer, training)
 
 
-def conv2d(x, layer, view_bias=None, residual=None, mode="same", twin=None, tap=False, res_fold=None):
+def conv2d(x, layer, view_bias=None, residual=None, mode="same", twin=None, tap=False, res_fold=None, gn_next=0):
     if not torch.is_grad_enabled():
         S, Cin, Hi, Wi = x.shape
         Cout, _, KS, _ = layer.weight.shape
@@ -291,8 +308,12 @@
     assert res_fold is None
     training = torch.is_grad_enabled() and layer.weight.requires_grad
     if tap and torch.is_grad_enabled():
-        return _Conv2dFn.apply(x, layer.weight, layer.bias, view_bias, residual, layer, mode, training, twin, True)
-    y = _Conv2dFn.apply(x, layer.weight, layer.bias, view_bias, residual, layer, mode, training, twin)
+        return _Conv2dFn.apply(x, layer.weight, layer.bias, view_bias, residual, layer, mode, training, twin, True, 0, 0)
+    from_gn = x.__dict__.pop("_vf_gn", 0) if torch.is_grad_enabled() else 0
+    if from_gn and (x.retains_grad or x._backward_hooks):
+        from_gn = 0
+    y = _Conv2dFn.apply(x, layer.weight, layer.bias, view_bias, residual, layer, mode, training, twin, False,
+                        int(gn_next), int(from_gn))
     return (y, x) if tap else y
 
 
diff --git a/view_fusion_amd/ops/norm.py b/view_fusion_amd/ops/norm.py
--- a/view_fusion_amd/ops/norm.py
+++ b/view_fusion_amd/ops/norm.py
@@ -6,12 +6,28 @@
 from .deferred import _colsum, _rowsum_put
 
 
+def _tail_take(t):
+    if not st._TAILS:
+        return None
+    rec = st._TAILS.pop(t.data_ptr(), None)
+    if rec is not None and rec[0].shape != t.shape:
+        raise _lib.VFHipError("a conv output with a deferred fix-up reached a GroupNorm of another shape")
+    return rec
+
+
 def _gn_forward(x, gamma, beta, groups, silu):
     _check(x, gamma, beta)
     S, C, H, W = x.shape
     y = torch.empty_like(x)
     mean = torch.empty(S * groups, device=x.device, dtype=torch.float32)
     rstd = torch.empty_like(mean)
+    tail = _tail_take(x)
+    if tail is not None:
+        _, ws, kind, nfull, split, bias, vbias, res = tail
+        _launch("gn_fwd", 0.0, "vf_gn_fwd_tail", _ptr(x), _ptr(gamma), _ptr(beta), _ptr(y), _ptr(mean), _ptr(rstd), S, C,
+                H * W, groups, 1e-5, int(silu), _ptr(ws), kind, nfull, split, _ptr(bias), _ptr(vbias), _ptr(res), _stream(),
+                nbytes=8.0 * x.numel())
+        return y, mean, rstd
     _launch("gn_fwd", 0.0, "vf_gn_fwd", _ptr(x), _ptr(gamma), _ptr(beta), _ptr(y), _ptr(mean), _ptr(rstd), S, C, H * W,
             groups, 1e-5, int(silu), _stream(), nbytes=8.0 * x.numel())
     return y, mean, rstd
@@ -37,9 +53,11 @@
         rowsum = torch.empty(S, C, device=x.device, dtype=torch.float32)
     if addend is None and addend2 is not None:
         addend, addend2 = addend2, None
-    _launch("gn_bwd", 0.0, "vf_gn_cat_bwd", _ptr(x), None, C, _ptr(gamma), _ptr(beta), _ptr(mean), _ptr(rstd), _ptr(dy),
+    tail = _tail_take(dy)
+    name, targs = ("vf_gn_cat_bwd", ()) if tail is None else ("vf_gn_cat_bwd_tail", (_ptr(tail[1]), *tail[2:5]))
+    _launch("gn_bwd", 0.0, name, _ptr(x), None, C, _ptr(gamma), _ptr(beta), _ptr(mean), _ptr(rstd), _ptr(dy),
             _ptr(addend), _ptr(addend2), _ptr(dx), None, _ptr(parts[0]), _ptr(parts[1]), _ptr(rowsum), S, C, H * W,
-            ctx.groups, ctx.silu, _stream(),
+            ctx.groups, ctx.silu, *targs, _stream(),
             nbytes=4.0 * x.numel() * (3 + (addend is not None) + (addend2 is not None)))
     if rowsum is not None:
         _rowsum_put(dx, rowsum, None)
@@ -104,10 +122,18 @@
         d2 = None if d2 is None else _c(d2)
         dx1, dx2 = torch.empty_like(x1), torch.empty_like(x2)
         parts = torch.empty(2, S, C, device=x1.device, dtype=torch.float32)
-        _launch("gn_bwd", 0.0, "vf_gn_cat_bwd", _ptr(x1), _ptr(x2), C1, _ptr(gamma), _ptr(beta), _ptr(mean), _ptr(rstd),
+        tail = _tail_take(dy)
+        name, targs = ("vf_gn_cat_bwd", ()) if tail is None else ("vf_gn_cat_bwd_tail", (_ptr(tail[1]), *tail[2:5]))
+        _launch("gn_bwd", 0.0, name, _ptr(x1), _ptr(x2), C1, _ptr(gamma), _ptr(beta), _ptr(mean), _ptr(rstd),
                 _ptr(dy), _ptr(d1), _ptr(d2), _ptr(dx1), _ptr(dx2), _ptr(parts[0]), _ptr(parts[1]), None, S, C, H * W,
-                ctx.groups, ctx.silu, _stream(), nbytes=4.0 * dy.numel() * (3 + (d1 is not None)))
+                ctx.groups, ctx.silu, *targs, _stream(), nbytes=4.0 * dy.numel() * (3 + (d1 is not None)))
         return (dx1, dx2, *_gb_grads(parts, ctx.gb), None, None)
+
+
+def _mark(y, groups):
+    if y.requires_grad:
+        y._vf_gn = groups
+    return y
 
 
 def cat_fusable(C1, C, HW, groups):
@@ -115,16 +141,18 @@
 
 
 def group_norm_cat_skip(x1, x2, weight, bias, groups, silu):
-    return _GroupNormCatSkipFn.apply(x1, x2, weight, bias, groups, silu)
+    out = _GroupNormCatSkipFn.apply(x1, x2, weight, bias, groups, silu)
+    return (_mark(out[0], groups), *out[1:])
 
 
 def group_norm(x, weight, bias, groups, silu):
-    return _GroupNormFn.apply(x, weight, bias, groups, silu)
+    return _mark(_GroupNormFn.apply(x, weight, bias, groups, silu), groups)
 
 
 def group_norm_skip(x, weight, bias, groups, silu, tap=False):
     if not (torch.is_grad_enabled() and x.requires_grad):
-        y = _GroupNormFn.apply(x, weight, bias, groups, silu)
+        y = _mark(_GroupNormFn.apply(x, weight, bias, groups, silu), groups)
         return (y, x, x) if tap else (y, x)
     out = _GroupNormSkipFn.apply(x, weight, bias, groups, silu)
+    _mark(out[0], groups)
     return out if tap else out[:2]
diff --git a/view_fusion_amd/ops/state.py b/view_fusion_amd/ops/state.py
--- a/view_fusion_amd/ops/state.py
+++ b/view_fusion_amd/ops/state.py
@@ -21,6 +21,7 @@
         self.SMALL_PACK = os.environ.get("VF_SMALL_PACK", "1") == "1"
         self.RES_FOLD = os.environ.get("VF_RES_FOLD", "1") == "1"
         self.WINO_GN_FUSION = os.environ.get("VF_WINO_GN", "1") == "1"
+        self.GN_FIXUP = os.environ.get("VF_GN_FIXUP", "1") != "0"
         self.ATTN_DSCORE = os.environ.get("VF_ATTN_DSCORE", "1") != "0"
         self.ATTN_DVDK = os.environ.get("VF_ATTN_DVDK", "1") != "0"
         self.BF16X3 = os.environ.get("VF_BF16X3") == "1"
@@ -32,6 +33,7 @@
         self.slab_sums = None
         self._PENDING_TASK = None
         self._WRED_ARENA = {}
+        self._TAILS = {}
         self._ws = {}
         self._WINO_KIND_CACHE = {}
         self._TA_DESC = {}
diff --git a/view_fusion_amd/unet.py b/view_fusion_amd/unet.py
--- a/view_fusion_amd/unet.py
+++ b/view_fusion_amd/unet.py
@@ -60,7 +60,7 @@
             return ops.conv2d(a2, conv2, residual=res, res_fold=fold), None
         return ops.conv2d_gn(a2, conv2, next_gn[0], self.groups, next_gn[1], residual=res, want_y=True, res_fold=fold)
 
-    def forward(self, x, e, skip=None, tap=False, draws=None):
+    def forward(self, x, e, skip=None, tap=False, draws=None, gn_next=0):
         from . import ops
         b1, b2 = self.block1["block"], self.block2["block"]
         if skip is not None:
@@ -69,15 +69,16 @@
                 x, skip = ops.concat_channels(x, skip), None
         if skip is not None:
             a, x1, x2 = ops.group_norm_cat_skip(x, skip, b1["0"].weight, b1["0"].bias, self.groups, silu=True)
-            h = ops.conv2d(a, b1["3"], view_bias=e)
+            h = ops.conv2d(a, b1["3"], view_bias=e, gn_next=self.groups)
             a = self._drop(ops.group_norm(h, b2["0"].weight, b2["0"].bias, self.groups, silu=True), draws)
-            return ops.conv2d(a, b2["3"], residual=ops.conv1x1_cat(x1, x2, self.res_conv), twin=self.res_conv)
+            return ops.conv2d(a, b2["3"], residual=ops.conv1x1_cat(x1, x2, self.res_conv), twin=self.res_conv,
+                              gn_next=gn_next)
         a, xs, xt = ops.group_norm_skip(x, b1["0"].weight, b1["0"].bias, self.groups, silu=True, tap=True)
-        h = ops.conv2d(a, b1["3"], view_bias=e)
+        h = ops.conv2d(a, b1["3"], view_bias=e, gn_next=self.groups)
         a = self._drop(ops.group_norm(h, b2["0"].weight, b2["0"].bias, self.groups, silu=True), draws)
         twin = None if isinstance(self.res_conv, nn.Identity) else self.res_conv
         skip = xs if twin is None else ops.conv2d(xs, twin)
-        y = ops.conv2d(a, b2["3"], residual=skip, twin=twin)
+        y = ops.conv2d(a, b2["3"], residual=skip, twin=twin, gn_next=gn_next)
         return (y, xt) if tap else y
 
 
@@ -114,12 +115,14 @@
             return self.attn(y, n), None
         return self.res_block._forward_inference(x, e, skip, a_in, next_gn)
 
-    def forward(self, x, e, skip=None, tap=False, draws=None):
+    def forward(self, x, e, skip=None, tap=False, draws=None, gn_next=0):
         xt = None
+        if self.with_attn:
+            gn_next = self.attn.groups
         if tap:
-            x, xt = self.res_block(x, e, skip, tap=True, draws=draws)
+            x, xt = self.res_block(x, e, skip, tap=True, draws=draws, gn_next=gn_next)
         else:
-            x = self.res_block(x, e, skip, draws=draws)
+            x = self.res_block(x, e, skip, draws=draws, gn_next=gn_next)
         x = self.attn(x) if self.with_attn else x
         return (x, xt) if tap else x
 
@@ -292,10 +295,13 @@
             return self._forward_inference(x, iter(embed()))
         es = iter(embed())
 
+        ng = self.norm_groups
+        downs = list(self.downs) + [self.mid[0]]
         feats = []
-        for layer in self.downs:
-            if isinstance(layer, _ResAttnBlock):
-                x, xin = layer(x, next(es), tap=True, draws=draws)
+        for i, layer in enumerate(self.downs):
+            if isinstance(layer, _ResAttnBlock):
+                x, xin = layer(x, next(es), tap=True, draws=draws,
+                               gn_next=ng if isinstance(downs[i + 1], _ResAttnBlock) else 0)
                 if feats:
                     feats[-1] = xin
             elif isinstance(layer, _Resample):
@@ -308,13 +314,14 @@
         first = True
         for layer in self.mid:
             if first:
-                x, feats[-1] = layer(x, next(es), tap=True, draws=draws)
+                x, feats[-1] = layer(x, next(es), tap=True, draws=draws, gn_next=0 if layer.with_attn else ng)
                 first = False
             else:
                 x = layer(x, next(es), draws=draws)
-        for layer in self.ups:
-            if isinstance(layer, _ResAttnBlock):
-                x = layer(x, next(es), feats.pop(), draws=draws)
+        for i, layer in enumerate(self.ups):
+            if isinstance(layer, _ResAttnBlock):
+                last = i + 1 == len(self.ups) and not layer.with_attn
+                x = layer(x, next(es), feats.pop(), draws=draws, gn_next=ng if last else 0)
             else:
                 x = layer(x)
         fc = self.final_conv["block"]
```

Measured after the change: 3277 view denoise-steps/s (UNet fwd+bwd per stacked view, incl. compose/MSE/Adam), median of 6. Within noise of the previous version (+0.4%).
